# mountain/qingdai

Measured on AMD Instinct MI355X. Metric: simulated planet-days/sec at 721x1440 f64, higher is better.
Workload: dtype f64; 1 GPU; 721x1440 seed-42 planet, dt=300 s: forcing + time_step(Teq, dt, albedo) with QD_ENERGY_W=1 QD_CLOUD_COUPLE=1 + slab-ocean coupling + driver-side precipitation/cloud/albedo diagnostics (run_simulation.py:1766-1934,2063-2146) (BASELINE configs[2]; loop order of benchmark_jax.py:124-158); ocean_n_sub=13, parallelism=lat-bands x1

## Files before the change

qingdai_amd/csrc/qd_api.hip:

```cpp
#include "qd_span.h"
#include <chrono>
#include <atomic>
#include <cstring>
#include <cstdio>
#include <cstdlib>
#include <algorithm>

thread_local std::string g_qd_create_err;

int qd_fail(qd_ctx* c, const char* what, hipError_t e) {
    std::string m = what ? what : "error";
    if (e != hipSuccess) { m += ": "; m += hipGetErrorString(e); }
    if (c) c->err = m; else g_qd_create_err = m;
    return -1;
}

static hipEvent_t qd_get_event(qd_ctx* c) {
    if (!c->ev_free.empty()) { hipEvent_t e = c->ev_free.back(); c->ev_free.pop_back(); return e; }
    hipEvent_t e = nullptr;
    hipEventCreate(&e);
    return e;
}
QdScope::QdScope(qd_ctx* c_, const char* n, bool attach_) : c(c_), name(n), attach(attach_) {
    on = c->timing == 1;
// ... 64 lines not shown
        double s = (lat_deg - p.polar_sponge_lat) / std::max(1e-6, 90.0 - p.polar_sponge_lat);
        s = std::min(std::max(s, 0.0), 1.0);
        rx[i] = p.polar_sponge_gain * (s * s);
    }
    {
        const double a = p.a, dphi = c->dlat, dlam = c->dlon;
        const double f_min = 2.0 * p.omega * std::sin(5.0 * (M_PI / 180.0));
        for (int k = 0; k < 2; ++k) {
            const std::vector<double>& ck = k == 0 ? c02 : c05;
            std::vector<double> A(nlat), P(nlat), Q(nlat);
            for (int i = 0; i < nlat; ++i) {
                A[i] = ck[i] / (2.0 * dphi);
                P[i] = 1.0 / ((a * a) * ck[i] * (2.0 * dphi));
                Q[i] = 1.0 / ((a * a) * (dlam * dlam) * (ck[i] * ck[i]));
            }
            std::vector<double> PA(8, 0.0);
            if (nlat >= 5) {
                const int n = nlat;
                PA[0] = ck[0] / dphi;               PA[1] = ck[1] / (2.0 * dphi);      P[0] = 1.0 / ((a * a) * ck[0] * dphi);
                PA[2] = ck[0] / dphi;               PA[3] = ck[2] / (2.0 * dphi);      P[1] = 1.0 / ((a * a) * ck[1] * (2.0 * dphi));
                PA[4] = ck[n - 3] / (2.0 * dphi);   PA[5] = ck[n - 1] / dphi;          P[n - 2] = 1.0 / ((a * a) * ck[n - 2] * (2.0 * dphi));
                PA[6] = ck[n - 2] / (2.0 * dphi);   PA[7] = ck[n - 1] / dphi;          P[n - 1] = 1.0 / ((a * a) * ck[n - 1] * dphi);
            }
            c->tabs.lapA[k] = dev_table(c, A); c->tabs.lapP[k] = dev_table(c, P); c->tabs.lapQ[k] = dev_table(c, Q);
            c->tabs.lapPoleA[k] = dev_table(c, PA);
            std::vector<double> K4((size_t)nlat * 4);
            for (int i = 0; i < nlat; ++i) {
                K4[4 * i + 0] = A[i > 0 ? i - 1 : 0]; K4[4 * i + 1] = A[i < nlat - 1 ? i + 1 : nlat - 1];
                K4[4 * i + 2] = P[i]; K4[4 * i + 3] = Q[i];
            }
            c->tabs.lapK[k] = dev_table(c, K4);
            c->h_lapK[k] = K4;
        }
        std::vector<double> cu(nlat), cv(nlat), px(nlat), igx(nlat), ia6(nlat);
        for (int i = 0; i < nlat; ++i) {
            const double f = fc[i];
            const double sgn = f >= 0.0 ? 1.0 : -1.0;
            const double f_safe = std::fabs(f) < f_min ? sgn * f_min : f;
            cu[i] = -(p.g / (f_safe * a * c6[i]));
            cv[i] = p.g / (f_safe * a);
            px[i] = -(p.g / (a * c6[i]));
            igx[i] = 1.0 / (a * c05[i]);
            ia6[i] = 1 / (a * c6[i]);
        }
        c->tabs.mom_cu = dev_table(c, cu); c->tabs.mom_cv = dev_table(c, cv); c->tabs.mom_px = dev_table(c, px);
        c->tabs.ocn_igx = dev_table(c, igx);
        c->tabs.inv_acos6 = dev_table(c, ia6);
    }
    std::vector<double> lr(nlon), sl(nlon), cl(nlon);
    for (int j = 0; j < nlon; ++j) { lr[j] = lon[j] * d2r; sl[j] = std::sin(lr[j]); cl[j] = std::cos(lr[j]); }
    QdTabs& T = c->tabs;
    T.cos_raw = dev_table(c, cr); T.sin_raw = dev_table(c, sr); T.cos6 = dev_table(c, c6); T.cos3 = dev_table(c, c3);
    T.cos02 = dev_table(c, c02); T.cos05 = dev_table(c, c05); T.fcor = dev_table(c, fc); T.warea = dev_table(c, wa);
    T.r_extra = dev_table(c, rx);
    T.lat_deg = dev_table(c, lat);
    T.lon_rad = dev_table(c, lr); T.sin_lon = dev_table(c, sl); T.cos_lon = dev_table(c, cl);
    if (!T.cos_raw || !T.lon_rad || !T.cos_lon) return -1;
    double ws = 0.0;
    for (int i = 0; i < nlat; ++i) ws += wa[i] * nlon;
    c->wsum_all = ws;
    return 0;
}

int qd_build_k4_tables(qd_ctx* c, double dt, bool ocean, double sub_dt) {
    const int nlat = c->geo.nlat;
    const qd_params& p = c->p;
    const double d2r = M_PI / 180.0;
    std::vector<double> lat = linspace(-90.0, 90.0, nlat);
    auto isset = [](double x) { return !(x != x); };
    if (!ocean) {
        if (c->k4_atm_dt == dt) return 0;
        std::vector<double> tab((size_t)5 * nlat);
        const double scale[5] = {1.0, 1.0, 0.5, 0.5, 0.25};
        const double ov[5] = {p.k4_u, p.k4_v, p.k4_h, p.k4_q, p.k4_cloud};
        bool anypos[5] = {false, false, false, false, false};
        for (int i = 0; i < nlat; ++i) {
            const double cs = std::max(std::cos(lat[i] * d2r), 1e-3);
            const double dxm = std::min(p.a * c->dlat, p.a * c->dlon * cs);
            const double base = p.sigma4 * std::pow(dxm, 4.0) / std::max(1e-12, dt);
            for (int f = 0; f < 5; ++f) {
// ... 738 lines not shown
```

qingdai_amd/csrc/qd_atmos.hip:

```cpp
#include "qd_internal.h"
#include "qd_pointwise.h"
#include "qd_device.h"
#include "qd_saf.h"

#include "qd_fluxes.h"
#include "qd_fused.h"

struct QdColPtrs {
    const double *u, *v, *Teq, *isr, *albedo, *csmap;
    double *h, *Ts, *q, *cloud, *hice;
    double *E, *Pcond, *LH, *LHrel, *olr, *cloud_eff;
    const uint8_t* land;
    const double* pref;
    unsigned long long* npos;
};

struct QdColIn { double cloud, isr, albedo, teq; };

template <int PHASE, bool HAS_ALB>
__device__ __forceinline__ void qd_column_cell(const QdColP& P, const QdColPtrs& A, size_t o, const QdColIn* IN, int i, int nlat) {
    const double u = A.u[o], v = A.v[o], h = A.h[o], Ts = A.Ts[o];
    const double hice = A.hice[o];
    const bool land = (A.land[o] == 1);
    const bool ocean = !land;
    const double T_a = 288.0 + P.ga * h;
    const double qsat_air = qd_qsat(T_a, P.p0);

    const QdHum Hm = qd_humidity_column(P, u, v, Ts, A.q[o], qsat_air, land, hice);
    const double q = Hm.q, E = Hm.E, Pc = Hm.Pc, LH = Hm.LH, LHrel = Hm.LHrel;
    if (PHASE == 1) { A.Pcond[o] = Pc; return; }
    A.q[o] = q; A.LH[o] = LH;
    if (PHASE != 2) A.Pcond[o] = Pc;
    if (P.write_diag) { A.E[o] = E; A.LHrel[o] = LHrel; }

    const double Teq = IN ? IN->teq : A.Teq[o];
    const double olr_old = P.sigma * qd_pow4(Ts);
    const double net_old = P.sigma * qd_pow4(Teq) + P.gfs * qd_pow4(T_a) - olr_old;
    const double Ts_newton = Ts + (net_old / P.c_sfc_safe) * P.dt;

    double Ts_new, h_new = h;
    QdFlux F;
    if (HAS_ALB) {
        const double cloud = IN ? IN->cloud : A.cloud[o];
        double cloud_eff;
        if (P.couple) {
            const double RH = qd_clip(q / qd_max(1e-12, qsat_air), 0.0, 1.5);
            const double rh_excess = qd_max(0.0, RH - P.rh0);
            const double P_ref = *A.pref;
            const double p_term = qd_tanh(P_ref > 0 ? Pc / P_ref : 0.0);
            cloud_eff = qd_clip(cloud + P.k_q * rh_excess + P.k_p * p_term, 0.0, 1.0);
        } else cloud_eff = cloud;
        A.cloud_eff[o] = cloud_eff;
        F = qd_surface_fluxes(P, IN ? IN->isr : A.isr[o], IN ? IN->albedo : A.albedo[o], cloud_eff, Ts, T_a, u, v, land, hice);
        double Ts_energy;
        if (P.seaice) {
            double Q = F.SW_sfc - F.LW_sfc - F.SH - LH;
            double Tn = Ts, hi = hice;
            if (hi > 0.0 && ocean && Q > 0.0) {
                const double dh_melt = (Q * P.dt) / P.rhoiLf;
                const double dh_cap = qd_min(dh_melt, hi);
                hi -= dh_cap;
                Q = Q - (dh_cap * P.rho_i * P.L_f) / P.dt;
            }
            if (ocean && Q < 0.0 && Tn <= (P.t_freeze + 0.5)) {
                hi += (-Q * P.dt) / P.rhoiLf;
                Q = 0.0;
                Tn = qd_min(Tn, P.t_freeze);
            }
            double Cs = land ? P.Cs_land : (hi > 0.0 ? P.Cs_ice : P.Cs_ocean);
            Cs = (isfinite(Cs) && Cs > 1e3) ? Cs : 1e3;
            Tn = Tn + (Q / Cs) * P.dt;
            if ((i == 0 && P.fix_s) || (i == nlat - 1 && P.fix_n)) {
                if (ocean && Q < 0.0 && Tn > P.t_freeze) Tn = P.t_freeze;
            }
            if (hi > 0.0 && ocean) Tn = qd_min(Tn, P.t_freeze);
            Tn = qd_max(P.t_floor, Tn);
            Ts_energy = qd_nn(Tn);
            { const double hn_ = qd_nn(hi); if (__double_as_longlong(hn_) != __double_as_longlong(hice)) A.hice[o] = hn_; }
        } else {
            const double net = F.SW_sfc - F.LW_sfc - F.SH - LH;
            double Cs;
            if (P.has_csmap) { const double cm = A.csmap[o]; Cs = (isfinite(cm) && cm > 1e3) ? cm : 1e3; }
            else Cs = P.c_sfc_safe;
            Ts_energy = qd_nn(qd_max(P.t_floor, Ts + (net / Cs) * P.dt));
        }
        if (P.write_diag) A.olr[o] = F.OLR;
        Ts_new = (1.0 - P.w_energy) * Ts_newton + P.w_energy * Ts_energy;
    } else {
        if (P.write_diag) A.olr[o] = olr_old;
        Ts_new = Ts_newton;
    }
    A.Ts[o] = Ts_new;

    const double h_eq = P.h_eq_fac * Teq;
    h_new = h + ((h_eq - h) / P.tau_rad) * P.dt;
    if (HAS_ALB && P.atm_couple) {
        const double F_atm = F.SW_atm + F.LW_atm + F.SH + LHrel;
        h_new = qd_nn(h_new + P.atm_w * (F_atm / P.atm_denom) * P.dt);
    }
    A.h[o] = h_new;
}

template <int PHASE, bool HAS_ALB>
__global__ void __launch_bounds__(QD_BLOCK)
k_column(QdGeom G, QdColP P, QdColPtrs A) {
    const QdTile tl = qd_tile();
    const int j = tl.seg * QD_BLOCK + threadIdx.x;
    if (j >= G.nlon) return;
    const int i = G.row0 + tl.row;
    qd_column_cell<PHASE, HAS_ALB>(P, A, (size_t)qd_lrow(G, i) * G.nlon + j, nullptr, i, G.nlat);
}

__global__ void __launch_bounds__(QD_BLOCK)
k_saf_column2(QdSafArgs K, QdColP P, QdColPtrs A) {
    const QdTile tl = qd_tile();
    const int j = tl.seg * QD_BLOCK + threadIdx.x;
    if (j >= K.G.nlon) return;
    const int i = K.G.row0 + tl.row;
    const size_t o = (size_t)qd_lrow(K.G, i) * K.G.nlon + j;
    const QdSafOut s = qd_saf_cell(K, i, j, o, K.write_diag != 0);
    const QdColIn in{s.cloud, s.isr, s.albedo, s.teq};
    qd_column_cell<2, true>(P, A, o, &in, i, K.G.nlat);
}

struct QdMomP { double g, a, dt, dlat, dlon, f_min; int primitive; };

__global__ void __launch_bounds__(QD_BLOCK)
k_momentum(QdGeom G, QdTabs T, QdMomP P, const double* __restrict__ h, const double* __restrict__ fric,
           double* __restrict__ u, double* __restrict__ v) {
    const QdTile tl = qd_tile();
    const int j = tl.seg * QD_BLOCK + threadIdx.x;
    if (j >= G.nlon) return;
    const int i = G.row0 + tl.row;
    const int n = G.nlat, m = G.nlon;
    const size_t b = (size_t)qd_lrow(G, i) * m;
    const size_t o = b + j;
    double dh_dlon;
    if (j == 0) dh_dlon = (h[b + 1] - h[b]) / P.dlon;
    else if (j == m - 1) dh_dlon = (h[b + m - 1] - h[b + m - 2]) / P.dlon;
    else dh_dlon = (h[b + j + 1] - h[b + j - 1]) / (2.0 * P.dlon);
    double dh_dlat;
    if (i == 0) dh_dlat = (h[(size_t)qd_lrow(G, 1) * m + j] - h[o]) / P.dlat;
    else if (i == n - 1) dh_dlat = (h[o] - h[(size_t)qd_lrow(G, n - 2) * m + j]) / P.dlat;
    else dh_dlat = (h[(size_t)qd_lrow(G, i + 1) * m + j] - h[(size_t)qd_lrow(G, i - 1) * m + j]) / (2.0 * P.dlat);
    const double cosc = T.cos6[i];
    const double f = T.fcor[i];
    const double r = fric[o];
    const double u0 = u[o], v0 = v[o];
    if (P.primitive) {
        const double PGF_x = -(P.g / (P.a * cosc)) * dh_dlon;
        const double PGF_y = -(P.g / P.a) * dh_dlat;
        const double du = (PGF_x + f * v0 - r * u0) * P.dt;
        const double dv = (PGF_y - f * u0 - r * v0) * P.dt;
        u[o] = qd_clip(u0 + du, -200.0, 200.0);
        v[o] = qd_clip(v0 + dv, -200.0, 200.0);
    } else {
        const double sgn = (f >= 0.0) ? 1.0 : -1.0;
        const double f_safe = (fabs(f) < P.f_min) ? sgn * P.f_min : f;
        const double u_g = qd_clip(-(P.g / (f_safe * P.a * cosc)) * dh_dlat, -200.0, 200.0);
        const double v_g = qd_clip((P.g / (f_safe * P.a)) * dh_dlon, -200.0, 200.0);
        double un = u0 * 0.8 + u_g * 0.2;
        double vn = v0 * 0.8 + v_g * 0.2;
        un = un + (-r * un) * P.dt;
        vn = vn + (-r * vn) * P.dt;
        u[o] = un; v[o] = vn;
    }
}

__global__ void __launch_bounds__(QD_BLOCK)
k_final(QdGeom G, const double* __restrict__ cosl, double dt, double a, double dlat, double dlon,
        double* __restrict__ u, double* __restrict__ v, double* __restrict__ h, double* __restrict__ Ts,
        double* __restrict__ q, const double* __restrict__ cloud_in, double* __restrict__ cloud_out,
        double decay, double dfac) {
    const QdTile tl = qd_tile();
    const int j = tl.seg * QD_BLOCK + threadIdx.x;
    if (j >= G.nlon) return;
    const int i = G.row0 + tl.row;
    const size_t o = (size_t)qd_lrow(G, i) * G.nlon + j;
    const double uu = u[o], vv = v[o];
    const QdBilin b = qd_departure(G, i, j, uu, vv, dt, a, cosl[i], dlat, dlon);
    double c = qd_gather(cloud_in, G, b);
    c = c * decay;
    cloud_out[o] = qd_nn(c * dfac);
    u[o] = qd_nn(uu * dfac);
    v[o] = qd_nn(vv * dfac);
    h[o] = qd_nn(h[o] * dfac);
    q[o] = qd_nn(q[o] * dfac);
    Ts[o] = qd_nn(Ts[o]);
}

__global__ void __launch_bounds__(QD_BLOCK)
k_forcing(QdGeom G, QdTabs T, QdForcingP P, double* __restrict__ isrA, double* __restrict__ isrB, double* __restrict__ isr,
          const double* __restrict__ albedo, double* __restrict__ Teq, double* __restrict__ eday, double eday_dt) {
    const QdTile tl = qd_tile();
    const int j = tl.seg * QD_BLOCK + threadIdx.x;
    if (j >= G.nlon) return;
    const int i = G.row0 + tl.row;
    const size_t o = (size_t)qd_lrow(G, i) * G.nlon + j;
    qd_forcing_cell(T, P, i, j, o, P.with_teq ? albedo[o] : 0.0, isrA, isrB, isr, Teq, eday, eday_dt);
}

int qd_forcing_impl(qd_ctx* c, const double* sa, const double* sb, double theta, int with_teq) {
    QdScope sc(c, "forcing");
    QdStar A{sa[0], std::sin(sa[1]), std::cos(sa[1]), sa[2]};
    QdStar B{sb[0], std::sin(sb[1]), std::cos(sb[1]), sb[2]};
    const int m = with_teq ? qd_plan(c, {QD_IN(c->f[QD_F_ALBEDO], 0)}) : c->geo.halo;
    if (m < 0) return -1;
    const QdForcingP FP{A, B, theta, 5.670374e-8, with_teq};
    QD_ROWS(c, m, G, hipLaunchKernelGGL(k_forcing, qd_grid2d(G), dim3(QD_BLOCK), 0, c->stream, G, c->tabs, FP,
                                        c->f[QD_F_ISR_A], c->f[QD_F_ISR_B], c->f[QD_F_ISR],
                                        c->f[QD_F_ALBEDO], c->f[QD_F_TEQ], c->eco.eday_dt > 0 ? c->f[QD_F_ECO_EDAY] : (double*)nullptr,
                                        c->eco.eday_dt));
    c->eco.eday_dt = 0;
// ... 24 lines not shown

QdColP qd_make_colp(const qd_ctx* c, double dt) {
    const qd_params& p = c->p;
    QdColP P;
    P.ga = p.g / 1004.0;
    P.M_col = std::max(1e-6, p.rho_a * p.h_mbl);
    P.tau_c = std::max(1e-6, p.tau_cond);
    P.L_v = p.L_v; P.p0 = p.p0; P.rhoCE = p.rho_a * p.C_E;
    P.s_ocean = p.ocean_evap_scale; P.s_land = p.land_evap_scale; P.s_ice = p.ice_evap_scale;
    P.sigma = 5.670374e-8;
    P.gfs = p.greenhouse_factor * P.sigma;
    P.c_sfc_safe = std::max(1e-12, p.c_sfc);
    P.dt = dt;
    P.rh0 = p.rh0; P.k_q = p.k_q; P.k_p = p.k_p;
    P.sw_a0 = p.sw_a0; P.sw_kc = p.sw_kc; P.lw_eps0 = p.lw_eps0; P.lw_kc = p.lw_kc;
    P.eps_clear = std::min(std::max(p.lw_eps0, 0.0), 1.0);
    P.tau0 = p.lw_tau0; P.k_tau = p.lw_ktau;
    P.hice_ref_safe = std::max(1e-6, p.hice_ref);
    P.eps_ocean = p.eps_ocean; P.eps_land = p.eps_land; P.eps_ice = p.eps_ice; P.eps_default = p.eps_default;
    P.g_lw = p.gh_factor_lw;
    P.rhocpch = p.rho_a * p.cp_a * p.ch;
    P.t_freeze = p.t_freeze; P.rho_i = p.rho_i; P.L_f = p.L_f; P.rhoiLf = p.rho_i * p.L_f;
    P.Cs_ocean = p.Cs_ocean; P.Cs_land = p.Cs_land; P.Cs_ice = p.Cs_ice; P.t_floor = p.t_floor;
    P.w_energy = std::min(1.0, std::max(0.0, p.energy_w));
    P.h_eq_fac = 287.0 / p.g;
    P.tau_rad = p.tau_rad;
    const double H_atm = qd_isset(p.atm_h) ? p.atm_h : p.h_mbl;
    P.atm_denom = std::max(1e-6, p.rho_a) * std::max(1.0, H_atm) * p.g;
    P.atm_w = p.energy_w;
    P.atm_couple = (p.energy_w > 0.0) ? 1 : 0;
    P.couple = p.cloud_couple; P.lw_v2 = p.lw_v2; P.gh_lock = p.gh_lock; P.seaice = p.seaice_enabled;
    P.fix_s = p.polar_freeze_fix_s; P.fix_n = p.polar_freeze_fix_n; P.has_csmap = p.has_csmap;
    P.write_diag = c->diag_write;
    return P;
}

__global__ void k_set_scalar(double* p, double v) { if (threadIdx.x == 0 && blockIdx.x == 0) *p = v; }
__global__ void k_zero_count(unsigned long long* p) { if (threadIdx.x == 0 && blockIdx.x == 0) *p = 0ull; }

static QdColPtrs qd_col_ptrs(qd_ctx* c) {
    double** F = c->f;
    QdColPtrs A;
    A.u = F[QD_F_U]; A.v = F[QD_F_V]; A.Teq = F[QD_F_TEQ]; A.isr = F[QD_F_ISR];
    A.albedo = F[QD_F_ALBEDO]; A.csmap = F[QD_F_CSMAP];
    A.h = F[QD_F_H]; A.Ts = F[QD_F_TS]; A.q = F[QD_F_Q]; A.cloud = F[QD_F_CLOUD]; A.hice = F[QD_F_HICE];
    A.E = F[QD_F_EFLUX]; A.Pcond = F[QD_F_PCOND]; A.LH = F[QD_F_LH]; A.LHrel = F[QD_F_LHREL];
    A.olr = F[QD_F_OLR]; A.cloud_eff = F[QD_F_CLOUD_EFF];
    A.land = c->land; A.pref = c->dscal + QD_S_PREF; A.npos = c->dcount;
    return A;
}

int qd_pcond_phase1(qd_ctx* c, double dt) {
    hipLaunchKernelGGL((k_column<1, true>), qd_grid2d(c->geo), dim3(QD_BLOCK), 0, c->stream, c->geo, qd_make_colp(c, dt), qd_col_ptrs(c));
    return 0;
}
int qd_pcond_median_side(qd_ctx* c, double dt) {
    QD_HIP(c, hipEventRecord(c->med_fork, c->stream));
    QD_HIP(c, hipStreamWaitEvent(c->side_stream, c->med_fork, 0));
    std::swap(c->stream, c->side_stream);
    c->med_side_active = true;
    const QdColP P = qd_make_colp(c, dt);
    const QdColPtrs A = qd_col_ptrs(c);
    hipLaunchKernelGGL((k_column<1, true>), qd_grid2d(c->geo), dim3(QD_BLOCK), 0, c->stream, c->geo, P, A);
    const int r = qd_median_positive_dev(c, c->f[QD_F_PCOND], 1e-6, QD_S_PREF, 0, 0.0, 1);
    c->med_side_active = false;
    std::swap(c->stream, c->side_stream);
// ... 13 lines not shown

    if (c->saf_pending && !(has_albedo && p.cloud_couple && !qd_isset(p.pcond_ref) && c->pcond_ahead == 3) && qd_saf_flush(c)) return -1;
    {
        QdScope sc(c, "column");
        int m = has_albedo
            ? qd_plan(c, {QD_IN(F[QD_F_U], 0), QD_IN(F[QD_F_V], 0), QD_IN(F[QD_F_H], 0), QD_IN(F[QD_F_TS], 0), QD_IN(F[QD_F_Q], 0),
                          QD_IN(F[QD_F_CLOUD], 0), QD_IN(F[QD_F_HICE], 0), QD_IN(F[QD_F_TEQ], 0), QD_IN(F[QD_F_ISR], 0),
                          QD_IN(F[QD_F_ALBEDO], 0)})
            : qd_plan(c, {QD_IN(F[QD_F_U], 0), QD_IN(F[QD_F_V], 0), QD_IN(F[QD_F_H], 0), QD_IN(F[QD_F_TS], 0), QD_IN(F[QD_F_Q], 0),
                          QD_IN(F[QD_F_HICE], 0), QD_IN(F[QD_F_TEQ], 0)});
        if (m < 0) return -1;
        QdColPtrs A;
        A.u = F[QD_F_U]; A.v = F[QD_F_V]; A.Teq = F[QD_F_TEQ]; A.isr = F[QD_F_ISR];
        A.albedo = F[QD_F_ALBEDO]; A.csmap = F[QD_F_CSMAP];
        A.h = F[QD_F_H]; A.Ts = F[QD_F_TS]; A.q = F[QD_F_Q]; A.cloud = F[QD_F_CLOUD]; A.hice = F[QD_F_HICE];
        A.E = F[QD_F_EFLUX]; A.Pcond = F[QD_F_PCOND]; A.LH = F[QD_F_LH]; A.LHrel = F[QD_F_LHREL];
        A.olr = F[QD_F_OLR]; A.cloud_eff = F[QD_F_CLOUD_EFF];
        A.land = c->land; A.pref = c->dscal + QD_S_PREF; A.npos = c->dcount;
        if (!has_albedo) {
            QD_ROWS(c, m, G, hipLaunchKernelGGL((k_column<0, false>), qd_grid2d(G), blk, 0, c->stream, G, P, A));
        } else if (!p.cloud_couple || qd_isset(p.pcond_ref)) {
            hipLaunchKernelGGL(k_set_scalar, dim3(1), dim3(1), 0, c->stream, c->dscal + QD_S_PREF,
                               qd_isset(p.pcond_ref) ? p.pcond_ref : 1e-6);
            QD_ROWS(c, m, G, hipLaunchKernelGGL((k_column<0, true>), qd_grid2d(G), blk, 0, c->stream, G, P, A));
        } else {
            const int ahead = c->pcond_ahead;
            c->pcond_ahead = 0;
            if (!ahead) QD_ROWS(c, m, G, hipLaunchKernelGGL((k_column<1, true>), qd_grid2d(G), blk, 0, c->stream, G, P, A));
            if (ahead == 2) QD_HIP(c, hipStreamWaitEvent(c->stream, c->med_done, 0));
            else if (ahead != 3 && qd_median_positive_dev(c, F[QD_F_PCOND], 1e-6, QD_S_PREF, 0, 0.0, 1)) return -1;
            if (c->saf_pending && ahead == 3 && c->geo.full) {
                QdSafArgs* K = (QdSafArgs*)c->saf_pending;
                c->saf_pending = nullptr;
                hipLaunchKernelGGL(k_saf_column2, qd_grid2d(K->G), blk, 0, c->stream, *K, P, A);
                delete K;
            } else {
                if (qd_saf_flush(c)) return -1;
                QD_ROWS(c, m, G, hipLaunchKernelGGL((k_column<2, true>), qd_grid2d(G), blk, 0, c->stream, G, P, A));
            }
        }
        qd_mark(c, {F[QD_F_H], F[QD_F_TS], F[QD_F_Q], F[QD_F_EFLUX], F[QD_F_PCOND], F[QD_F_LH], F[QD_F_LHREL], F[QD_F_OLR]}, m);
        if (has_albedo) { qd_mark(c, {F[QD_F_HICE], F[QD_F_CLOUD_EFF]}, m); c->cloud_eff_valid = 1; }
    }
    c->atm_counter += 1;
    const int64_t sc_ = c->atm_counter;

    {
        QdScope sc(c, "advect_tsq");
        const int m = qd_plan(c, {QD_IN(F[QD_F_TS], R), QD_IN(F[QD_F_Q], R), QD_IN(F[QD_F_U], 0), QD_IN(F[QD_F_V], 0)});
        if (m < 0) return -1;
        double* oT = qd_scratch(c, 0); double* oq = qd_scratch(c, 1);
        qd_launch_advect(c, F[QD_F_U], F[QD_F_V], c->tabs.cos6, dt, F[QD_F_TS], oT, F[QD_F_Q], oq, 0.2, 1, m);
        qd_swap(c, QD_F_TS, 0); qd_swap(c, QD_F_Q, 1);
    }
    const int ft = p.filter_type;
    const bool do_diff = p.diff_enable && (ft == 0 || ft == 1) && (sc_ % std::max(1, p.diff_every) == 0);
    const double f_min = 2.0 * p.omega * std::sin(5.0 * (M_PI / 180.0));
    if (do_diff) { int rc = qd_build_k4_tables(c, dt, false, 0.0); if (rc) return rc; }
    const double ov[5] = {p.k4_u, p.k4_v, p.k4_h, p.k4_q, p.k4_cloud};
    if (do_diff && c->use_fused && p.k4_nsub == 1) {
        const int m = qd_plan(c, {QD_IN(F[QD_F_H], 5), QD_IN(F[QD_F_U], 4), QD_IN(F[QD_F_V], 4), QD_IN(F[QD_F_FRICTION], 4),
                                  QD_IN(F[QD_F_Q], 4), QD_IN(F[QD_F_CLOUD], 4)});
        if (m < 0) return -1;
        QdDynArgs D;
        D.u = F[QD_F_U]; D.v = F[QD_F_V]; D.h = F[QD_F_H]; D.fric = F[QD_F_FRICTION];
        D.q = F[QD_F_Q]; D.cloud = F[QD_F_CLOUD];
        D.uo = qd_scratch(c, 0); D.vo = qd_scratch(c, 1); D.ho = qd_scratch(c, 2); D.qo = qd_scratch(c, 3); D.co = qd_scratch(c, 4);
// ... 41 lines not shown
        const int m = qd_plan(c, {QD_IN(F[QD_F_U], np_), QD_IN(F[QD_F_V], np_), QD_IN(F[QD_F_H], np_)});
        if (m < 0) return -1;
        double* fl[3] = {F[QD_F_U], F[QD_F_V], F[QD_F_H]};
        qd_shapiro_fields(c, fl, 3, np_, m);
        F[QD_F_U] = fl[0]; F[QD_F_V] = fl[1]; F[QD_F_H] = fl[2];
        const int n1 = std::max(1, p.shapiro_n - 1);
        if (p.diff_q) {
            const int mq = qd_plan(c, {QD_IN(F[QD_F_Q], n1)}); if (mq < 0) return -1;
            double* g1[1] = {F[QD_F_Q]}; qd_shapiro_fields(c, g1, 1, n1, mq); F[QD_F_Q] = g1[0];
        }
        if (p.diff_cloud) {
            const int mc = qd_plan(c, {QD_IN(F[QD_F_CLOUD], n1)}); if (mc < 0) return -1;
            double* g1[1] = {F[QD_F_CLOUD]}; qd_shapiro_fields(c, g1, 1, n1, mc); F[QD_F_CLOUD] = g1[0];
        }
    }
    if ((ft == 0 || ft == 3) && p.spec_every > 0 && (sc_ % p.spec_every == 0)) {
        QdScope sc(c, "zonal_filter");
        const int m = qd_plan(c, {QD_IN(F[QD_F_U], 0), QD_IN(F[QD_F_V], 0), QD_IN(F[QD_F_H], 0)});
        if (m < 0) return -1;
        double* fl[3] = {F[QD_F_U], F[QD_F_V], F[QD_F_H]};
        if (qd_zonal_filter_fields(c, fl, 3, p.spec_cutoff, p.spec_damp, m)) return -1;
    }
    {
        QdScope sc(c, "final");
        const int m = qd_plan(c, {QD_IN(F[QD_F_CLOUD], R), QD_IN(F[QD_F_U], 0), QD_IN(F[QD_F_V], 0), QD_IN(F[QD_F_H], 0),
                                  QD_IN(F[QD_F_TS], 0), QD_IN(F[QD_F_Q], 0)});
        if (m < 0) return -1;
        const double decay = 1 - dt / (2.0 * 24 * 3600);
        if (c->defer_final && c->geo.full) {
            c->final_pending.on = 1; c->final_pending.dt = dt; c->final_pending.decay = decay; c->final_pending.dfac = p.diff_factor;
            return 0;
        }
        double* oc = qd_scratch(c, 0);
        QD_ROWS(c, m, G, hipLaunchKernelGGL(k_final, qd_grid2d(G), blk, 0, c->stream, G, c->tabs.cos6, dt, p.a, c->dlat, c->dlon,
                                            F[QD_F_U], F[QD_F_V], F[QD_F_H], F[QD_F_TS], F[QD_F_Q], F[QD_F_CLOUD], oc, decay,
                                            p.diff_factor));
        qd_mark(c, {F[QD_F_U], F[QD_F_V], F[QD_F_H], F[QD_F_TS], F[QD_F_Q], oc}, m);
        qd_swap(c, QD_F_CLOUD, 0);
    }
    return 0;
}
```

qingdai_amd/csrc/qd_device.h:

```cpp
#pragma once
#include "qd_internal.h"
#include "qd_math.h"

template <bool SCRUB>
__device__ __forceinline__ double qd_ld(const double* __restrict__ F, const QdGeom& G, int g, int j) {
    double x = F[(size_t)qd_lrow(G, g) * G.nlon + j];
    return SCRUB ? qd_nn(x) : x;
}

template <bool SCRUB>
__device__ __forceinline__ double qd_dphi(const double* __restrict__ F, const QdGeom& G, int r, int j, double dphi) {
    const int n = G.nlat;
    if (r == 0) return (qd_ld<SCRUB>(F, G, 1, j) - qd_ld<SCRUB>(F, G, 0, j)) / dphi;
    if (r == n - 1) return (qd_ld<SCRUB>(F, G, n - 1, j) - qd_ld<SCRUB>(F, G, n - 2, j)) / dphi;
    return (qd_ld<SCRUB>(F, G, r + 1, j) - qd_ld<SCRUB>(F, G, r - 1, j)) / (2.0 * dphi);
}

template <bool SCRUB>
__device__ __forceinline__ double qd_lap_point(const double* __restrict__ F, const QdGeom& G,
                                               const double* __restrict__ cosf, int i, int j,
                                               double dphi, double dlam, double a) {
    const int n = G.nlat;
    int ra, rb; double den;
    if (i == 0) { ra = 0; rb = 1; den = dphi; }
// ... 4 lines not shown
    const double ci = cosf[i];
    const double term_phi = (1.0 / ci) * ((Gb - Ga) / den);
    const int jp = qd_wrapc(j + 1, G.nlon), jm = qd_wrapc(j - 1, G.nlon);
    const double c = qd_ld<SCRUB>(F, G, i, j);
    const double d2 = ((qd_ld<SCRUB>(F, G, i, jp) - 2.0 * c) + qd_ld<SCRUB>(F, G, i, jm)) / (dlam * dlam);
    const double term_lam = d2 / (ci * ci);
    return (term_phi + term_lam) / (a * a);
}


template <bool SCRUB>
__device__ __forceinline__ double qd_lap_point_fast(const double* __restrict__ F, const QdGeom& G, const QdTabs& T,
                                                    int k, int i, int j, double dphi, double dlam, double a) {
    if (i < 2 || i > G.nlat - 3) return qd_lap_point<SCRUB>(F, G, k ? T.cos05 : T.cos02, i, j, dphi, dlam, a);
    const int jp = qd_wrapc(j + 1, G.nlon), jm = qd_wrapc(j - 1, G.nlon);
    const double cc = qd_ld<SCRUB>(F, G, i, j);
    const double Gb = T.lapA[k][i + 1] * (qd_ld<SCRUB>(F, G, i + 2, j) - cc);
    const double Ga = T.lapA[k][i - 1] * (cc - qd_ld<SCRUB>(F, G, i - 2, j));
    const double d2 = (qd_ld<SCRUB>(F, G, i, jp) - 2.0 * cc) + qd_ld<SCRUB>(F, G, i, jm);
    return T.lapP[k][i] * (Gb - Ga) + T.lapQ[k][i] * d2;
}

__device__ __forceinline__ double qd_fold(double x, int n) {
    const double sz = (double)(n - 1);
    if (n <= 1) return 0.0;
    if (x < 0.0) return x + sz * (trunc(-x / sz) + 1.0);
    if (x > sz) return x - sz * trunc(x / sz);
    return x;
}

struct QdBilin { int l0, l1, c0, c1; double wr0, wr1, wc0, wc1; bool nan_coord; };

__device__ __forceinline__ QdBilin qd_departure(const QdGeom& G, int gi, int j, double u, double v, double dt,
                                                double a, double cosl, double dlat, double dlon) {
    const double dl = u * dt / (a * cosl);
    const double dp = v * dt / a;
    const double dx = dl / dlon;
    const double dy = dp / dlat;
    double r = qd_fold((double)gi - dy, G.nlat);
    double cc = qd_fold((double)j - dx, G.nlon);
    const bool nan_coord = (dx != dx) || (dy != dy);
    r = fmin(fmax(r, 0.0), (double)(G.nlat - 1));
    cc = fmin(fmax(cc, 0.0), (double)(G.nlon - 1));
    const double r0f = floor(r), c0f = floor(cc);
    QdBilin b;
    const int r0 = (int)r0f, c0 = (int)c0f;
    const int r1 = r0 + 1 < G.nlat ? r0 + 1 : G.nlat - 1;
    b.c0 = c0; b.c1 = c0 + 1 < G.nlon ? c0 + 1 : G.nlon - 1;
    b.l0 = qd_lrow_far(G, r0); b.l1 = qd_lrow_far(G, r1);
    const double tr = r - r0f, tc = cc - c0f;
    b.wr0 = 1.0 - tr; b.wr1 = tr; b.wc0 = 1.0 - tc; b.wc1 = tc;
    b.nan_coord = nan_coord;
    return b;
}

__device__ __forceinline__ double qd_gather(const double* __restrict__ F, const QdGeom& G, const QdBilin& b) {
    const size_t r0 = (size_t)b.l0 * G.nlon, r1 = (size_t)b.l1 * G.nlon;
    double t = 0.0;
    t += F[r0 + b.c0] * b.wr0 * b.wc0;
    t += F[r0 + b.c1] * b.wr0 * b.wc1;
    t += F[r1 + b.c0] * b.wr1 * b.wc0;
    t += F[r1 + b.c1] * b.wr1 * b.wc1;
    return b.nan_coord ? 0.0 : t;
}


__device__ __forceinline__ double qd_divvort_point(const QdGeom& G, const QdTabs& T, const double* __restrict__ p,
                                                   const double* __restrict__ q, int i, int j, double a,
                                                   double dlat, double dlon, int vort) {
    const size_t b = (size_t)qd_lrow(G, i) * G.nlon;
    const int jp = qd_wrapc(j + 1, G.nlon), jm = qd_wrapc(j - 1, G.nlon);
    const double dp = (p[b + jp] - p[b + jm]) / (2 * dlon);
    double dq = 0.0;
    if (i != 0 && i != G.nlat - 1) {
        const double qn = q[(size_t)qd_lrow(G, i + 1) * G.nlon + j] * T.cos_raw[i + 1];
        const double qs = q[(size_t)qd_lrow(G, i - 1) * G.nlon + j] * T.cos_raw[i - 1];
        dq = (qn - qs) / (2 * dlat);
    }
    const double pre = 1 / (a * T.cos6[i]);
    return vort ? pre * (dp - dq) : pre * (dp + dq);
}
```

qingdai_amd/csrc/qd_fluxes.h:

```cpp
#pragma once
#include "qd_internal.h"

#define QD_EPSILON 0.622

struct QdColP {
    double ga;
    double M_col, tau_c, L_v, p0, rhoCE, s_ocean, s_land, s_ice;
    double sigma, gfs, c_sfc_safe, dt;
    double rh0, k_q, k_p;
    double sw_a0, sw_kc, lw_eps0, lw_kc, eps_clear, tau0, k_tau, hice_ref_safe;
    double eps_ocean, eps_land, eps_ice, eps_default;
    double g_lw, rhocpch;
    double t_freeze, rhoiLf, rho_i, L_f, Cs_ocean, Cs_land, Cs_ice, t_floor;
    double w_energy, h_eq_fac, tau_rad, atm_denom, atm_w;
    int couple, lw_v2, gh_lock, seaice, fix_s, fix_n, has_csmap, atm_couple;
    int write_diag = 1;
};

__device__ __forceinline__ double qd_qsat(double T, double p0) {
    const double T_c = qd_clip(T - 273.15, -80.0, 60.0);
    const double e_s = 610.94 * exp(17.625 * T_c / (T_c + 243.04));
    const double denom = qd_max(p0 - (1.0 - QD_EPSILON) * e_s, 1.0);
    return qd_clip(QD_EPSILON * e_s / denom, 0.0, 0.5);
}

struct QdHum { double q, E, Pc, LH, LHrel; };
__device__ __forceinline__ QdHum qd_humidity_column(const QdColP& P, double u, double v, double Ts, double q0, double qsat_air,
                                                    bool land, double hice) {
    QdHum r;
    const double fac = land ? P.s_land : ((hice > 1e-6) ? P.s_ice : P.s_ocean);
    const double V = sqrt(u * u + v * v);
    const double deficit = qd_max(0.0, qd_qsat(Ts, P.p0) - q0);
    r.E = qd_nn(P.rhoCE * V * deficit * fac);
    r.LH = P.L_v * r.E;
    const double q_evap = q0 + (r.E / P.M_col) * P.dt;
    const double excess = qd_max(0.0, q_evap - qsat_air);
    double Pc = (excess / P.tau_c) * P.M_col;
    double q_next = q_evap - (Pc / P.M_col) * P.dt;
    q_next = qd_clip(qd_nn(q_next), 0.0, 0.5);
    r.Pc = qd_nn(Pc);
    r.LHrel = P.L_v * r.Pc;
    r.q = qd_clip(qd_nn(q_next), 0.0, 0.5);
    return r;
}

struct QdFlux { double SW_atm, SW_sfc, R, LW_atm, LW_sfc, OLR, SH; };

__device__ __forceinline__ QdFlux qd_surface_fluxes(const QdColP& P, double I, double albedo, double cloud_eff,
                                                    double Ts, double Ta, double u, double v, bool land, double hice) {
    QdFlux F;
    const double alpha = qd_clip(albedo, 0.0, 1.0);
    const double Ic = qd_max(0.0, I);
    F.R = Ic * alpha;
    const double A_sw = qd_clip(P.sw_a0 + P.sw_kc * qd_clip(cloud_eff, 0.0, 1.0), 0.0, 0.95);
    F.SW_atm = Ic * A_sw;
    F.SW_sfc = qd_max(0.0, Ic - F.R - F.SW_atm);
    const double s = P.sigma;
    const double Tsp = qd_max(0.0, Ts), Tap = qd_max(0.0, Ta);
    const double Ts4 = qd_pow4(Tsp), Ta4 = qd_pow4(Tap);
    if (P.lw_v2) {
        const double ce = qd_clip(cloud_eff, 0.0, 1.0);
        const double tau_cloud = P.tau0 * ce;
        const double eps_cloud = qd_clip(1.0 - exp(-P.k_tau * tau_cloud), 0.0, 1.0);
        const double eps_eff = 1.0 - (1.0 - P.eps_clear) * (1.0 - eps_cloud);
        double es;
        if (land) es = P.eps_land;
        else {
            const double ice_frac = 1.0 - exp(-qd_max(hice, 0.0) / P.hice_ref_safe);
            const double fi = qd_clip(ice_frac, 0.0, 1.0);
            es = (1.0 - fi) * P.eps_ocean + fi * P.eps_ice;
        }
        es = qd_clip(qd_nn(es), 0.0, 1.0);
        F.OLR = eps_eff * s * Ta4 + (1.0 - eps_eff) * s * es * Ts4;
        const double DLR = eps_eff * s * Ta4;
        F.LW_sfc = DLR - s * es * Ts4;
        F.LW_atm = eps_eff * (s * es * Ts4 - 2.0 * s * Ta4);
        if (P.gh_lock) {
            F.OLR = (1.0 - P.g_lw) * s * Ts4;
            const double DLRt = P.g_lw * s * Ts4;
            F.LW_sfc = DLRt - s * es * Ts4;
        }
    } else {
        const double eps = qd_clip(P.lw_eps0 + P.lw_kc * qd_clip(cloud_eff, 0.0, 1.0), 0.0, 1.0);
        F.OLR = eps * s * Ta4 + (1.0 - eps) * s * Ts4;
        const double DLR = eps * s * Ta4;
        F.LW_sfc = DLR - s * Ts4;
        F.LW_atm = eps * (s * Ts4 - 2.0 * s * Ta4);
        if (P.gh_lock) {
            F.OLR = (1.0 - P.g_lw) * s * Ts4;
            const double DLRt = P.g_lw * s * Ts4;
            F.LW_sfc = DLRt - s * Ts4;
        }
    }
    const double V = sqrt(u * u + v * v);
    F.SH = P.rhocpch * V * (Ts - Ta);
    return F;
}
```

qingdai_amd/csrc/qd_internal.h:

```cpp
#pragma once

#include <hip/hip_runtime.h>
#include <hip/hip_ext.h>
#include <stdint.h>
#include <string>
#include <vector>
#include <functional>
#include <map>
#include <unordered_map>
#include <initializer_list>
#include <climits>
#include <cfloat>
#include <cmath>

#include "../../include/qingdai_hip.h"

#define QD_NSCRATCH 16
#define QD_MAX_DEVICES 64
#define QD_PAD_ROWS 8
#define QD_BLOCK 256
#define QD_MAXF 5
#define QD_HIST_BINS 2048

struct QdGeom {
    int nlat, nlon;
    int row0, nrows, halo;
    int full;
    int lbase;
    int lrows_;
    __host__ __device__ inline int lrows() const { return lrows_; }
    __host__ __device__ inline size_t cells() const { return (size_t)lrows() * (size_t)nlon; }
};

struct QdTabs {
    const double* cos_raw;
    const double* sin_raw;
    const double* cos6;
    const double* cos3;
    const double* cos02;
    const double* cos05;
    const double* fcor;
    const double* warea;
    const double* r_extra;
    const double* lapA[2];
    const double* lapP[2];
    const double* lapQ[2];
    const double* lapPoleA[2];
    const double* lapK[2];
    const double* mom_cu;
    const double* mom_cv;
    const double* mom_px;
    const double* ocn_igx;
    const double* inv_acos6;
    const double* lat_deg;
    const double* lon_rad;
    const double* sin_lon;
    const double* cos_lon;
};

__device__ __forceinline__ double qd_nn(double x) {
    if (x != x) return 0.0;
    if (x > DBL_MAX) return DBL_MAX;
    if (x < -DBL_MAX) return -DBL_MAX;
    return x;
}
__device__ __forceinline__ double qd_max(double a, double b) {
    return (a >= b || a != a) ? a : b;
}
__device__ __forceinline__ double qd_min(double a, double b) {
    return (a <= b || a != a) ? a : b;
}
__device__ __forceinline__ double qd_clip(double x, double lo, double hi) {
    return qd_min(qd_max(x, lo), hi);
}
__device__ __forceinline__ double qd_pow4(double x) { double x2 = x * x; return x2 * x2; }

__device__ __forceinline__ int qd_lrow(const QdGeom& G, int g) {
    int l = g - G.lbase;
    if (l < 0) l += G.nlat; else if (l >= G.nlat) l -= G.nlat;
    return l;
}
__device__ __forceinline__ int qd_lrow_far(const QdGeom& G, int g) {
    int l = g - G.lbase;
    if (l < 0) l += G.nlat; else if (l >= G.nlat) l -= G.nlat;
    if (l >= G.lrows()) l = G.lrows() - 1;
    return l;
}
__device__ __forceinline__ int qd_wrapc(int j, int n) {
    return j < 0 ? j + n : (j >= n ? j - n : j);
}

// ... 365 lines not shown
```

qingdai_amd/csrc/qd_math.h:

```cpp
#pragma once
#include <math.h>
#ifdef __HIPCC__
#define QD_MATH_FN __host__ __device__ __forceinline__
#else
#define QD_MATH_FN static inline
#endif

QD_MATH_FN double qd_expm1_pos(double y) {
    const double k = rint(y * 1.4426950408889634);
    double r = fma(k, -6.93147180369123816490e-01, y);
    r = fma(k, -1.90821492927058770002e-10, r);
    double p = 1.0 / 6227020800.0;
    p = fma(p, r, 1.0 / 479001600.0);
    p = fma(p, r, 1.0 / 39916800.0);
    p = fma(p, r, 1.0 / 3628800.0);
    p = fma(p, r, 1.0 / 362880.0);
    p = fma(p, r, 1.0 / 40320.0);
    p = fma(p, r, 1.0 / 5040.0);
    p = fma(p, r, 1.0 / 720.0);
    p = fma(p, r, 1.0 / 120.0);
    p = fma(p, r, 1.0 / 24.0);
    p = fma(p, r, 1.0 / 6.0);
    p = fma(p, r, 0.5);
    p = fma(p, r, 1.0);
    const double pm1 = p * r;
    const double twok = ldexp(1.0, (int)k);
    return fma(twok, pm1, twok - 1.0);
}

QD_MATH_FN double qd_tanh_nonneg(double x) {
    const double s = x * x;
    double q = 18888466084.0 / 194896477400625.0;
    q = fma(q, s, -443861162.0 / 1856156927625.0);
    q = fma(q, s, 6404582.0 / 10854718875.0);
    q = fma(q, s, -929569.0 / 638512875.0);
    q = fma(q, s, 21844.0 / 6081075.0);
    q = fma(q, s, -1382.0 / 155925.0);
    q = fma(q, s, 62.0 / 2835.0);
    q = fma(q, s, -17.0 / 315.0);
    q = fma(q, s, 2.0 / 15.0);
    q = fma(q, s, -1.0 / 3.0);
    const double small = fma(x * s, q, x);
    const double xe = x < 19.1 ? x : 19.1;
    const double em1 = qd_expm1_pos(xe + xe);
    const double big = em1 / (em1 + 2.0);
    const double t = x < 0.25 ? small : big;
    return x != x ? x : t;
}

QD_MATH_FN double qd_tanh(double x) { return copysign(qd_tanh_nonneg(fabs(x)), x); }
```

qingdai_amd/csrc/qd_ocean.hip:

```cpp
#include <cstdlib>
#include <atomic>
#include <chrono>
#include "qd_internal.h"
#include "qd_device.h"
#include "qd_wave.h"

#include "qd_fluxes.h"
#include "qd_fused.h"
#include "qd_ocntail.h"
#include "qd_band.h"
#include "qd_blockred.h"

QdColP qd_make_colp(const qd_ctx* c, double dt);

__global__ void __launch_bounds__(QD_BLOCK)
k_qnet(QdGeom G, QdColP P, const double* __restrict__ isr, const double* __restrict__ albedo,
       const double* __restrict__ cloud, const double* __restrict__ Ts, const double* __restrict__ h,
       const double* __restrict__ u, const double* __restrict__ v, const uint8_t* __restrict__ land,
       const double* __restrict__ hice, const double* __restrict__ LH, double* __restrict__ qnet,
       uint8_t* __restrict__ icemask) {
    const QdTile tl = qd_tile();
    const int j = tl.seg * QD_BLOCK + threadIdx.x;
    if (j >= G.nlon) return;
    const size_t o = (size_t)qd_lrow(G, G.row0 + tl.row) * G.nlon + j;
// ... 84 lines not shown
             double* __restrict__ taux, double* __restrict__ tauy, double* __restrict__ partial, double* seq_out, double seq) {
    __shared__ double sm[2][QD_BLOCK / 64];
    const int i = G.row0 + blockIdx.y;
    const size_t b = (size_t)qd_lrow(G, i) * G.nlon;
    double mVa = 0.0, mUo = 0.0;
    for (int j = threadIdx.x; j < G.nlon; j += QD_BLOCK) {
        const size_t o = b + j;
        const double u_o = uo[o], v_o = vo[o];
        const double u_rel = ua[o] - u_o, v_rel = va[o] - v_o;
        const double Va = sqrt(u_rel * u_rel + v_rel * v_rel);
        const double Va_eff = qd_min(Va, vcap);
        taux[o] = tau_scale * (rhoCD * Va_eff * u_rel);
        tauy[o] = tau_scale * (rhoCD * Va_eff * v_rel);
        const double so = sqrt(u_o * u_o + v_o * v_o);
        mVa = Va > mVa ? Va : mVa;
        mUo = so > mUo ? so : mUo;
    }
    mVa = qd_wave_max(mVa); mUo = qd_wave_max(mUo);
    const int lane = threadIdx.x & 63, w = threadIdx.x >> 6;
    if (lane == 0) { sm[0][w] = mVa; sm[1][w] = mUo; }
    __syncthreads();
    if (threadIdx.x == 0) {
        for (int k = 1; k < QD_BLOCK / 64; ++k) { mVa = sm[0][k] > mVa ? sm[0][k] : mVa; mUo = sm[1][k] > mUo ? sm[1][k] : mUo; }
        partial[blockIdx.y] = mVa;
        partial[gridDim.y + blockIdx.y] = mUo;
        if (seq_out) {
            asm volatile("s_waitcnt vmcnt(0)" ::: "memory");
            __hip_atomic_store(seq_out + blockIdx.y, seq, __ATOMIC_RELAXED, __HIP_MEMORY_SCOPE_SYSTEM);
        }
    }
}

struct QdFqsArgs {
    const double* cosl; double dt, a, dlat, dlon, decay, dfac;
    double *u, *v, *h, *Ts, *q; const double* cloud_in; double* cloud_out;
    const double *isr, *albedo, *cloud_eff, *hice, *LH; const uint8_t* land; double* qnet; uint8_t* icemask;
    const double *uo, *vo; double vcap, rhoCD, tau_scale; double *taux, *tauy;
    double* dev_wg; int n_wg;
};
__global__ void __launch_bounds__(QD_BLOCK)
k_final_qnet_stress(QdGeom G, QdColP P, QdFqsArgs A) {
    __shared__ double sm[2][QD_BLOCK / 64];
    const QdTile tl = qd_tile();
    const int j = tl.seg * QD_BLOCK + threadIdx.x;
    const int i = G.row0 + tl.row;
    double Va = 0.0, so = 0.0;
    if (j < G.nlon) {
        const size_t o = (size_t)qd_lrow(G, i) * G.nlon + j;
        const double uu = A.u[o], vv = A.v[o];
        const QdBilin b = qd_departure(G, i, j, uu, vv, A.dt, A.a, A.cosl[i], A.dlat, A.dlon);
        double c = qd_gather(A.cloud_in, G, b);
        c = c * A.decay;
        const double cn = qd_nn(c * A.dfac), un = qd_nn(uu * A.dfac), vn = qd_nn(vv * A.dfac);
        const double t0 = A.Ts[o];
        const double hn = qd_nn(A.h[o] * A.dfac), tn = qd_nn(t0);
        A.cloud_out[o] = cn; A.u[o] = un; A.v[o] = vn; A.h[o] = hn; A.q[o] = qd_nn(A.q[o] * A.dfac);
        if (__double_as_longlong(tn) != __double_as_longlong(t0)) A.Ts[o] = tn;
        const double u_o = A.uo[o], v_o = A.vo[o];
        const double u_rel = un - u_o, v_rel = vn - v_o;
        Va = sqrt(u_rel * u_rel + v_rel * v_rel);
        const double Va_eff = qd_min(Va, A.vcap);
        A.taux[o] = A.tau_scale * (A.rhoCD * Va_eff * u_rel);
        A.tauy[o] = A.tau_scale * (A.rhoCD * Va_eff * v_rel);
        so = sqrt(u_o * u_o + v_o * v_o);
        const double T_a = 288.0 + P.ga * hn;
        const double hi = A.hice[o];
        const QdFlux F = qd_surface_fluxes(P, A.isr[o], A.albedo[o], A.cloud_eff ? A.cloud_eff[o] : cn, tn, T_a, un, vn, A.land[o] == 1, hi);
        A.qnet[o] = F.SW_sfc - F.LW_sfc - F.SH - A.LH[o];
        A.icemask[o] = (hi > 0.0) ? 1 : 0;
    }
    double mVa = Va > 0.0 ? Va : 0.0, mUo = so > 0.0 ? so : 0.0;
    mVa = qd_wave_max(mVa); mUo = qd_wave_max(mUo);
    const int lane = threadIdx.x & 63, w = threadIdx.x >> 6;
    if (lane == 0) { sm[0][w] = mVa; sm[1][w] = mUo; }
    __syncthreads();
    if (threadIdx.x == 0) {
        for (int k = 1; k < QD_BLOCK / 64; ++k) { mVa = sm[0][k] > mVa ? sm[0][k] : mVa; mUo = sm[1][k] > mUo ? sm[1][k] : mUo; }
        const unsigned wg = (unsigned)tl.row * gridDim.x + (unsigned)tl.seg;
        A.dev_wg[wg] = mVa; A.dev_wg[A.n_wg + wg] = mUo;
    }
}

__global__ void __launch_bounds__(1024)
// ... 37 lines not shown
}

struct QdOcnP { double a, g, dlat, dlon, sub_dt, rhoH, r_bot; };

__global__ void __launch_bounds__(QD_BLOCK)
k_ocean_momentum(QdGeom G, QdTabs T, QdOcnP P, const double* __restrict__ eta, const double* __restrict__ taux,
                 const double* __restrict__ tauy, const uint8_t* __restrict__ land,
                 double* __restrict__ uo, double* __restrict__ vo) {
    const QdTile tl = qd_tile();
    const int j = tl.seg * QD_BLOCK + threadIdx.x;
    if (j >= G.nlon) return;
    const int i = G.row0 + tl.row;
    const size_t b = (size_t)qd_lrow(G, i) * G.nlon;
    const size_t o = b + j;
    const int jp = qd_wrapc(j + 1, G.nlon), jm = qd_wrapc(j - 1, G.nlon);
    const double deta_dlam = (eta[b + jp] - eta[b + jm]) / (2.0 * P.dlon);
    const double deta_dphi = (eta[(size_t)qd_lrow(G, i + 1) * G.nlon + j] - eta[(size_t)qd_lrow(G, i - 1) * G.nlon + j]) / (2.0 * P.dlat);
    const double gx = deta_dlam / (P.a * T.cos05[i]);
    const double gy = deta_dphi / P.a;
    const double f = T.fcor[i];
    const double u0 = uo[o], v0 = vo[o];
    const double du = (f * v0 - P.g * gx + taux[o] / P.rhoH - P.r_bot * u0);
    const double dv = (-f * u0 - P.g * gy + tauy[o] / P.rhoH - P.r_bot * v0);
    double un = u0 + P.sub_dt * du;
    double vn = v0 + P.sub_dt * dv;
    if (land[o] == 1) { un = 0.0; vn = 0.0; }
    const double rx = T.r_extra[i];
    un = un - P.sub_dt * rx * un;
    vn = vn - P.sub_dt * rx * vn;
    uo[o] = un; vo[o] = vn;
}

__global__ void __launch_bounds__(QD_BLOCK)
k_continuity(QdGeom G, QdTabs T, double a, double dlat, double dlon, double msdtH, const double* __restrict__ uo,
             const double* __restrict__ vo, const uint8_t* __restrict__ land, double* __restrict__ eta,
             double* __restrict__ partial) {
    __shared__ double sm[QD_BLOCK / 64];
    const int i = G.row0 + blockIdx.y;
    const size_t b = (size_t)qd_lrow(G, i) * G.nlon;
    const double w = T.warea[i];
    double acc = 0.0;
    for (int j = threadIdx.x; j < G.nlon; j += QD_BLOCK) {
        const size_t o = b + j;
        const double div = qd_divvort_point(G, T, uo, vo, i, j, a, dlat, dlon, 0);
        double e = eta[o] + msdtH * div;
        const bool island = land[o] == 1;
        if (island) e = 0.0;
        eta[o] = e;
        acc += e * (island ? 0.0 : w);
    }
    acc = qd_wave_sum(acc);
    const int lane = threadIdx.x & 63, wv = threadIdx.x >> 6;
    if (lane == 0) sm[wv] = acc;
    __syncthreads();
    if (threadIdx.x == 0) {
        double r = sm[0];
        for (int k = 1; k < QD_BLOCK / 64; ++k) r += sm[k];
        partial[blockIdx.y] = r;
    }
}

__global__ void __launch_bounds__(QD_BLOCK)
k_eta_mean(const double* __restrict__ partial, int n, double wsum, double* __restrict__ out, double seq = 0.0) {
    __shared__ double sm[QD_BLOCK / 64];
    double acc = 0.0;
    for (int k = threadIdx.x; k < n; k += QD_BLOCK) acc += partial[k];
    acc = qd_wave_sum(acc);
    const int lane = threadIdx.x & 63, wv = threadIdx.x >> 6;
    if (lane == 0) sm[wv] = acc;
    __syncthreads();
    if (threadIdx.x == 0) {
        double r = sm[0];
        for (int k = 1; k < QD_BLOCK / 64; ++k) r += sm[k];
        *out = (wsum < 0.0) ? r : r / (wsum + 1e-15);
        if (seq != 0.0) __hip_atomic_store(&out[1], seq, __ATOMIC_RELEASE, __HIP_MEMORY_SCOPE_SYSTEM);
    }
}

__global__ void __launch_bounds__(QD_BLOCK)
k_cont_sstadv(QdGeom G, QdTabs T, double a, double dlat, double dlon, double msdtH, double sub_dt, double alpha,
              const double* __restrict__ uo, const double* __restrict__ vo, const uint8_t* __restrict__ land,
              double* __restrict__ eta, const double* __restrict__ Ts, double* __restrict__ Ts_out,
              int own0, int own1, double* __restrict__ partial, unsigned long long* ticket, double wsum,
              double* __restrict__ eta_mean) {
    __shared__ double sm[QD_BLOCK / 64];
    __shared__ int s_last;
    const int i = G.row0 + blockIdx.y;
    const size_t b = (size_t)qd_lrow(G, i) * G.nlon;
    const double w = (i >= own0 && i < own1) ? T.warea[i] : 0.0;
    const double cosl = T.cos05[i];
    const int pidx = blockIdx.y * gridDim.x + blockIdx.x, pcount = gridDim.x * gridDim.y;
    double acc = 0.0;
    for (int j = blockIdx.x * QD_BLOCK + threadIdx.x; j < G.nlon; j += gridDim.x * QD_BLOCK) {
        const size_t o = b + j;
        const double div = qd_divvort_point(G, T, uo, vo, i, j, a, dlat, dlon, 0);
        double e = eta[o] + msdtH * div;
        const bool island = land[o] == 1;
        if (island) e = 0.0;
        eta[o] = e;
        acc += e * (island ? 0.0 : w);
        const QdBilin bl = qd_departure(G, i, j, uo[o], vo[o], sub_dt, a, cosl, dlat, dlon);
        Ts_out[o] = (1.0 - alpha) * Ts[o] + alpha * qd_gather(Ts, G, bl);
    }
    acc = qd_wave_sum(acc);
    const int lane = threadIdx.x & 63, wv = threadIdx.x >> 6;
    if (lane == 0) sm[wv] = acc;
    __syncthreads();
    if (threadIdx.x == 0) {
        double r = sm[0];
        for (int k = 1; k < QD_BLOCK / 64; ++k) r += sm[k];
        if (!ticket) partial[pidx] = r;
        else {
            __hip_atomic_store(&partial[pidx], r, __ATOMIC_RELAXED, __HIP_MEMORY_SCOPE_AGENT);
            asm volatile("s_waitcnt vmcnt(0)" ::: "memory");
            const unsigned long long t = atomicAdd(ticket, 1ull);
            s_last = (t == (unsigned long long)pcount - 1ull) ? 1 : 0;
        }
    }
    if (!ticket) return;
    __syncthreads();
    if (!s_last) return;
    double a2 = 0.0;
    for (int k = threadIdx.x; k < pcount; k += QD_BLOCK)
        a2 += __hip_atomic_load(&partial[k], __ATOMIC_RELAXED, __HIP_MEMORY_SCOPE_AGENT);
    a2 = qd_wave_sum(a2);
    __syncthreads();
    if (lane == 0) sm[wv] = a2;
    __syncthreads();
    if (threadIdx.x == 0) {
        double r = sm[0];
        for (int k = 1; k < QD_BLOCK / 64; ++k) r += sm[k];
        *eta_mean = r / (wsum + 1e-15);
        __hip_atomic_store(ticket, 0ull, __ATOMIC_RELAXED, __HIP_MEMORY_SCOPE_AGENT);
    }
}

__global__ void __launch_bounds__(QD_BLOCK)
k_sst_advect(QdGeom G, const double* __restrict__ cos05, double sub_dt, double a, double dlat, double dlon,
             const double* __restrict__ uo, const double* __restrict__ vo, const double* __restrict__ Ts,
             double* __restrict__ Ts_out, double alpha, double* __restrict__ eta, const double* __restrict__ eta_mean,
             int has_ocean) {
    const QdTile tl = qd_tile();
    const int j = tl.seg * QD_BLOCK + threadIdx.x;
    if (j >= G.nlon) return;
    const int i = G.row0 + tl.row;
    const size_t o = (size_t)qd_lrow(G, i) * G.nlon + j;
    if (has_ocean) eta[o] = eta[o] - *eta_mean;
    const QdBilin b = qd_departure(G, i, j, uo[o], vo[o], sub_dt, a, cos05[i], dlat, dlon);
    const double adv = qd_gather(Ts, G, b);
    Ts_out[o] = (1.0 - alpha) * Ts[o] + alpha * adv;
}

struct QdHeatP { double sub_dt, K_h, rcH, ice_qfac; int use_q, has_ice; };

__global__ void __launch_bounds__(QD_BLOCK)
k_sst_diffuse_heat(QdGeom G, const double* __restrict__ cos05, double dlat, double dlon, double a, QdHeatP P,
                   const double* __restrict__ Ts1, double* __restrict__ Ts_out, const double* __restrict__ qnet,
                   const uint8_t* __restrict__ land, const uint8_t* __restrict__ ice) {
    const QdTile tl = qd_tile();
    const int j = tl.seg * QD_BLOCK + threadIdx.x;
    if (j >= G.nlon) return;
    const int i = G.row0 + tl.row;
    const size_t o = (size_t)qd_lrow(G, i) * G.nlon + j;
    double T = Ts1[o];
    if (P.K_h > 0.0) T = qd_nn(T) + P.sub_dt * P.K_h * qd_lap_point<true>(Ts1, G, cos05, i, j, dlat, dlon, a);
    if (P.use_q) {
        const double heat = qnet[o] / P.rcH;
        const bool ocean = land[o] == 0;
        if (P.has_ice) {
            const bool ic = ice[o] != 0;
            if (ocean && !ic) T = T + P.sub_dt * heat;
            if (P.ice_qfac > 0.0 && ocean && ic) T = T + P.sub_dt * P.ice_qfac * heat;
        } else if (ocean) T = T + P.sub_dt * heat;
    }
    Ts_out[o] = qd_nn(T);
}

__global__ void __launch_bounds__(QD_BLOCK)
k_outlier(QdGeom G, const double* __restrict__ uo, const double* __restrict__ vo, double* __restrict__ uo_out,
          double* __restrict__ vo_out, double* __restrict__ eta, double cap, double eta_cap, int mean4) {
    const QdTile tl = qd_tile();
// ... 259 lines not shown
        QdScope sc(c, "ocean_qnet");
        QdColP P = qd_make_colp_driver(c, dt);
        double*& cl = c->cloud_eff_valid ? F[QD_F_CLOUD_EFF] : F[QD_F_CLOUD];
        const int m = qd_plan(c, {QD_IN(F[QD_F_ISR], 0), QD_IN(F[QD_F_ALBEDO], 0), QD_IN(cl, 0), QD_IN(F[QD_F_TS], 0),
                                  QD_IN(F[QD_F_H], 0), QD_IN(F[QD_F_U], 0), QD_IN(F[QD_F_V], 0), QD_IN(F[QD_F_HICE], 0),
                                  QD_IN(F[QD_F_LH], 0)});
        if (m < 0) return -1;
        QD_ROWS(c, m, G, hipLaunchKernelGGL(k_qnet, qd_grid2d(G), blk, 0, c->stream, G, P, F[QD_F_ISR], F[QD_F_ALBEDO], cl,
                                            F[QD_F_TS], F[QD_F_H], F[QD_F_U], F[QD_F_V], c->land, F[QD_F_HICE], F[QD_F_LH],
                                            F[QD_F_QNET], c->icemask));
        qd_mark(c, {F[QD_F_QNET], c->icemask}, m);
        use_ice_mask = 1;
        return 0;
    };
    if (compute_qnet && band && launch_qnet()) return -1;
    double*& taux = c->scratch[14];
    double*& tauy = c->scratch[15];
    int n_sub;
    bool band_fix_stats = false;
    {
        QdScope sc(c, "ocean_stress");
        const int m = qd_plan(c, {QD_IN(F[QD_F_U], 0), QD_IN(F[QD_F_V], 0), QD_IN(F[QD_F_UO], 0), QD_IN(F[QD_F_VO], 0)});
        if (m < 0) return -1;
        QdSegs S = qd_segments(c, m);
        double maxVa = 0.0, maxUo = 0.0;
        if (!band) {
            const QdGeom& G = S.g[0];
            c->eta_seq += 1.0;
            bool merged_final = false;
            if (c->final_pending.on) {
                if (!compute_qnet) return qd_fail(c, "ocean step: a deferred k_final needs compute_qnet");
                c->final_pending.on = 0;
                QdFqsArgs A;
                A.cosl = c->tabs.cos6; A.dt = c->final_pending.dt; A.a = p.a; A.dlat = c->dlat; A.dlon = c->dlon;
                A.decay = c->final_pending.decay; A.dfac = c->final_pending.dfac;
                A.u = F[QD_F_U]; A.v = F[QD_F_V]; A.h = F[QD_F_H]; A.Ts = F[QD_F_TS]; A.q = F[QD_F_Q];
                A.cloud_in = F[QD_F_CLOUD]; A.cloud_out = qd_scratch(c, 0);
                A.isr = F[QD_F_ISR]; A.albedo = F[QD_F_ALBEDO]; A.cloud_eff = c->cloud_eff_valid ? F[QD_F_CLOUD_EFF] : nullptr;
                A.hice = F[QD_F_HICE]; A.LH = F[QD_F_LH]; A.land = c->land; A.qnet = F[QD_F_QNET]; A.icemask = c->icemask;
                A.uo = F[QD_F_UO]; A.vo = F[QD_F_VO]; A.vcap = p.vcap; A.rhoCD = p.rho_a_ocean * p.CD; A.tau_scale = p.tau_scale;
                A.taux = taux; A.tauy = tauy;
                A.dev_wg = c->wgmax; A.n_wg = c->n_wgmax;
                merged_final = true;
                hipLaunchKernelGGL(k_final_qnet_stress, qd_grid2d(G), blk, 0, c->stream, G, qd_make_colp_driver(c, dt), A);
                hipLaunchKernelGGL(k_max2_publish, dim3(1), dim3(1024), 0, c->stream, c->wgmax, c->n_wgmax, c->hpin + 58, c->fix_count);
                qd_swap(c, QD_F_CLOUD, 0);
                use_ice_mask = 1;
            } else {
            hipLaunchKernelGGL(k_stress_max, dim3(1, G.nrows), blk, 0, c->stream, G, F[QD_F_U], F[QD_F_V], F[QD_F_UO],
                               F[QD_F_VO], p.vcap, p.rho_a_ocean * p.CD, p.tau_scale, taux, tauy, c->hpin_rows,
                               c->hpin_rows + (size_t)2 * G0.lrows(), c->eta_seq);
            qd_mark(c, {taux, tauy}, m);
            if (compute_qnet && launch_qnet()) return -1;
            }
            if (c->before_cfl_wait) {
                std::function<int()> fn = std::move(c->before_cfl_wait);
                c->before_cfl_wait = nullptr;
                if (c->side_stream_on && c->timing != 1 && !c->ocn_fused) {
                    QD_HIP(c, hipEventRecord(c->side_fork, c->stream));
                    QD_HIP(c, hipStreamWaitEvent(c->side_stream, c->side_fork, 0));
                    std::swap(c->stream, c->side_stream);
                    const int r = fn();
                    std::swap(c->stream, c->side_stream);
                    if (r) return -1;
                    QD_HIP(c, hipEventRecord(c->side_done, c->side_stream));
                    c->side_pending = true;
                } else if (fn()) return -1;
// ... 208 lines not shown
                const bool folded = qd_peer_fold_begin(c, &pf);
                if (fix_now && S.n == 1) { A.fix_count = c->fix_count; A.fix_list = c->fix_list; }
                for (int k = 0; k < S.n; ++k) {
                    const QdGeom& Gs = S.g[k];
                    const bool owned = Gs.row0 <= c->own_row0 && c->own_row0 < Gs.row0 + Gs.nrows;
                    A.acc = owned ? c->eta_acc : nullptr;
                    A.pf = owned ? pf : QdPeerFold();
                    A.partial = c->red_partial + off;
                    if (qd_launch_ocn_tail(c, Gs, A)) return -1;
                    off += (size_t)qd_ocn_tail_tiles(c, Gs);
                }
                if (!folded && qd_allreduce_sum_deferred(c, c->dscal + QD_S_ETA_MEAN)) return -1;
                if (A.fix_count) qd_mark(c, {F[QD_F_ETA], A.Ts_out, F[QD_F_UO], F[QD_F_VO]}, m);
                else qd_mark(c, {F[QD_F_ETA], A.Ts_out, A.uo_out, A.vo_out}, m);
            } else {
            if (fix_now) { A.fix_count = c->fix_count; A.fix_list = c->fix_list; }
            if (qd_launch_ocn_tail(c, Gown, A)) return -1;
            if (!tail_acc)
                hipLaunchKernelGGL(k_eta_mean_tail, dim3(1), dim3(256), 0, c->stream, c->red_partial, qd_ocn_tail_tiles(c, Gown), c->wsum_ocean,
                                   c->dscal + QD_S_ETA_MEAN);
            }
            qd_swap(c, QD_F_SST, 1);
            if (!A.fix_count) { qd_swap(c, QD_F_UO, 2); qd_swap(c, QD_F_VO, 3); }
        } else if (c->use_fused) {
            QdScope sc(c, "ocean_cont_sst");
            bool band_raw_mean = false;
            const int m = qd_plan(c, {QD_IN(F[QD_F_UO], 1), QD_IN(F[QD_F_VO], 1), QD_IN(F[QD_F_ETA], 0), QD_IN(F[QD_F_SST], Ro)});
            if (m < 0) return -1;
            double* T1 = qd_scratch(c, 0);
            const int own0 = c->own_row0, own1 = c->own_row0 + c->own_nrows;
            const int has_ocean = c->wsum_ocean > 0.0 ? 1 : 0;
            if (!band) {
                const dim3 g2 = qd_grid2d(Gown);
                hipLaunchKernelGGL(k_cont_sstadv, g2, blk, 0, c->stream, Gown, c->tabs, p.a, c->dlat, c->dlon, -sub_dt * H, sub_dt,
                                   p.ocean_adv_alpha, F[QD_F_UO], F[QD_F_VO], c->land, F[QD_F_ETA], F[QD_F_SST], T1, own0, own1,
                                   c->red_partial, (unsigned long long*)nullptr, 0.0, (double*)nullptr);
                if (!defer_eta)
                    hipLaunchKernelGGL(k_eta_mean, dim3(1), blk, 0, c->stream, c->red_partial, (int)(g2.x * g2.y), c->wsum_ocean,
                                       c->dscal + QD_S_ETA_MEAN);
            } else {
                QdSegs S = qd_segments(c, m);
                size_t off = 0;
                for (int k = 0; k < S.n; ++k) {
                    hipLaunchKernelGGL(k_cont_sstadv, qd_grid2d(S.g[k]), blk, 0, c->stream, S.g[k], c->tabs, p.a, c->dlat, c->dlon,
                                       -sub_dt * H, sub_dt, p.ocean_adv_alpha, F[QD_F_UO], F[QD_F_VO], c->land, F[QD_F_ETA],
                                       F[QD_F_SST], T1, own0, own1, c->red_partial + off, (unsigned long long*)nullptr, 0.0,
                                       (double*)nullptr);
                    off += (size_t)S.g[k].nrows * qd_grid2d(S.g[k]).x;
                }
                if (band_defer) {
                    c->eta_seq += 1.0;
                    hipLaunchKernelGGL(k_eta_mean, dim3(1), blk, 0, c->stream, c->red_partial, (int)off, -1.0, c->hpin + 40, c->eta_seq);
                } else {
                hipLaunchKernelGGL(k_eta_mean, dim3(1), blk, 0, c->stream, c->red_partial, (int)off, -1.0, c->dscal + QD_S_ETA_MEAN);
                if (qd_allreduce_f64(c, c->dscal + QD_S_ETA_MEAN, 1, 0)) return -1;
                band_raw_mean = !defer_eta;
                if (!band_raw_mean)
                    hipLaunchKernelGGL(k_eta_mean_post, dim3(1), dim3(64), 0, c->stream, c->dscal + QD_S_ETA_MEAN, c->wsum_ocean);
                }
            }
            qd_mark(c, {T1, F[QD_F_ETA]}, m);
            double*& T1s = c->scratch[0];
            double* T2 = qd_scratch(c, 1);
            const int m2 = qd_plan(c, {QD_IN(T1s, 2), QD_IN(F[QD_F_QNET], 0), QD_IN8(c->icemask, 0), QD_IN(F[QD_F_UO], 1),
                                       QD_IN(F[QD_F_VO], 1), QD_IN(F[QD_F_ETA], 0)});
            if (m2 < 0) return -1;
            double* u2 = qd_scratch(c, 2); double* v2 = qd_scratch(c, 3);
            QD_ROWS(c, m2, G, hipLaunchKernelGGL(k_sst_outlier_fused, qd_grid2d(G), blk, 0, c->stream, G, c->tabs, c->dlat,
                                                 c->dlon, p.a, HP, c->scratch[0], T2, F[QD_F_QNET], c->land, c->icemask,
                                                 F[QD_F_UO], F[QD_F_VO], u2, v2, F[QD_F_ETA], p.ocean_max_u, p.eta_cap,
                                                 p.ocean_outlier == 0 ? 1 : 0,
                                                 has_ocean ? c->dscal + QD_S_ETA_MEAN : (const double*)nullptr,
                                                 c->red_partial, band_defer ? 0 : (band_raw_mean ? -1 : (int)(qd_grid2d(Gown).x * qd_grid2d(Gown).y)), c->wsum_ocean,
                                                 band_defer ? c->dscal + QD_S_TMP1 : (defer_eta ? c->dscal + QD_S_ETA_MEAN : (double*)nullptr)));
            qd_mark(c, {T2, u2, v2, F[QD_F_ETA]}, m2);
            if (band_defer) {
                if (qd_wait_host_flag(c, c->hpin + 41, c->eta_seq, "ocean sub-step: the eta sum never arrived")) return -1;
                double sum = c->hpin[40];
                if (qd_host_allreduce(c, &sum, 1, 0)) return -1;
                c->hpin[42] = sum / (c->wsum_ocean + 1e-15);
            }
            qd_swap(c, QD_F_SST, 1); qd_swap(c, QD_F_UO, 2); qd_swap(c, QD_F_VO, 3);
        } else {
        {
            QdScope sc(c, "ocean_continuity");
            const int m = qd_plan(c, {QD_IN(F[QD_F_UO], 1), QD_IN(F[QD_F_VO], 1), QD_IN(F[QD_F_ETA], 0)});
            if (m < 0) return -1;
            if (band && m > 0) {
                QdSegs S = qd_segments(c, m);
                for (int k = 0; k < S.n; ++k) {
                    QdGeom G = S.g[k];
                    const int own0 = c->own_row0, own1 = c->own_row0 + c->own_nrows;
                    int a0 = G.row0, a1 = G.row0 + G.nrows;
                    auto run = [&](int r0, int r1) {
                        if (r1 <= r0) return;
                        QdGeom g2 = G; g2.row0 = r0; g2.nrows = r1 - r0;
                        hipLaunchKernelGGL(k_continuity, dim3(1, g2.nrows), blk, 0, c->stream, g2, c->tabs, p.a, c->dlat, c->dlon,
                                           -sub_dt * H, F[QD_F_UO], F[QD_F_VO], c->land, F[QD_F_ETA],
                                           c->red_partial + (size_t)G0.lrows());
                    };
                    if (a1 <= own0 || a0 >= own1) run(a0, a1);
                    else { run(a0, std::max(a0, own0)); run(std::min(a1, own1), a1); }
                }
            }
            hipLaunchKernelGGL(k_continuity, rows, blk, 0, c->stream, Gown, c->tabs, p.a, c->dlat, c->dlon, -sub_dt * H,
                               F[QD_F_UO], F[QD_F_VO], c->land, F[QD_F_ETA], c->red_partial);
            qd_mark(c, {F[QD_F_ETA]}, m);
            if (band) {
                hipLaunchKernelGGL(k_eta_mean, dim3(1), blk, 0, c->stream, c->red_partial, Gown.nrows, -1.0,
                                   c->dscal + QD_S_ETA_MEAN);
                if (qd_allreduce_f64(c, c->dscal + QD_S_ETA_MEAN, 1, 0)) return -1;
                hipLaunchKernelGGL(k_eta_mean_post, dim3(1), dim3(64), 0, c->stream, c->dscal + QD_S_ETA_MEAN, c->wsum_ocean);
            } else {
                hipLaunchKernelGGL(k_eta_mean, dim3(1), blk, 0, c->stream, c->red_partial, Gown.nrows, c->wsum_ocean,
                                   c->dscal + QD_S_ETA_MEAN);
            }
        }
        {
            QdScope sc(c, "ocean_sst");
            const int m1 = qd_plan(c, {QD_IN(F[QD_F_SST], Ro), QD_IN(F[QD_F_UO], 0), QD_IN(F[QD_F_VO], 0), QD_IN(F[QD_F_ETA], 0)});
            if (m1 < 0) return -1;
            double* T1 = qd_scratch(c, 0);
            QD_ROWS(c, m1, G, hipLaunchKernelGGL(k_sst_advect, qd_grid2d(G), blk, 0, c->stream, G, c->tabs.cos05, sub_dt, p.a,
                                                 c->dlat, c->dlon, F[QD_F_UO], F[QD_F_VO], F[QD_F_SST], T1, p.ocean_adv_alpha,
                                                 F[QD_F_ETA], c->dscal + QD_S_ETA_MEAN, c->wsum_ocean > 0.0 ? 1 : 0));
            qd_mark(c, {T1, F[QD_F_ETA]}, m1);
            double*& T1s = c->scratch[0];
            double* T2 = qd_scratch(c, 1);
            const int m2 = qd_plan(c, {QD_IN(T1s, 2), QD_IN(F[QD_F_QNET], 0), QD_IN8(c->icemask, 0)});
            if (m2 < 0) return -1;
            QD_ROWS(c, m2, G, hipLaunchKernelGGL(k_sst_diffuse_heat, qd_grid2d(G), blk, 0, c->stream, G, c->tabs.cos05,
                                                 c->dlat, c->dlon, p.a, HP, c->scratch[0], T2, F[QD_F_QNET], c->land,
                                                 c->icemask));
            qd_mark(c, {T2}, m2);
            qd_swap(c, QD_F_SST, 1);
        }
        }
        if (!c->use_fused) {
            QdScope sc(c, "ocean_outlier");
            const int m = qd_plan(c, {QD_IN(F[QD_F_UO], 1), QD_IN(F[QD_F_VO], 1), QD_IN(F[QD_F_ETA], 0)});
            if (m < 0) return -1;
            double* u2 = qd_scratch(c, 2); double* v2 = qd_scratch(c, 3);
            QD_ROWS(c, m, G, hipLaunchKernelGGL(k_outlier, qd_grid2d(G), blk, 0, c->stream, G, F[QD_F_UO], F[QD_F_VO], u2, v2,
                                                F[QD_F_ETA], p.ocean_max_u, p.eta_cap, p.ocean_outlier == 0 ? 1 : 0));
            qd_mark(c, {u2, v2, F[QD_F_ETA]}, m);
            qd_swap(c, QD_F_UO, 2); qd_swap(c, QD_F_VO, 3);
        }
    }
    if (qd_allreduce_flush(c)) return -1;
    if (c->budget_fire != 0.0 && qd_budget_ocean_energy(c, dt, use_ice_mask)) return -1;
    {
        QdScope sc(c, "ocean_finish");
        if (!band && p.ocean_polar_fix && c->merge_pointwise) {
            hipLaunchKernelGGL(k_polar_clamp_inject, qd_grid2d(G0), blk, 0, c->stream, G0, c->tabs, F[QD_F_SST], F[QD_F_UO], F[QD_F_VO],
                               p.ts_min, p.ts_max, inject_sst, c->land, c->icemask, use_ice_mask ? 1 : 0, F[QD_F_TS],
                               (defer_eta && n_sub > 0) ? F[QD_F_ETA] : (double*)nullptr, mean_ptr, p.eta_cap);
            return 0;
// ... 18 lines not shown
```

qingdai_amd/csrc/qd_ocntail.hip:

```cpp
#include "qd_internal.h"
#include "qd_device.h"
#include "qd_wave.h"
#include "qd_ocntail.h"
#include "qd_stream.h"
#include "qd_blockred.h"
#include <cstdlib>
#include <cstdio>
#include <vector>
#include <cstring>
#include <algorithm>


__device__ __forceinline__ double qt_div(double x, double c, double rc) {
    const double q0 = x * rc;
    const double e = __builtin_fma(-c, q0, x);
    const double q1 = __builtin_fma(e, rc, q0);
    return (q0 - q0 == 0.0) ? q1 : q0;
}

__device__ __forceinline__ double qt_div_fin(double x, double c, double rc) {
    const double q0 = x * rc;
    const double e = __builtin_fma(-c, q0, x);
    return __builtin_fma(e, rc, q0);
}

__device__ __forceinline__ QdBilin qt_departure(const QdGeom& G, int gi, int j, double u, double v, double dt,
                                                double acos, double r_acos, const QdTailArgs& P) {
    const double dl = qt_div(u * dt, acos, r_acos);
    const double dp = qt_div(v * dt, P.a, P.r_a);
    const double dx = qt_div(dl, P.dlon, P.r_dlon);
    const double dy = qt_div(dp, P.dlat, P.r_dlat);
    double r = qd_fold((double)gi - dy, G.nlat);
    double cc = qd_fold((double)j - dx, G.nlon);
    const bool nan_coord = (dx != dx) || (dy != dy);
    r = fmin(fmax(r, 0.0), (double)(G.nlat - 1));
    cc = fmin(fmax(cc, 0.0), (double)(G.nlon - 1));
    const double r0f = floor(r), c0f = floor(cc);
    QdBilin b;
    const int r0 = (int)r0f, c0 = (int)c0f;
    const int r1 = r0 + 1 < G.nlat ? r0 + 1 : G.nlat - 1;
    b.c0 = c0; b.c1 = c0 + 1 < G.nlon ? c0 + 1 : G.nlon - 1;
    b.l0 = qd_lrow_far(G, r0); b.l1 = qd_lrow_far(G, r1);
    const double tr = r - r0f, tc = cc - c0f;
    b.wr0 = 1.0 - tr; b.wr1 = tr; b.wc0 = 1.0 - tc; b.wc1 = tc;
    b.nan_coord = nan_coord;
    return b;
}

__device__ __forceinline__ double qt_div_point(const QdGeom& G, const QdTabs& T, const double* __restrict__ p,
                                               const double* __restrict__ q, int i, int j, const QdTailArgs& P) {
    const size_t b = (size_t)qd_lrow(G, i) * G.nlon;
    const int jp = qd_wrapc(j + 1, G.nlon), jm = qd_wrapc(j - 1, G.nlon);
    const double dp = qt_div(p[b + jp] - p[b + jm], 2 * P.dlon, P.r_2dlon);
    double dq = 0.0;
    if (i != 0 && i != G.nlat - 1) {
        const double qn = q[(size_t)qd_lrow(G, i + 1) * G.nlon + j] * T.cos_raw[i + 1];
        const double qs = q[(size_t)qd_lrow(G, i - 1) * G.nlon + j] * T.cos_raw[i - 1];
        dq = qt_div(qn - qs, 2 * P.dlat, P.r_2dlat);
    }
    return T.inv_acos6[i] * (dp + dq);
}


#define QS_TC2 62
#define QS_TCF 60

typedef unsigned int qt_u32x2 __attribute__((ext_vector_type(2)));
typedef __amdgpu_buffer_rsrc_t qt_rsrc;
__device__ __forceinline__ qt_rsrc qt_make_rsrc(const void* p, unsigned bytes) { return __builtin_amdgcn_make_buffer_rsrc(const_cast<void*>(p), 0, (int)bytes, 0x00020000); }
__device__ __forceinline__ double qt_ld(qt_rsrc r, unsigned row_elems, unsigned vo) { return __builtin_bit_cast(double, __builtin_amdgcn_raw_buffer_load_b64(r, vo, row_elems * 8u, 0)); }
__device__ __forceinline__ void qt_st(qt_rsrc r, unsigned row_elems, unsigned vo, double v) { __builtin_amdgcn_raw_buffer_store_b64(__builtin_bit_cast(qt_u32x2, v), r, vo, row_elems * 8u, 0); }
__device__ __forceinline__ int qt_ld8(qt_rsrc r, unsigned row_elems, unsigned vo8) { return (int)__builtin_amdgcn_raw_buffer_load_b8(r, vo8, row_elems, 0); }

#define QT_FIX_STAGE 512
struct QtFixW { unsigned int* fixc; unsigned long long* fixl; unsigned long long* stage; unsigned int* nstage; };
template <bool FIX>
__device__ __forceinline__ void qt_put_uv(const QtFixW& X, qt_rsrc UO, qt_rsrc VO, unsigned row_elems, unsigned vs,
                                          double u, double v, double uc, double vc) {
    if (!FIX) { qt_st(UO, row_elems, vs, u); qt_st(VO, row_elems, vs, v); return; }
    const unsigned long long ub = (unsigned long long)__double_as_longlong(u), vb = (unsigned long long)__double_as_longlong(v);
    const bool ch = vs != 0x80000000u && (ub != (unsigned long long)__double_as_longlong(uc) || vb != (unsigned long long)__double_as_longlong(vc));
    const unsigned long long chm = __builtin_amdgcn_ballot_w64(ch);
    if (chm != 0ull) {
        const int lane = (int)(threadIdx.x & 63u);
        const unsigned cnt = (unsigned)__popcll(chm);
        const unsigned base = __hip_atomic_load(X.nstage, __ATOMIC_RELAXED, __HIP_MEMORY_SCOPE_WAVEFRONT);
        const unsigned k = base + (unsigned)__popcll(chm & ((1ull << lane) - 1ull));
        const unsigned long long off = (unsigned long long)row_elems * 8ull + (unsigned long long)vs;
        if (base + cnt <= (unsigned)QT_FIX_STAGE) {
            if (ch) { X.stage[3u * k] = off; X.stage[3u * k + 1u] = ub; X.stage[3u * k + 2u] = vb; }
            if (lane == 0) __hip_atomic_store(X.nstage, base + cnt, __ATOMIC_RELAXED, __HIP_MEMORY_SCOPE_WAVEFRONT);
        } else {
            const int leader = __ffsll((long long)chm) - 1;
// ... 57 lines not shown
        const double div = qd_sload(T.inv_acos6, g) * (dp + dq);
        double e = e0 + P.msdtH * div;
        const bool island = l0 == 1;
        if (island) e = 0.0;
        const unsigned r0 = qt_row(W, g);
        qt_st(E, r0, W.vs, e);
        acc += (W.own && g >= W.own0 && g < W.own1) ? e * (island ? 0.0 : qd_sload(T.warea, g)) : 0.0;
        double u = qd_nn(uc), v = qd_nn(vc);
        const double cap = P.cap, s2 = u * u + v * v;
        const double ue = qd_east(uc), uw = qd_west(uc), ve = qd_east(vc), vw = qd_west(vc);
        if (!(s2 < 0.81 * (cap * cap))) {
            const double speed = sqrt(s2);
            if (P.mean4) {
                if (speed > cap) {
                    u = 0.25 * (qd_nn(un) + qd_nn(us) + qd_nn(ue) + qd_nn(uw));
                    v = 0.25 * (qd_nn(vn) + qd_nn(vs) + qd_nn(ve) + qd_nn(vw));
                }
                const double sp2 = sqrt(u * u + v * v);
                const double sc2 = (sp2 > cap) ? cap / (sp2 + 1e-12) : 1.0;
                u = u * sc2; v = v * sc2;
            } else {
                const double sc = (speed > cap) ? cap / (speed + 1e-12) : 1.0;
                u = u * sc; v = v * sc;
            }
        }
        qt_put_uv<FIX>(FX, UO, VO, r0, W.vs, u, v, uc, vc);
        us = uc; uc = un; vs = vc; vc = vn;
    }
    return acc;
}

struct QtGather { double f00, f01, f10, f11, wr0, wr1, wc0, wc1; bool nan_coord; };
__device__ __forceinline__ QtGather qt_gather_issue(const QdGeom& G, const QdTabs& T, const QdTailArgs& P, int gi, int j, double u, double v) {
    const QdBilin b = qt_departure(G, gi, j, u, v, P.sub_dt, P.a * qd_sload(T.cos05, gi), qd_sload(T.ocn_igx, gi), P);
    const size_t r0 = (size_t)b.l0 * G.nlon, r1 = (size_t)b.l1 * G.nlon;
    QtGather q;
    q.f00 = P.Ts[r0 + b.c0]; q.f01 = P.Ts[r0 + b.c1]; q.f10 = P.Ts[r1 + b.c0]; q.f11 = P.Ts[r1 + b.c1];
    q.wr0 = b.wr0; q.wr1 = b.wr1; q.wc0 = b.wc0; q.wc1 = b.wc1; q.nan_coord = b.nan_coord;
    return q;
}
__device__ __forceinline__ double qt_gather_use(const QtGather& q) {
    double t = 0.0;
    t += q.f00 * q.wr0 * q.wc0;
    t += q.f01 * q.wr0 * q.wc1;
    t += q.f10 * q.wr1 * q.wc0;
    t += q.f11 * q.wr1 * q.wc1;
    return q.nan_coord ? 0.0 : t;
}

__device__ __forceinline__ double qt_lap_win(const double (&w)[5], const QdTabs& T, int i, int n, double dphi, double dlam, double a) {
    const double cc = w[2], e = qd_east(cc), wst = qd_west(cc);
    if (i >= 2 && i <= n - 3) {
        const double Gb = qd_sload(T.lapA[1], i + 1) * (w[4] - cc);
        const double Ga = qd_sload(T.lapA[1], i - 1) * (cc - w[0]);
        const double d2 = (e - 2.0 * cc) + wst;
        return qd_sload(T.lapP[1], i) * (Gb - Ga) + qd_sload(T.lapQ[1], i) * d2;
    }
    const double* __restrict__ cosf = T.cos05;
    auto dphi_of = [&](int r) -> double {
        if (r == 0) return (w[1 - i + 2] - w[0 - i + 2]) / dphi;
        if (r == n - 1) return (w[n - 1 - i + 2] - w[n - 2 - i + 2]) / dphi;
        return (w[r + 1 - i + 2] - w[r - 1 - i + 2]) / (2.0 * dphi);
    };
    int ra, rb; double den;
    if (i == 0) { ra = 0; rb = 1; den = dphi; }
    else if (i == n - 1) { ra = n - 2; rb = n - 1; den = dphi; }
    else { ra = i - 1; rb = i + 1; den = 2.0 * dphi; }
// ... 753 lines not shown
```

qingdai_amd/csrc/qd_physics.hip:

```cpp
#include "qd_internal.h"
#include "qd_band.h"
#include "qd_pointwise.h"
#include "qd_device.h"
#include "qd_saf.h"
#include "qd_fluxes.h"
#include "qd_blockred.h"
QdColP qd_make_colp(const qd_ctx* c, double dt);


__global__ void __launch_bounds__(QD_BLOCK)
k_precip_raw(QdGeom G, QdTabs T, const double* __restrict__ u, const double* __restrict__ v,
             const double* __restrict__ pcond, double a, double dlat, double dlon, double D_crit, double beta,
             const double* __restrict__ scale_p, const unsigned long long* __restrict__ sel_state,
             double* __restrict__ praw, double* __restrict__ pos_out, double* __restrict__ partial,
             const double* __restrict__ orog) {
    __shared__ double sm[2][QD_BLOCK / 64];
    const int i = G.row0 + blockIdx.y;
    const size_t b = (size_t)qd_lrow(G, i) * G.nlon;
    const double w = T.warea[i];
    const bool anypos = sel_state[0] > 0;
    const double scale = qd_max(*scale_p, 1e-12);
    double s_num = 0.0, s_den = 0.0;
    for (int j = threadIdx.x; j < G.nlon; j += QD_BLOCK) {
        const double div = qd_divvort_point(G, T, u, v, i, j, a, dlat, dlon, 0);
        const double pos = qd_max(0.0, -(div - D_crit));
        const double F_div = anypos ? qd_clip(pos / scale, 0.0, 5.0) : 0.0;
        const double Pq = qd_max(0.0, pcond[b + j]);
        const double F_orog = orog ? qd_clip(orog[b + j], 1.0, 3.0) : 1.0;
        const double F = (1.0 + beta * F_div) * F_orog;
        const double pr = Pq * F;
        praw[b + j] = pr;
        pos_out[b + j] = pos;
        s_num += Pq * w;
        s_den += pr * w;
    }
    s_num = qd_wave_sum(s_num); s_den = qd_wave_sum(s_den);
    const int lane = threadIdx.x & 63, wv = threadIdx.x >> 6;
    if (lane == 0) { sm[0][wv] = s_num; sm[1][wv] = s_den; }
    __syncthreads();
    if (threadIdx.x == 0) {
        for (int k = 1; k < QD_BLOCK / 64; ++k) { s_num += sm[0][k]; s_den += sm[1][k]; }
        partial[blockIdx.y] = s_num;
        partial[gridDim.y + blockIdx.y] = s_den;
    }
}

__global__ void __launch_bounds__(QD_BLOCK)
k_orog_factor(QdGeom G, QdTabs T, const double* __restrict__ elev, const double* __restrict__ u, const double* __restrict__ v,
              double a, double dlat, double dlon, double k_orog, double cap, double* __restrict__ out) {
    const QdTile tl = qd_tile();
    const int j = tl.seg * QD_BLOCK + threadIdx.x;
    if (j >= G.nlon) return;
    const int i = G.row0 + tl.row, n = G.nlat;
    const size_t b = (size_t)qd_lrow(G, i) * G.nlon;
    const int jp = qd_wrapc(j + 1, G.nlon), jm = qd_wrapc(j - 1, G.nlon);
    const double dx = a * T.cos6[i] * dlon, dy = a * dlat;
    const double dHdx = (elev[b + jp] - elev[b + jm]) / (2.0 * dx);
// ... 34 lines not shown
    out[o] = s ? in[o] * (*s) : k * in[o];
}

__global__ void __launch_bounds__(QD_BLOCK)
k_precip_blend(QdGeom G, const double* __restrict__ P, const double* __restrict__ Pdyn, const double* __restrict__ sc,
               double* __restrict__ out) {
    const QdTile tl = qd_tile();
    const int j = tl.seg * QD_BLOCK + threadIdx.x;
    if (j >= G.nlon) return;
    const size_t o = (size_t)qd_lrow(G, G.row0 + tl.row) * G.nlon + j;
    const double al = sc[1];
    double p = P[o];
    if (al != 0.0) p = (1.0 - al) * p + al * Pdyn[o];
    out[o] = qd_max(p, 0.0);
}

__global__ void __launch_bounds__(QD_BLOCK)
k_cloud_from_p(QdGeom G, const double* __restrict__ precip, const double* __restrict__ pref, double cmax,
               double* __restrict__ out) {
    const QdTile tl = qd_tile();
    const int j = tl.seg * QD_BLOCK + threadIdx.x;
    if (j >= G.nlon) return;
    const size_t o = (size_t)qd_lrow(G, G.row0 + tl.row) * G.nlon + j;
    out[o] = cmax * qd_tanh(precip[o] / (*pref + 1e-12));
}


__device__ __forceinline__ double qd_tanh01(double x) {
    double t = 0.0;
    if (!(x <= 0.0)) t = qd_tanh_nonneg(x);
    return qd_clip(t, 0.0, 1.0);
}

__device__ __forceinline__ double qd_cloud_source_cell(const QdGeom& G, const QdTabs& T, const double* __restrict__ u, const double* __restrict__ v,
                                                       const double* __restrict__ Ts, double a, double dlat, double dlon, int i, int j);

__global__ void __launch_bounds__(QD_BLOCK)
k_cloud_source(QdGeom G, QdTabs T, const double* __restrict__ u, const double* __restrict__ v,
               const double* __restrict__ Ts, double a, double dlat, double dlon, double* __restrict__ out) {
    const QdTile tl = qd_tile();
    const int j = tl.seg * QD_BLOCK + threadIdx.x;
    if (j >= G.nlon) return;
    const int i = G.row0 + tl.row;
    out[(size_t)qd_lrow(G, i) * G.nlon + j] = qd_cloud_source_cell(G, T, u, v, Ts, a, dlat, dlon, i, j);
}

__global__ void __launch_bounds__(QD_BLOCK)
k_cloud_fromp_source(QdGeom G, QdTabs T, const double* __restrict__ precip, const double* __restrict__ pref, double cmax,
                     const double* __restrict__ u, const double* __restrict__ v, const double* __restrict__ Ts, double a, double dlat,
                     double dlon, double* __restrict__ cfp, double* __restrict__ src) {
    const QdTile tl = qd_tile();
    const int j = tl.seg * QD_BLOCK + threadIdx.x;
    if (j >= G.nlon) return;
    const int i = G.row0 + tl.row;
    const size_t o = (size_t)qd_lrow(G, i) * G.nlon + j;
    cfp[o] = cmax * qd_tanh(precip[o] / (*pref + 1e-12));
    src[o] = qd_cloud_source_cell(G, T, u, v, Ts, a, dlat, dlon, i, j);
}

__device__ __forceinline__ double qd_cloud_source_cell(const QdGeom& G, const QdTabs& T, const double* __restrict__ u, const double* __restrict__ v,
                                                       const double* __restrict__ Ts, double a, double dlat, double dlon, int i, int j) {
    const size_t b = (size_t)qd_lrow(G, i) * G.nlon;
    const size_t o = b + j;
    const double T0 = Ts[o];
    double src = 0.0;
    src = src + 0.5 * qd_tanh01((T0 - 285.0) / 12.0);
    const double vort = qd_divvort_point(G, T, v, u, i, j, a, dlat, dlon, 1);
    const double rel = vort / (T.fcor[i] + 1e-12);
    src = src + 0.4 * qd_tanh01((rel - 0.5) / 2.0);
    const double dx = dlon * a * T.cos6[i];
    const double dy = dlat * a;
    const int jp = qd_wrapc(j + 1, G.nlon), jm = qd_wrapc(j - 1, G.nlon);
    const double gx = (Ts[b + jp] - Ts[b + jm]) / (2 * dx);
    const double gy = (Ts[(size_t)qd_lrow(G, i + 1) * G.nlon + j] - Ts[(size_t)qd_lrow(G, i - 1) * G.nlon + j]) / (2 * dy);
    const double tadv = -(u[o] * gx + v[o] * gy);
    src = src + 0.3 * qd_tanh01(fabs(tadv) / 2e-5);
    return src;
}

struct QdBlendP { double w_mem, w_p, w_src, tend, c_floor; };

__global__ void __launch_bounds__(QD_BLOCK)
k_cloud_blend(QdGeom G, QdBlendP P, const double* __restrict__ cfp, const double* __restrict__ src,
              double* __restrict__ cloud) {
    const QdTile tl = qd_tile();
    const int j = tl.seg * QD_BLOCK + threadIdx.x;
    if (j >= G.nlon) return;
    const size_t o = (size_t)qd_lrow(G, G.row0 + tl.row) * G.nlon + j;
    const double c0 = cloud[o], cp = cfp[o];
    const double tendency = src[o] * P.tend;
    double c = (P.w_mem * c0 + P.w_p * cp + P.w_src * qd_clip(c0 + tendency, 0.0, 1.0));
    if (P.c_floor > 0.0) c = qd_max(c, qd_clip(P.c_floor * cp, 0.0, 1.0));
    cloud[o] = qd_clip(c, 0.0, 1.0);
}

__global__ void __launch_bounds__(QD_BLOCK)
k_cloud_albedo(QdGeom G, QdAlbP P, const double* __restrict__ adv, double* __restrict__ cloud,
               const double* __restrict__ cloud_eff, const double* __restrict__ hice,
               const double* __restrict__ base, const uint8_t* __restrict__ land, const double* __restrict__ csnow,
               const double* __restrict__ eco_alpha, const double* __restrict__ glacier, const double* __restrict__ banded,
               const double* __restrict__ water, double* __restrict__ albedo) {
    const QdTile tl = qd_tile();
    const int j = tl.seg * QD_BLOCK + threadIdx.x;
    if (j >= G.nlon) return;
    const size_t o = (size_t)qd_lrow(G, G.row0 + tl.row) * G.nlon + j;
    double c = cloud[o];
    if (P.do_adv) { c = qd_clip((1.0 - P.alpha) * c + P.alpha * adv[o], 0.0, 1.0); cloud[o] = c; }
    const int landv = land[o];
    const double cs = (P.snow && landv == 1) ? csnow[o] : 0.0;
    const double gl = (P.eco && landv == 1) ? glacier[o] : 0.0;
    albedo[o] = qd_albedo_cell(P, o, c, cloud_eff, hice, base, landv, cs, gl, eco_alpha, banded, water);
}

__global__ void k_precip_scalars_post(const double* raw, double wsum, double pq_min, double p_blend, int use_fb, double* out) {
    if (threadIdx.x == 0 && blockIdx.x == 0) {
        const double a = raw[0], b = raw[1];
        const double den = b + 1e-20;
        out[0] = den > 0 ? a / den : 1.0;
        const double pq_mean = a / (wsum + 1e-15);
        out[1] = (use_fb && pq_mean < pq_min) ? p_blend : 0.0;
    }
}
__global__ void __launch_bounds__(QD_BLOCK)
k_precip_rawsums(const double* __restrict__ partial, int n, double* __restrict__ out) {
    __shared__ double sm[2][QD_BLOCK / 64];
    double a = 0.0, b = 0.0;
    for (int k = threadIdx.x; k < n; k += QD_BLOCK) { a += partial[k]; b += partial[n + k]; }
    a = qd_wave_sum(a); b = qd_wave_sum(b);
    const int lane = threadIdx.x & 63, wv = threadIdx.x >> 6;
    if (lane == 0) { sm[0][wv] = a; sm[1][wv] = b; }
    __syncthreads();
    if (threadIdx.x == 0) {
        for (int k = 1; k < QD_BLOCK / 64; ++k) { a += sm[0][k]; b += sm[1][k]; }
        out[0] = a; out[1] = b;
    }
}

__global__ void __launch_bounds__(QD_BLOCK)
k_snow_provisional(QdGeom G, QdTabs T, QdSnowP P, const double* __restrict__ precip, const double* __restrict__ h,
                   const double* __restrict__ S_snow, const double* __restrict__ elev, const uint8_t* __restrict__ land,
                   double* __restrict__ P_rain, double* __restrict__ S_next, double* __restrict__ melt,
                   double* __restrict__ C_snow, double* __restrict__ glacier) {
    const QdTile tl = qd_tile();
    const int j = tl.seg * QD_BLOCK + threadIdx.x;
    if (j >= G.nlon) return;
    const int i = G.row0 + tl.row;
    const size_t o = (size_t)qd_lrow(G, i) * G.nlon + j;
    const QdSnowOut r = qd_snow_cell(T, P, i, land[o] == 1, h[o], S_snow[o], elev[o], precip[o]);
    P_rain[o] = r.Pr; S_next[o] = r.Sn; melt[o] = r.melt; C_snow[o] = r.Cs; glacier[o] = r.gl;
}

__global__ void __launch_bounds__(QD_BLOCK)
k_snow_albedo_forcing(QdSafArgs K) {
    const QdTile tl = qd_tile();
    const int j = tl.seg * QD_BLOCK + threadIdx.x;
    if (j >= K.G.nlon) return;
    const int i = K.G.row0 + tl.row;
    qd_saf_cell(K, i, j, (size_t)qd_lrow(K.G, i) * K.G.nlon + j, true);
}
int qd_saf_launch(qd_ctx* c, const QdSafArgs& K) {
    hipLaunchKernelGGL(k_snow_albedo_forcing, qd_grid2d(K.G), dim3(QD_BLOCK), 0, c->stream, K);
    return 0;
}
void qd_saf_drop(qd_ctx* c) { delete (QdSafArgs*)c->saf_pending; c->saf_pending = nullptr; }
int qd_saf_flush(qd_ctx* c) {
    if (!c->saf_pending) return 0;
    QdSafArgs* K = (QdSafArgs*)c->saf_pending;
    c->saf_pending = nullptr;
    const int r = qd_saf_launch(c, *K);
    delete K;
    return r;
}

struct QdBucketP { double dt, tau_s, cap; };

__global__ void __launch_bounds__(QD_BLOCK)
k_hydro_commit(QdGeom G, QdBucketP P, const double* __restrict__ P_rain, const double* __restrict__ melt,
               const double* __restrict__ glacier, const double* __restrict__ E, const uint8_t* __restrict__ land,
               const double* __restrict__ S_next, double* __restrict__ S_snow, double* __restrict__ W_land,
               double* __restrict__ runoff) {
    const QdTile tl = qd_tile();
    const int j = tl.seg * QD_BLOCK + threadIdx.x;
    if (j >= G.nlon) return;
    const size_t o = (size_t)qd_lrow(G, G.row0 + tl.row) * G.nlon + j;
    const double L = land[o] == 1 ? 1.0 : 0.0;
    const double gl = glacier[o];
    const double non_gl = (L != 0.0 && gl == 0.0) ? 1.0 : 0.0;
    const double ml = melt[o];
    const double P_in = (P_rain[o] * L + ml) * non_gl;
    const double E_l = (E[o] * L) * non_gl;
    const double W = W_land[o];
// ... 46 lines not shown
    if (pcond_side && qd_pcond_median_side(c, dt)) return -1;
    const bool pcond_pair = part != 1 && !pcond_side && c->want_pcond_ahead && c->med_pair && c->hist_b && c->geo.full && p.cloud_couple &&
                            !isset(p.pcond_ref) && !(isset(p.pref) && p.pref != 0.0);
    if (part != 2) {
        QdScope sc(c, "phys_precip");
        int m = qd_plan(c, {QD_IN(F[QD_F_U], 1), QD_IN(F[QD_F_V], 1), QD_IN(F[QD_F_PCOND], 0)});
        if (m < 0) return -1;
        qd_launch_divvort(c, F[QD_F_U], F[QD_F_V], tmp, 0, m);
        if (qd_median_positive_dev(c, tmp, 1e-12, QD_S_PSCALE, 1, p.D_crit, 2)) return -1;
        const double* orog = nullptr;
        if (p.orog_enable && c->has_elevation) {
            double*& of = c->scratch[8];
            const int mo = qd_plan(c, {QD_IN(F[QD_F_U], 0), QD_IN(F[QD_F_V], 0), QD_IN(F[QD_F_ELEVATION], 1)});
            if (mo < 0) return -1;
            QD_ROWS(c, mo, G, hipLaunchKernelGGL(k_orog_factor, qd_grid2d(G), blk, 0, c->stream, G, c->tabs, F[QD_F_ELEVATION],
                                                 F[QD_F_U], F[QD_F_V], p.a, c->dlat, c->dlon, p.orog_k, 2.0, of));
            qd_mark(c, {of}, mo);
            const int mb = qd_plan(c, {QD_IN(of, R1)});
            if (mb < 0) return -1;
            if (qd_gaussian_swap(c, of, tmp, 1.0, 0, mb)) return -1;
            orog = of;
            m = qd_plan(c, {QD_IN(F[QD_F_U], 1), QD_IN(F[QD_F_V], 1), QD_IN(F[QD_F_PCOND], 0), QD_IN(c->scratch[8], 0)});
            if (m < 0) return -1;
        }
        if (band && m > 0) {
            QdSegs S = qd_segments(c, m);
            const int own0 = c->own_row0, own1 = c->own_row0 + c->own_nrows;
            for (int k = 0; k < S.n; ++k) {
                const QdGeom& G = S.g[k];
                auto run = [&](int r0, int r1) {
                    if (r1 <= r0) return;
                    QdGeom g2 = G; g2.row0 = r0; g2.nrows = r1 - r0;
                    hipLaunchKernelGGL(k_precip_raw, dim3(1, g2.nrows), blk, 0, c->stream, g2, c->tabs, F[QD_F_U], F[QD_F_V],
                                       F[QD_F_PCOND], p.a, c->dlat, c->dlon, p.D_crit, p.p_betadiv, c->dscal + QD_S_PSCALE,
                                       c->dcount, praw, pos, rp + (size_t)2 * G0.lrows(), orog);
                };
                const int a0 = G.row0, a1 = G.row0 + G.nrows;
                if (a1 <= own0 || a0 >= own1) run(a0, a1);
                else { run(a0, std::max(a0, own0)); run(std::min(a1, own1), a1); }
            }
        }
        hipLaunchKernelGGL(k_precip_raw, dim3(1, Gown.nrows), blk, 0, c->stream, Gown, c->tabs, F[QD_F_U], F[QD_F_V],
                           F[QD_F_PCOND], p.a, c->dlat, c->dlon, p.D_crit, p.p_betadiv, c->dscal + QD_S_PSCALE, c->dcount, praw,
                           pos, rp, orog);
        qd_mark(c, {praw, pos}, m);
        if (band && qd_peer_hooks(c)) {
            QdPeerHook H; H.pre = 2; H.partial = rp; H.n = Gown.nrows;
            H.post = 1; H.wsum = c->wsum_all; H.pq_min = p.pq_min; H.p_blend = p.p_blend; H.use_fb = p.p_hybrid_fallback; H.out = c->dscal + QD_S_RENORM;
            c->allreduces++;
            if (qd_peer_allreduce_hooked(c, c->dscal + QD_S_TMP0, 2, 0, H)) return -1;
        } else if (band) {
            hipLaunchKernelGGL(k_precip_rawsums, dim3(1), blk, 0, c->stream, rp, Gown.nrows, c->dscal + QD_S_TMP0);
            if (qd_allreduce_f64(c, c->dscal + QD_S_TMP0, 2, 0)) return -1;
            hipLaunchKernelGGL(k_precip_scalars_post, dim3(1), dim3(64), 0, c->stream, c->dscal + QD_S_TMP0, c->wsum_all, p.pq_min,
                               p.p_blend, p.p_hybrid_fallback, c->dscal + QD_S_RENORM);
        } else {
            hipLaunchKernelGGL(k_precip_scalars, dim3(1), blk, 0, c->stream, rp, Gown.nrows, c->wsum_all, p.pq_min,
                               p.p_blend, p.p_hybrid_fallback, c->dscal + QD_S_RENORM);
        }
        if (qd_gauss_pair_ok(c, 1.0)) {
            const int mg = qd_plan(c, {QD_IN(praw, R1), QD_IN(pos, R1)});
            if (mg < 0) return -1;
            if (qd_gaussian_pair(c, praw, pos, 1.0, 0, c->dscal + QD_S_RENORM, 1.0, p.k_precip, c->dscal + QD_S_RENORM, 1, nullptr,
                                 nullptr, nullptr, F[QD_F_PRECIP], mg)) return -1;
            qd_mark(c, {F[QD_F_PRECIP]}, mg);
        } else if (qd_gauss_can_fuse(c, 1.0)) {
            const int mg = qd_plan(c, {QD_IN(praw, R1), QD_IN(pos, R1)});
            if (mg < 0) return -1;
            if (qd_gaussian_swap(c, praw, tmp, 1.0, 0, mg, 0, c->dscal + QD_S_RENORM)) return -1;
            if (qd_gaussian(c, pos, pdyn, nullptr, 1.0, 0, mg, 0, nullptr, p.k_precip)) return -1;
            QD_ROWS(c, mg, G, hipLaunchKernelGGL(k_precip_blend, qd_grid2d(G), blk, 0, c->stream, G, praw, pdyn,
                                                 c->dscal + QD_S_RENORM, F[QD_F_PRECIP]));
            qd_mark(c, {F[QD_F_PRECIP]}, mg);
        } else {
        QD_ROWS(c, m, G, hipLaunchKernelGGL(k_scale_field, qd_grid2d(G), blk, 0, c->stream, G, praw, c->dscal + QD_S_RENORM, 0.0, praw));
        QD_ROWS(c, m, G, hipLaunchKernelGGL(k_scale_field, qd_grid2d(G), blk, 0, c->stream, G, pos, (const double*)nullptr,
// ... 3 lines not shown
        if (mg < 0) return -1;
        if (qd_gaussian_swap(c, praw, tmp, 1.0, 0, mg)) return -1;
        if (qd_gaussian_swap(c, pdyn, tmp, 1.0, 0, mg)) return -1;
        QD_ROWS(c, mg, G, hipLaunchKernelGGL(k_precip_blend, qd_grid2d(G), blk, 0, c->stream, G, praw, pdyn,
                                             c->dscal + QD_S_RENORM, F[QD_F_PRECIP]));
        qd_mark(c, {F[QD_F_PRECIP]}, mg);
        }
    }
    if (part == 1) return 0;
    {
        QdScope sc(c, "phys_cloud");
        if (isset(p.pref) && p.pref != 0.0) {
            hipMemcpyAsync(c->dscal + QD_S_MED_OUT, &p.pref, sizeof(double), hipMemcpyHostToDevice, c->stream);
        } else if (pcond_pair) {
            if (c->med_fold && qd_median_pair_ready(c, 3, 1)) {
                if (qd_median_pair_pcond_dev(c, F[QD_F_PRECIP], 1e-6, QD_S_MED_OUT, 0, 0.0, 3, qd_make_colp(c, dt), 1e-6, QD_S_PREF, 1)) return -1;
            } else {
                if (qd_pcond_phase1(c, dt)) return -1;
                if (qd_median_pair_dev(c, F[QD_F_PRECIP], 1e-6, QD_S_MED_OUT, 0, 0.0, 3, F[QD_F_PCOND], 1e-6, QD_S_PREF, 0, 0.0, 1)) return -1;
            }
            c->pcond_ahead = 3;
        } else {
            if (qd_median_positive_dev(c, F[QD_F_PRECIP], 1e-6, QD_S_MED_OUT, 0, 0.0, 3)) return -1;
        }
        double*& cfp = F[QD_F_CLOUD_FROM_P];
        double*& src = F[QD_F_CLOUD_SRC];
        int m = qd_plan(c, {QD_IN(F[QD_F_PRECIP], 0)});
        if (m < 0) return -1;
        int ms = qd_plan(c, {QD_IN(F[QD_F_U], 1), QD_IN(F[QD_F_V], 1), QD_IN(F[QD_F_TS], 1)});
        if (ms < 0) return -1;
        if (c->merge_pointwise) {
            m = ms = std::min(m, ms);
            QD_ROWS(c, m, G, hipLaunchKernelGGL(k_cloud_fromp_source, qd_grid2d(G), blk, 0, c->stream, G, c->tabs, F[QD_F_PRECIP],
                                                c->dscal + QD_S_MED_OUT, p.cmax, F[QD_F_U], F[QD_F_V], F[QD_F_TS], p.a, c->dlat, c->dlon, cfp, src));
        } else {
        QD_ROWS(c, m, G, hipLaunchKernelGGL(k_cloud_from_p, qd_grid2d(G), blk, 0, c->stream, G, F[QD_F_PRECIP],
                                            c->dscal + QD_S_MED_OUT, p.cmax, cfp));
        QD_ROWS(c, ms, G, hipLaunchKernelGGL(k_cloud_source, qd_grid2d(G), blk, 0, c->stream, G, c->tabs, F[QD_F_U], F[QD_F_V],
                                             F[QD_F_TS], p.a, c->dlat, c->dlon, src));
        }
        qd_mark(c, {cfp}, m);
        qd_mark(c, {src}, ms);
        const int mg = qd_plan(c, {QD_IN(cfp, R1), QD_IN(src, R1), QD_IN(F[QD_F_CLOUD], 0)});
        if (mg < 0) return -1;
        double wm = p.w_mem, wp = p.w_p, ws = p.w_src, wsum = wm + wp + ws;
        if (wsum <= 0) { wm = 0.5; wp = 0.4; ws = 0.1; wsum = 1.0; }
        wm /= wsum; wp /= wsum; ws /= wsum;
        QdBlendP B{wm, wp, ws, dt / (6 * 3600), p.cloud_from_p_floor};
        if (qd_gauss_pair_ok(c, 1.0)) {
            double*& oa = c->scratch[6]; double*& ob = c->scratch[7];
            const double b5[5] = {B.w_mem, B.w_p, B.w_src, B.tend, B.c_floor};
            if (qd_gaussian_pair(c, cfp, src, 1.0, 0, nullptr, 1.0, 1.0, nullptr, 2, b5, oa, ob, F[QD_F_CLOUD], mg)) return -1;
            std::swap(cfp, oa); std::swap(src, ob);
            qd_mark(c, {cfp, src, F[QD_F_CLOUD]}, mg);
        } else {
        if (qd_gaussian_swap(c, cfp, tmp, 1.0, 0, mg, 1)) return -1;
        if (qd_gaussian_swap(c, src, tmp, 1.0, 0, mg, 1)) return -1;
        QD_ROWS(c, mg, G, hipLaunchKernelGGL(k_cloud_blend, qd_grid2d(G), blk, 0, c->stream, G, B, cfp, src, F[QD_F_CLOUD]));
        qd_mark(c, {F[QD_F_CLOUD]}, mg);
        }
    }
    {
        QdScope sc(c, "phys_albedo");
        double*& adv = c->scratch[7];
        int m;
        if (p.cloud_advect) {
            const int ma = qd_plan(c, {QD_IN(F[QD_F_CLOUD], Rc), QD_IN(F[QD_F_U], 0), QD_IN(F[QD_F_V], 0)});
            if (ma < 0) return -1;
            qd_launch_advect(c, F[QD_F_U], F[QD_F_V], c->tabs.cos05, dt, F[QD_F_CLOUD], adv, nullptr, nullptr, 1.0, 0, ma);
            if (p.cloud_smooth_sigma > 0.0) {
                const int rs = qd_gauss_radius(p.cloud_smooth_sigma);
                const int mb = qd_plan(c, {QD_IN(adv, rs)});
                if (mb < 0) return -1;
                if (qd_gaussian_swap(c, adv, tmp, p.cloud_smooth_sigma, 1, mb)) return -1;
            }
            m = qd_plan(c, {QD_IN(adv, 0), QD_IN(F[QD_F_CLOUD], 0), QD_IN(F[QD_F_HICE], 0)});
        } else {
            m = qd_plan(c, {QD_IN(F[QD_F_CLOUD], 0), QD_IN(F[QD_F_HICE], 0)});
        }
        if (m < 0) return -1;
        if (c->cloud_eff_valid) { const int me = qd_plan(c, {QD_IN(F[QD_F_CLOUD_EFF], 0)}); if (me < 0) return -1; m = std::min(m, me); }
        const QdEco& E = c->eco;
        QdAlbP A{p.cloud_adv_alpha, std::max(1e-6, p.hice_ref), p.alpha_ice, p.alpha_cloud, p.alpha_water, p.snow_albedo_fresh, E.p.w_lai,
                 p.cloud_advect ? 1 : 0, p.use_topo_albedo ? 1 : 0, p.swe_enable ? 1 : 0,
                 (E.configured && E.p.albedo_couple && E.alpha_valid) ? 1 : 0, (E.configured && E.p.bands_couple && E.banded_valid) ? 1 : 0,
                 ((E.configured && E.p.water_couple && E.water_valid) || qd_phyto_daily_couples(c)) ? 1 : 0,
                 (E.configured && E.p.map_f32) ? 1 : 0};
        if (A.eco) { const int me = qd_plan(c, {QD_IN(F[QD_F_ECO_ALPHA], 0)}); if (me < 0) return -1; m = std::min(m, me); }
        if (A.banded) { const int me = qd_plan(c, {QD_IN(F[QD_F_ECO_ALPHA_BANDED], 0)}); if (me < 0) return -1; m = std::min(m, me); }
        if (A.water) { const int me = qd_plan(c, {QD_IN(F[QD_F_WATER_ALPHA], 0)}); if (me < 0) return -1; m = std::min(m, me); }
        {
            const int msn = qd_plan(c, {QD_IN(F[QD_F_PRECIP], 0), QD_IN(F[QD_F_H], 0), QD_IN(F[QD_F_S_SNOW], 0), QD_IN(F[QD_F_ELEVATION], 0)});
            if (msn < 0) return -1;
            QdSnowP S;
            S.dt = dt; S.ga = 9.81 / 1004.0; S.rho_snow_safe = std::max(p.rho_snow, 1e-6); S.polar_lat = p.polar_lat_thresh;
            S.ice_max = p.polar_ice_thick_max_m; S.elev_max = p.land_elev_max_m; S.gamma = p.lapse_k_kpm; S.lapse = p.lapse_enable;
            S.t_thresh = p.snow_thresh_K; S.dT = std::max(1e-6, p.snow_t_band_K); S.mode = p.snow_melt_mode;
            S.ddf_s = p.snow_ddf_mm_per_k_day / 86400.0; S.tref = p.snow_melt_tref_K; S.rate_s = p.snow_melt_rate_mm_day / 86400.0;
            S.swe_max = (p.swe_max_mm == p.swe_max_mm && p.swe_max_mm > 0) ? p.swe_max_mm : -1.0;
            S.swe_ref_safe = std::max(1e-6, p.swe_ref_mm); S.gl_frac = p.glacier_frac; S.gl_swe = p.glacier_swe_mm; S.swe = p.swe_enable;
            if (fc) {
                const QdForcingP Fo{QdStar{fc->sa[0], std::sin(fc->sa[1]), std::cos(fc->sa[1]), fc->sa[2]},
                                    QdStar{fc->sb[0], std::sin(fc->sb[1]), std::cos(fc->sb[1]), fc->sb[2]}, fc->theta, 5.670374e-8, 1};
                const int mm = std::min(m, msn);
                QdSafArgs K;
                K.T = c->tabs; K.S = S; K.A = A; K.Fo = Fo;
                K.precip = F[QD_F_PRECIP]; K.h = F[QD_F_H]; K.S_snow = F[QD_F_S_SNOW]; K.elev = F[QD_F_ELEVATION]; K.land = c->land;
                K.P_rain = F[QD_F_P_RAIN]; K.S_next = F[QD_F_S_SNOW_NEXT]; K.melt = F[QD_F_MELT]; K.C_snow = F[QD_F_C_SNOW]; K.glacier = F[QD_F_GLACIER];
                K.adv = adv; K.cloud = F[QD_F_CLOUD]; K.cloud_eff = c->cloud_eff_valid ? F[QD_F_CLOUD_EFF] : (const double*)nullptr;
                K.hice = F[QD_F_HICE]; K.base = F[QD_F_BASE_ALBEDO]; K.eco_alpha = F[QD_F_ECO_ALPHA]; K.banded = F[QD_F_ECO_ALPHA_BANDED];
                K.water = F[QD_F_WATER_ALPHA]; K.albedo = F[QD_F_ALBEDO]; K.isrA = F[QD_F_ISR_A]; K.isrB = F[QD_F_ISR_B]; K.isr = F[QD_F_ISR];
                K.Teq = F[QD_F_TEQ]; K.eday = c->eco.eday_dt > 0 ? F[QD_F_ECO_EDAY] : (double*)nullptr; K.eday_dt = c->eco.eday_dt;
                K.write_diag = c->diag_write;
                K.col1 = (c->want_pcond_ahead && !pcond_side && !pcond_pair && c->geo.full && p.cloud_couple && !isset(p.pcond_ref)) ? 1 : 0;
                K.P = qd_make_colp(c, dt);
                K.u = F[QD_F_U]; K.v = F[QD_F_V]; K.Ts = F[QD_F_TS]; K.q = F[QD_F_Q]; K.Pcond = F[QD_F_PCOND];
                if (pcond_pair && c->merge_saf && c->pcond_ahead == 3 && c->geo.full) {
                    K.G = c->geo;
                    delete (QdSafArgs*)c->saf_pending;
                    c->saf_pending = new QdSafArgs(K);
                } else
                QD_ROWS(c, mm, G, K.G = G; hipLaunchKernelGGL(k_snow_albedo_forcing, qd_grid2d(G), blk, 0, c->stream, K));
                c->eco.eday_dt = 0;
                if (K.col1) c->pcond_ahead = 1;
                qd_mark(c, {F[QD_F_P_RAIN], F[QD_F_S_SNOW_NEXT], F[QD_F_MELT], F[QD_F_C_SNOW], F[QD_F_GLACIER]}, mm);
                qd_mark(c, {F[QD_F_CLOUD], F[QD_F_ALBEDO], F[QD_F_ISR_A], F[QD_F_ISR_B], F[QD_F_ISR], F[QD_F_TEQ]}, mm);
                return 0;
            }
            QD_ROWS(c, msn, G, hipLaunchKernelGGL(k_snow_provisional, qd_grid2d(G), blk, 0, c->stream, G, c->tabs, S, F[QD_F_PRECIP],
                                                  F[QD_F_H], F[QD_F_S_SNOW], F[QD_F_ELEVATION], c->land, F[QD_F_P_RAIN],
                                                  F[QD_F_S_SNOW_NEXT], F[QD_F_MELT], F[QD_F_C_SNOW], F[QD_F_GLACIER]));
            qd_mark(c, {F[QD_F_P_RAIN], F[QD_F_S_SNOW_NEXT], F[QD_F_MELT], F[QD_F_C_SNOW], F[QD_F_GLACIER]}, msn);
            m = std::min(m, msn);
// ... 66 lines not shown
```

qingdai_amd/csrc/qd_phyto.hip:

```cpp
#include "qd_internal.h"
#include "qd_device.h"
#include <vector>

__global__ void __launch_bounds__(QD_BLOCK)
k_phyto_advect(QdGeom G, const double* __restrict__ cos05, double dt, double a, double dlat, double dlon,
               const double* __restrict__ uo, const double* __restrict__ vo, const double* __restrict__ Cst,
               double* __restrict__ Tst, size_t stride, double alpha, int scrub) {
    const QdTile tl = qd_tile();
    const int j = tl.seg * QD_BLOCK + threadIdx.x;
    if (j >= G.nlon) return;
    const int i = G.row0 + tl.row;
    const size_t o = (size_t)qd_lrow(G, i) * G.nlon + j;
    const double* __restrict__ C = Cst + (size_t)tl.fld * stride;
    const QdBilin b = qd_departure(G, i, j, uo[o], vo[o], dt, a, cos05[i], dlat, dlon);
    const double adv = qd_gather(C, G, b);
    const double v = (1.0 - alpha) * C[o] + alpha * adv;
    Tst[(size_t)tl.fld * stride + o] = scrub ? qd_nn(v) : v;
}

__global__ void __launch_bounds__(QD_BLOCK)
k_phyto_diffuse(QdGeom G, const double* __restrict__ cos05, double dlat, double dlon, double a, double dtK, int has_diff,
                const double* __restrict__ Tst, double* __restrict__ Cst, size_t stride, const uint8_t* __restrict__ land) {
    const QdTile tl = qd_tile();
    const int j = tl.seg * QD_BLOCK + threadIdx.x;
    if (j >= G.nlon) return;
    const int i = G.row0 + tl.row;
    const size_t o = (size_t)qd_lrow(G, i) * G.nlon + j;
    const double* __restrict__ T = Tst + (size_t)tl.fld * stride;
    double v = T[o];
    if (has_diff) v = v + dtK * qd_lap_point<true>(T, G, cos05, i, j, dlat, dlon, a);
    v = (v >= 0.0 || v != v) ? v : 0.0;
    Cst[(size_t)tl.fld * stride + o] = land[o] != 0 ? 0.0 : v;
}

__global__ void __launch_bounds__(QD_BLOCK)
k_phyto_polar(QdGeom G, const uint8_t* __restrict__ land, double* __restrict__ Cst, size_t stride) {
    __shared__ double sm[2][QD_BLOCK / 64];
    const int i = blockIdx.x == 1 ? G.nlat - 1 : 0;
    if (i < G.row0 || i >= G.row0 + G.nrows) return;
    const size_t b = (size_t)qd_lrow(G, i) * G.nlon;
    double* __restrict__ C = Cst + (size_t)blockIdx.y * stride;
    double cnt = 0.0, s = 0.0;
    for (int j = threadIdx.x; j < G.nlon; j += QD_BLOCK)
        if (land[b + j] == 0) { cnt += 1.0; s += C[b + j]; }
#pragma unroll
    for (int o = 32; o > 0; o >>= 1) { cnt += __shfl_down(cnt, o, 64); s += __shfl_down(s, o, 64); }
    if ((threadIdx.x & 63) == 0) { sm[0][threadIdx.x >> 6] = cnt; sm[1][threadIdx.x >> 6] = s; }
// ... 49 lines not shown
    hipSetDevice(c->desc.device);
    if (qd_band_copy_in(c, c->phyto.cur[s], host, sizeof(double))) return qd_fail(c, "qd_phyto_upload: copy failed");
    qd_mark(c, {c->phyto.cur[s]}, c->geo.halo);
    QD_HIP(c, hipStreamSynchronize(c->stream));
    return 0;
}

extern "C" int qd_phyto_download(qd_handle c, int s, double* host) {
    if (!c || !host) return -1;
    if (s < 0 || s >= c->phyto.S) return qd_fail(c, "qd_phyto_download: no such species");
    hipSetDevice(c->desc.device);
    const QdGeom& G = c->geo;
    const size_t rowb = (size_t)G.nlon * sizeof(double);
    QD_HIP(c, hipMemcpyAsync((char*)host + (size_t)G.row0 * rowb, (const char*)c->phyto.cur[s] + (size_t)G.halo * rowb,
                             rowb * G.nrows, hipMemcpyDeviceToHost, c->stream));
    QD_HIP(c, hipStreamSynchronize(c->stream));
    return 0;
}

int qd_phyto_step_impl(qd_ctx* c, double dt) {
    QdPhyto& P = c->phyto;
    if (P.S == 0 || dt <= 0.0) return 0;
    QdScope sc(c, "phyto");
    double** F = c->f;
    const qd_params& p = c->p;
    const dim3 blk(QD_BLOCK);
    const int has_diff = P.K_h > 0.0 ? 1 : 0;
    const int Ro = qd_adv_reach(c, dt, 4.0);
    std::vector<QdUse> in;
    for (int s = 0; s < P.S; ++s) in.push_back(QD_IN(P.cur[s], Ro));
    in.push_back(QD_IN(F[QD_F_UO], 0)); in.push_back(QD_IN(F[QD_F_VO], 0));
    const int m1 = qd_plan(c, in.data(), (int)in.size());
    if (m1 < 0) return -1;
    QD_ROWS(c, m1, G, hipLaunchKernelGGL(k_phyto_advect, qd_grid2d(G, P.S), blk, 0, c->stream, G, c->tabs.cos05, dt, p.a, c->dlat,
                                         c->dlon, F[QD_F_UO], F[QD_F_VO], P.stack[0], P.stack[1], P.stride, P.alpha, has_diff));
    for (int s = 0; s < P.S; ++s) qd_mark(c, {P.tmp[s]}, m1);
    in.clear();
    for (int s = 0; s < P.S; ++s) in.push_back(QD_IN(P.tmp[s], has_diff ? 2 : 0));
    const int m2 = qd_plan(c, in.data(), (int)in.size());
    if (m2 < 0) return -1;
    QD_ROWS(c, m2, G, hipLaunchKernelGGL(k_phyto_diffuse, qd_grid2d(G, P.S), blk, 0, c->stream, G, c->tabs.cos05, c->dlat, c->dlon,
                                         p.a, dt * P.K_h, has_diff, P.stack[1], P.stack[0], P.stride, c->land));
    const QdGeom Gown = qd_segments(c, 0).g[0];
    hipLaunchKernelGGL(k_phyto_polar, dim3(2, P.S), blk, 0, c->stream, Gown, c->land, P.stack[0], P.stride);
    for (int s = 0; s < P.S; ++s) qd_mark(c, {P.cur[s]}, 0);
    return 0;
}

extern "C" int qd_phyto_advect_diffuse(qd_handle c, double dt) {
    if (!c) return -1;
    if (c->phyto.S == 0) return qd_fail(c, "qd_phyto_advect_diffuse: no tracers (qd_phyto_configure first)");
    hipSetDevice(c->desc.device);
    if (int rc = qd_phyto_step_impl(c, dt)) return rc;
    return qd_launch_check(c, "qd_phyto_advect_diffuse");
}
```

qingdai_amd/csrc/qd_pointwise.h:

```cpp
#pragma once
#include "qd_internal.h"

struct QdSnowP {
    double dt, ga, rho_snow_safe, polar_lat, ice_max, elev_max, gamma, t_thresh, dT, ddf_s, tref, rate_s, swe_max, swe_ref_safe,
           gl_frac, gl_swe;
    int lapse, mode, swe;
};
struct QdSnowOut { double Pr, Sn, melt, Cs, gl; };

__device__ __forceinline__ QdSnowOut qd_snow_cell(const QdTabs& T, const QdSnowP& P, int i, bool is_land, double hval, double S0, double elev,
                                                  double Pf) {
    QdSnowOut r;
    const double T_a = 288.0 + P.ga * hval;
    const double h_snow = is_land ? qd_max(S0, 0.0) / P.rho_snow_safe : 0.0;
    const bool polar = fabs(T.lat_deg[i]) >= P.polar_lat;
    const double h_ice_eff = polar ? qd_min(h_snow, P.ice_max) : h_snow;
    const double H_eff = qd_min(elev + h_ice_eff, P.elev_max);
    const double T_hat = P.lapse ? T_a - P.gamma * (H_eff / 1000.0) : T_a;
    double f_snow = 1.0 / (1.0 + exp((T_hat - P.t_thresh) / P.dT));
    f_snow = qd_clip(f_snow, 0.0, 1.0);
    const double Ps = qd_nn(f_snow * Pf);
    const double Pr = qd_nn((1.0 - f_snow) * Pf);
    r.Pr = Pr;
    if (!P.swe) { r.Sn = S0; r.melt = 0.0; r.Cs = 0.0; r.gl = 0.0; return r; }
    const double Ps_land = Ps * (is_land ? 1.0 : 0.0);
    double melt_flux;
    if (P.mode == 0) melt_flux = P.ddf_s * qd_max(T_hat - P.tref, 0.0);
    else melt_flux = (T_hat >= P.t_thresh) ? P.rate_s : 0.0;
    const double actual = qd_min(qd_max(S0, 0.0), melt_flux * P.dt);
    double Sn = S0 + Ps_land * P.dt - actual;
    if (P.swe_max > 0.0) Sn = qd_min(Sn, P.swe_max);
    Sn = qd_max(0.0, Sn);
    const double melt_out = (P.dt > 0) ? actual / P.dt : 0.0;
    const double Cs = qd_clip(1.0 - exp(-qd_max(Sn, 0.0) / P.swe_ref_safe), 0.0, 1.0);
    Sn = qd_nn(Sn);
    const bool gl = is_land && ((Cs >= P.gl_frac) || (Sn >= P.gl_swe));
    const double Pr_gl = (Pr * (is_land ? 1.0 : 0.0)) * (gl ? 1.0 : 0.0);
    if (Pr_gl != 0.0) Sn = Sn + Pr_gl * P.dt;
    r.Sn = Sn; r.melt = qd_nn(melt_out); r.Cs = Cs; r.gl = gl ? 1.0 : 0.0;
    return r;
}

struct QdAlbP { double alpha, hice_ref_safe, alpha_ice, alpha_cloud, alpha_water, alpha_snow, w_lai; int do_adv, use_topo, snow, eco, banded, water, eco_f32; };

__device__ __forceinline__ double qd_albedo_cell(const QdAlbP& P, size_t o, double c, const double* __restrict__ cloud_eff,
                                                 const double* __restrict__ hice, const double* __restrict__ base, int landv, double cs, double gl,
                                                 const double* __restrict__ eco_alpha, const double* __restrict__ banded,
                                                 const double* __restrict__ water) {
    const double crad = cloud_eff ? cloud_eff[o] : c;
    const double C = qd_clip(crad, 0.0, 1.0);
    const double ice_frac = 1.0 - exp(-qd_max(hice[o], 0.0) / P.hice_ref_safe);
    double fi = qd_clip(ice_frac, 0.0, 1.0);
    fi = fi * ((landv == 0) ? 1.0 : 0.0);
    double b0 = P.use_topo ? base[o] : P.alpha_water;
    if (P.eco && landv == 1 && gl == 0.0) {
        const double ae = P.eco_f32 ? (double)reinterpret_cast<const float*>(eco_alpha)[o] : eco_alpha[o];
        if (fabs(ae) <= DBL_MAX) b0 = (1.0 - P.w_lai) * b0 + P.w_lai * ae;
    }
    if (P.banded && landv == 1) {
        const double ab = P.eco_f32 ? (double)reinterpret_cast<const float*>(banded)[o] : banded[o];
        if (fabs(ab) <= DBL_MAX) b0 = qd_clip(ab, 0.0, 1.0);
    }
    if (P.water && landv == 0) {
        const double aw = water[o];
        if (fabs(aw) <= DBL_MAX) b0 = qd_clip(aw, 0.0, 1.0);
    }
    if (P.snow && landv == 1) b0 = qd_clip((1.0 - cs) * b0 + cs * P.alpha_snow, 0.0, 1.0);
    const double surf = b0 * (1.0 - fi) + P.alpha_ice * fi;
    return qd_clip(surf * (1.0 - C) + P.alpha_cloud * C, 0.0, 1.0);
}

struct QdStar { double flux, sin_d, cos_d, alpha; };
struct QdForcingP { QdStar A, B; double theta, sigma; int with_teq; };

__device__ __forceinline__ void qd_star_insolation(const QdTabs& T, const QdStar& A, const QdStar& B, double theta, int i, int j,
                                                   double& a_, double& b_) {
    const double sl = T.sin_raw[i], cl = T.cos_raw[i], lon = T.lon_rad[j];
    const double hA = theta + lon - A.alpha;
    const double hB = theta + lon - B.alpha;
    const double czA = qd_max(0.0, sl * A.sin_d + cl * A.cos_d * cos(hA));
    const double czB = qd_max(0.0, sl * B.sin_d + cl * B.cos_d * cos(hB));
    a_ = A.flux * czA; b_ = B.flux * czB;
}

struct QdForcingOut { double tot, teq; };
__device__ __forceinline__ QdForcingOut qd_forcing_cell(const QdTabs& T, const QdForcingP& P, int i, int j, size_t o, double alb,
                                                        double* __restrict__ isrA, double* __restrict__ isrB, double* __restrict__ isr,
                                                        double* __restrict__ Teq, double* __restrict__ eday, double eday_dt) {
    double a_, b_;
    qd_star_insolation(T, P.A, P.B, P.theta, i, j, a_, b_);
    const double tot = a_ + b_;
    if (isrA) { isrA[o] = a_; isrB[o] = b_; }
    isr[o] = tot;
    if (eday) eday[o] += qd_nn(tot) * eday_dt;
    QdForcingOut r{tot, 0.0};
    if (P.with_teq) {
        double num = tot * (1 - alb);
        if (num < 0) num = 0;
        r.teq = sqrt(sqrt(num / P.sigma));
        if (Teq) Teq[o] = r.teq;
    }
    return r;
}
```

qingdai_amd/csrc/qd_saf.h:

```cpp
#pragma once
#include "qd_internal.h"
#include "qd_pointwise.h"
#include "qd_fluxes.h"

struct QdSafArgs {
    QdGeom G; QdTabs T; QdSnowP S; QdAlbP A; QdForcingP Fo;
    const double *precip, *h, *S_snow, *elev; const uint8_t* land;
    double *P_rain, *S_next, *melt, *C_snow, *glacier;
    const double* adv; double* cloud; const double *cloud_eff, *hice, *base, *eco_alpha, *banded, *water;
    double *albedo, *isrA, *isrB, *isr, *Teq, *eday; double eday_dt;
    int write_diag, col1; QdColP P; const double *u, *v, *Ts, *q; double* Pcond;
};
struct QdSafOut { double cloud, albedo, isr, teq; };

__device__ __forceinline__ QdSafOut qd_saf_cell(const QdSafArgs& K, int i, int j, size_t o, bool store_teq) {
    const int landv = K.land[o];
    const double hh = K.h[o];
    if (K.col1) {
        const double hi = K.hice[o];
        const double qsat_air = qd_qsat(288.0 + K.P.ga * hh, K.P.p0);
        K.Pcond[o] = qd_humidity_column(K.P, K.u[o], K.v[o], K.Ts[o], K.q[o], qsat_air, landv == 1, hi).Pc;
    }
    const QdSnowOut r = qd_snow_cell(K.T, K.S, i, landv == 1, hh, K.S_snow[o], K.elev[o], K.precip[o]);
    if (K.write_diag) { K.P_rain[o] = r.Pr; K.S_next[o] = r.Sn; K.melt[o] = r.melt; K.C_snow[o] = r.Cs; K.glacier[o] = r.gl; }
    double c = K.cloud[o];
    if (K.A.do_adv) { c = qd_clip((1.0 - K.A.alpha) * c + K.A.alpha * K.adv[o], 0.0, 1.0); K.cloud[o] = c; }
    const double alb = qd_albedo_cell(K.A, o, c, K.cloud_eff, K.hice, K.base, landv, r.Cs, r.gl, K.eco_alpha, K.banded, K.water);
    K.albedo[o] = alb;
    const QdForcingOut f = qd_forcing_cell(K.T, K.Fo, i, j, o, alb, K.write_diag ? K.isrA : nullptr, K.isrB, K.isr, store_teq ? K.Teq : nullptr,
                                           K.eday, K.eday_dt);
    return QdSafOut{c, alb, f.tot, f.teq};
}
```

qingdai_amd/csrc/qd_stencil.hip:

```cpp
#include "qd_internal.h"
#include "qd_device.h"
#include "qd_wave.h"
#include <cstdlib>

__global__ void __launch_bounds__(QD_BLOCK)
k_laplacian(QdGeom G, QdFieldList fl, const double* __restrict__ cosf, double dphi, double dlam, double a) {
    const QdTile tl = qd_tile();
    const int j = tl.seg * QD_BLOCK + threadIdx.x;
    if (j >= G.nlon) return;
    const int i = G.row0 + tl.row;
    const int f = tl.fld;
    const size_t o = (size_t)qd_lrow(G, i) * G.nlon + j;
    fl.out[f][o] = qd_lap_point<true>(fl.in[f], G, cosf, i, j, dphi, dlam, a);
}

__global__ void __launch_bounds__(QD_BLOCK)
k_hyper_apply(QdGeom G, QdFieldList fl, const double* __restrict__ cosf, double dphi, double dlam, double a,
              double sub_dt) {
    const QdTile tl = qd_tile();
    const int j = tl.seg * QD_BLOCK + threadIdx.x;
    if (j >= G.nlon) return;
    const int i = G.row0 + tl.row;
    const int f = tl.fld;
    const size_t o = (size_t)qd_lrow(G, i) * G.nlon + j;
// ... 162 lines not shown
        }
    }
}

static int qd_shapiro_rows(const qd_ctx* c) { return c->tune.shapiro_r > 0 ? c->tune.shapiro_r : 12; }

int qd_shapiro_fields(qd_ctx* c, double** fields, int n, int npass, int m_out) {
    if (npass < 1) npass = 1;
    QdFieldList a; a.n = n;
    if (npass <= 3 && c->geo.nlon >= 64 && c->shapiro_stream) {
        for (int k = 0; k < n; ++k) { a.in[k] = fields[k]; a.out[k] = qd_scratch(c, k); a.aux[k] = nullptr; a.k4row[k] = nullptr; a.k4s[k] = 0; }
        const int R = qd_shapiro_rows(c), W = 64 - 2 * npass, ntc = (c->geo.nlon + W - 1) / W;
        QD_ROWS(c, m_out, G, {
            const int ns = ((G.nrows + R - 1) / R) * ntc;
            const dim3 grid((ns + QD_SH_WAVES - 1) / QD_SH_WAVES, n), blk(64 * QD_SH_WAVES);
            if (npass == 1) hipLaunchKernelGGL(k_shapiro_stream<1>, grid, blk, 0, c->stream, G, a, 1, R, ntc, ns);
            else if (npass == 2) hipLaunchKernelGGL(k_shapiro_stream<2>, grid, blk, 0, c->stream, G, a, 1, R, ntc, ns);
            else hipLaunchKernelGGL(k_shapiro_stream<3>, grid, blk, 0, c->stream, G, a, 1, R, ntc, ns);
        });
        for (int k = 0; k < n; ++k) { double* t = fields[k]; fields[k] = c->scratch[k]; c->scratch[k] = t; qd_mark(c, {fields[k]}, m_out); }
        return 0;
    }
    for (int p = 0; p < npass; ++p) {
        for (int k = 0; k < n; ++k) { a.in[k] = fields[k]; a.out[k] = qd_scratch(c, k); a.aux[k] = nullptr; a.k4row[k] = nullptr; a.k4s[k] = 0; }
        const int m = m_out + (npass - 1 - p);
        qd_launch_shapiro_pass(c, a, p == 0, m);
        for (int k = 0; k < n; ++k) { double* t = fields[k]; fields[k] = c->scratch[k]; c->scratch[k] = t; qd_mark(c, {fields[k]}, m); }
    }
    return 0;
}

__global__ void __launch_bounds__(QD_BLOCK)
k_advect(QdGeom G, const double* __restrict__ u, const double* __restrict__ v, const double* __restrict__ cosl,
         double dt, double a, double dlat, double dlon,
         const double* __restrict__ f0, double* __restrict__ o0,
         const double* __restrict__ f1, double* __restrict__ o1, double alpha, int clipq) {
    const QdTile tl = qd_tile();
    const int j = tl.seg * QD_BLOCK + threadIdx.x;
    if (j >= G.nlon) return;
    const int i = G.row0 + tl.row;
    const size_t o = (size_t)qd_lrow(G, i) * G.nlon + j;
    const QdBilin b = qd_departure(G, i, j, u[o], v[o], dt, a, cosl[i], dlat, dlon);
    const bool blend = (alpha != 1.0);
    {
        const double adv = qd_gather(f0, G, b);
        o0[o] = blend ? (1.0 - alpha) * f0[o] + alpha * adv : adv;
    }
    if (f1) {
        const double adv = qd_gather(f1, G, b);
        double x = blend ? (1.0 - alpha) * f1[o] + alpha * adv : adv;
        if (clipq) x = qd_clip(qd_nn(x), 0.0, 0.5);
        o1[o] = x;
    }
}

void qd_launch_advect(qd_ctx* c, const double* u, const double* v, const double* coslat, double dt,
                      const double* f0, double* o0, const double* f1, double* o1, double alpha, int clipq, int m) {
    QD_ROWS(c, m, G, hipLaunchKernelGGL(k_advect, qd_grid2d(G), dim3(QD_BLOCK), 0, c->stream, G, u, v, coslat, dt,
                                        c->p.a, c->dlat, c->dlon, f0, o0, f1, o1, alpha, clipq));
    qd_mark(c, {o0, o1}, m);
}

__global__ void __launch_bounds__(QD_BLOCK)
k_divvort(QdGeom G, QdTabs T, const double* __restrict__ u, const double* __restrict__ v, double* __restrict__ out,
          double a, double dlat, double dlon, int vort) {
    const QdTile tl = qd_tile();
    const int j = tl.seg * QD_BLOCK + threadIdx.x;
    if (j >= G.nlon) return;
    const int i = G.row0 + tl.row;
    out[(size_t)qd_lrow(G, i) * G.nlon + j] =
        vort ? qd_divvort_point(G, T, v, u, i, j, a, dlat, dlon, 1) : qd_divvort_point(G, T, u, v, i, j, a, dlat, dlon, 0);
}

void qd_launch_divvort(qd_ctx* c, const double* u, const double* v, double* out, int vort, int m) {
    QD_ROWS(c, m, G, hipLaunchKernelGGL(k_divvort, qd_grid2d(G), dim3(QD_BLOCK), 0, c->stream, G, c->tabs, u, v, out,
                                        c->p.a, c->dlat, c->dlon, vort));
    qd_mark(c, {out}, m);
}

#define QD_GAUSS_MAXR 24
struct QdGaussW { double w[QD_GAUSS_MAXR + 1]; int r; };

__device__ __forceinline__ int qd_ext(int i, int n, int mode_wrap) {
    if (mode_wrap) { i %= n; return i < 0 ? i + n : i; }
    const int p = 2 * n;
    i %= p; if (i < 0) i += p;
    return i >= n ? p - 1 - i : i;
}

__global__ void __launch_bounds__(QD_BLOCK)
k_gauss_axis(QdGeom G, const double* __restrict__ in, double* __restrict__ out, QdGaussW W, int axis, int mode_wrap) {
    const QdTile tl = qd_tile();
    const int j = tl.seg * QD_BLOCK + threadIdx.x;
    if (j >= G.nlon) return;
    const int i = G.row0 + tl.row;
    const size_t o = (size_t)qd_lrow(G, i) * G.nlon + j;
    double tmp = in[o] * W.w[0];
    if (axis == 0) {
        for (int k = W.r; k >= 1; --k) {
            const double lo = in[(size_t)qd_lrow(G, qd_ext(i - k, G.nlat, mode_wrap)) * G.nlon + j];
            const double hi = in[(size_t)qd_lrow(G, qd_ext(i + k, G.nlat, mode_wrap)) * G.nlon + j];
            tmp += (lo + hi) * W.w[k];
        }
    } else {
        const size_t b = (size_t)qd_lrow(G, i) * G.nlon;
        for (int k = W.r; k >= 1; --k) {
            const double lo = in[b + qd_ext(j - k, G.nlon, mode_wrap)];
            const double hi = in[b + qd_ext(j + k, G.nlon, mode_wrap)];
            tmp += (lo + hi) * W.w[k];
// ... 353 lines not shown
```

Before: 4.963 planet-days/s.

## Replace per-cell divisions with precomputed reciprocals and share hour-angle cosines

Divisions by constants across the column physics, advection departure points and div/vort stencils become multiplications by host-precomputed reciprocals, with an FMA correction step (qd_div_rc) intended to keep results bit-identical to true division. The fused SAF+column kernel now computes the per-longitude hour-angle cosines once per block into shared memory, processes 4 rows per block, and passes the ice fraction through so the exp is not evaluated twice. New reciprocal tables and a QdMet parameter struct are added. The aim is to cut f64 division and transcendental cost; the tradeoffs are more kernel arguments, register pressure and a changed block shape.

```diff
diff --git a/qingdai_amd/csrc/qd_api.hip b/qingdai_amd/csrc/qd_api.hip
--- a/qingdai_amd/csrc/qd_api.hip
+++ b/qingdai_amd/csrc/qd_api.hip
@@ -120,7 +120,7 @@
             c->tabs.lapK[k] = dev_table(c, K4);
             c->h_lapK[k] = K4;
         }
-        std::vector<double> cu(nlat), cv(nlat), px(nlat), igx(nlat), ia6(nlat);
+        std::vector<double> cu(nlat), cv(nlat), px(nlat), igx(nlat), ia6(nlat), i2dx(nlat), ifc(nlat);
         for (int i = 0; i < nlat; ++i) {
             const double f = fc[i];
             const double sgn = f >= 0.0 ? 1.0 : -1.0;
@@ -130,10 +130,13 @@
             px[i] = -(p.g / (a * c6[i]));
             igx[i] = 1.0 / (a * c05[i]);
             ia6[i] = 1 / (a * c6[i]);
+            i2dx[i] = 1.0 / (2 * (dlam * a * c6[i]));
+            ifc[i] = 1.0 / (fc[i] + 1e-12);
         }
         c->tabs.mom_cu = dev_table(c, cu); c->tabs.mom_cv = dev_table(c, cv); c->tabs.mom_px = dev_table(c, px);
         c->tabs.ocn_igx = dev_table(c, igx);
         c->tabs.inv_acos6 = dev_table(c, ia6);
+        c->tabs.inv_2dx6 = dev_table(c, i2dx); c->tabs.inv_fcor = dev_table(c, ifc);
     }
     std::vector<double> lr(nlon), sl(nlon), cl(nlon);
     for (int j = 0; j < nlon; ++j) { lr[j] = lon[j] * d2r; sl[j] = std::sin(lr[j]); cl[j] = std::cos(lr[j]); }
diff --git a/qingdai_amd/csrc/qd_atmos.hip b/qingdai_amd/csrc/qd_atmos.hip
--- a/qingdai_amd/csrc/qd_atmos.hip
+++ b/qingdai_amd/csrc/qd_atmos.hip
@@ -5,6 +5,7 @@
 
 #include "qd_fluxes.h"
 #include "qd_fused.h"
+#include <cstring>
 
 struct QdColPtrs {
     const double *u, *v, *Teq, *isr, *albedo, *csmap;
@@ -15,7 +16,7 @@
     unsigned long long* npos;
 };
 
-struct QdColIn { double cloud, isr, albedo, teq; };
+struct QdColIn { double cloud, isr, albedo, teq, ice_frac; int has_ice_frac; };
 
 template <int PHASE, bool HAS_ALB>
 __device__ __forceinline__ void qd_column_cell(const QdColP& P, const QdColPtrs& A, size_t o, const QdColIn* IN, int i, int nlat) {
@@ -36,7 +37,7 @@
     const double Teq = IN ? IN->teq : A.Teq[o];
     const double olr_old = P.sigma * qd_pow4(Ts);
     const double net_old = P.sigma * qd_pow4(Teq) + P.gfs * qd_pow4(T_a) - olr_old;
-    const double Ts_newton = Ts + (net_old / P.c_sfc_safe) * P.dt;
+    const double Ts_newton = Ts + qd_div_rc(net_old, P.c_sfc_safe, P.r_c_sfc_safe) * P.dt;
 
     double Ts_new, h_new = h;
     QdFlux F;
@@ -51,25 +52,26 @@
             cloud_eff = qd_clip(cloud + P.k_q * rh_excess + P.k_p * p_term, 0.0, 1.0);
         } else cloud_eff = cloud;
         A.cloud_eff[o] = cloud_eff;
-        F = qd_surface_fluxes(P, IN ? IN->isr : A.isr[o], IN ? IN->albedo : A.albedo[o], cloud_eff, Ts, T_a, u, v, land, hice);
+        F = qd_surface_fluxes(P, IN ? IN->isr : A.isr[o], IN ? IN->albedo : A.albedo[o], cloud_eff, Ts, T_a, u, v, land, hice,
+                              IN && IN->has_ice_frac, IN ? IN->ice_frac : 0.0);
         double Ts_energy;
         if (P.seaice) {
             double Q = F.SW_sfc - F.LW_sfc - F.SH - LH;
             double Tn = Ts, hi = hice;
             if (hi > 0.0 && ocean && Q > 0.0) {
-                const double dh_melt = (Q * P.dt) / P.rhoiLf;
+                const double dh_melt = qd_div_rc(Q * P.dt, P.rhoiLf, P.r_rhoiLf);
                 const double dh_cap = qd_min(dh_melt, hi);
                 hi -= dh_cap;
-                Q = Q - (dh_cap * P.rho_i * P.L_f) / P.dt;
+                Q = Q - qd_div_rc(dh_cap * P.rho_i * P.L_f, P.dt, P.r_dt);
             }
             if (ocean && Q < 0.0 && Tn <= (P.t_freeze + 0.5)) {
-                hi += (-Q * P.dt) / P.rhoiLf;
+                hi += qd_div_rc(-Q * P.dt, P.rhoiLf, P.r_rhoiLf);
                 Q = 0.0;
                 Tn = qd_min(Tn, P.t_freeze);
             }
-            double Cs = land ? P.Cs_land : (hi > 0.0 ? P.Cs_ice : P.Cs_ocean);
-            Cs = (isfinite(Cs) && Cs > 1e3) ? Cs : 1e3;
-            Tn = Tn + (Q / Cs) * P.dt;
+            const double Cs = land ? P.Cs_land_safe : (hi > 0.0 ? P.Cs_ice_safe : P.Cs_ocean_safe);
+            const double r_Cs = land ? P.r_Cs_land_safe : (hi > 0.0 ? P.r_Cs_ice_safe : P.r_Cs_ocean_safe);
+            Tn = Tn + qd_div_rc(Q, Cs, r_Cs) * P.dt;
             if ((i == 0 && P.fix_s) || (i == nlat - 1 && P.fix_n)) {
                 if (ocean && Q < 0.0 && Tn > P.t_freeze) Tn = P.t_freeze;
             }
@@ -79,10 +81,10 @@
             { const double hn_ = qd_nn(hi); if (__double_as_longlong(hn_) != __double_as_longlong(hice)) A.hice[o] = hn_; }
         } else {
             const double net = F.SW_sfc - F.LW_sfc - F.SH - LH;
-            double Cs;
-            if (P.has_csmap) { const double cm = A.csmap[o]; Cs = (isfinite(cm) && cm > 1e3) ? cm : 1e3; }
-            else Cs = P.c_sfc_safe;
-            Ts_energy = qd_nn(qd_max(P.t_floor, Ts + (net / Cs) * P.dt));
+            double qc;
+            if (P.has_csmap) { const double cm = A.csmap[o]; qc = net / ((isfinite(cm) && cm > 1e3) ? cm : 1e3); }
+            else qc = qd_div_rc(net, P.c_sfc_safe, P.r_c_sfc_safe);
+            Ts_energy = qd_nn(qd_max(P.t_floor, Ts + qc * P.dt));
         }
         if (P.write_diag) A.olr[o] = F.OLR;
         Ts_new = (1.0 - P.w_energy) * Ts_newton + P.w_energy * Ts_energy;
@@ -93,10 +95,10 @@
     A.Ts[o] = Ts_new;
 
     const double h_eq = P.h_eq_fac * Teq;
-    h_new = h + ((h_eq - h) / P.tau_rad) * P.dt;
+    h_new = h + qd_div_rc(h_eq - h, P.tau_rad, P.r_tau_rad) * P.dt;
     if (HAS_ALB && P.atm_couple) {
         const double F_atm = F.SW_atm + F.LW_atm + F.SH + LHrel;
-        h_new = qd_nn(h_new + P.atm_w * (F_atm / P.atm_denom) * P.dt);
+        h_new = qd_nn(h_new + P.atm_w * qd_div_rc(F_atm, P.atm_denom, P.r_atm_denom) * P.dt);
     }
     A.h[o] = h_new;
 }
@@ -111,15 +113,21 @@
     qd_column_cell<PHASE, HAS_ALB>(P, A, (size_t)qd_lrow(G, i) * G.nlon + j, nullptr, i, G.nlat);
 }
 
-__global__ void __launch_bounds__(QD_BLOCK)
-k_saf_column2(QdSafArgs K, QdColP P, QdColPtrs A) {
-    const QdTile tl = qd_tile();
-    const int j = tl.seg * QD_BLOCK + threadIdx.x;
-    if (j >= K.G.nlon) return;
-    const int i = K.G.row0 + tl.row;
+#define QD_SAF_R 4
+__global__ void __launch_bounds__(64 * QD_SAF_R)
+k_saf_column2(QdSafArgs K, QdColP P, QdColPtrs A, int share_ice) {
+    __shared__ double hc[2][64];
+    const QdTile tl = qd_tile();
+    const int lane = threadIdx.x & 63, w = threadIdx.x >> 6;
+    const int j = tl.seg * 64 + lane;
+    const int i = K.G.row0 + tl.row * QD_SAF_R + w;
+    if (w < 2) hc[w][lane] = qd_hour_cos1(K.T, w == 0 ? K.Fo.A.alpha : K.Fo.B.alpha, K.Fo.theta, j < K.G.nlon ? j : K.G.nlon - 1);
+    __syncthreads();
+    if (j >= K.G.nlon || i >= K.G.row0 + K.G.nrows) return;
+    const QdHourCos H{hc[0][lane], hc[1][lane]};
     const size_t o = (size_t)qd_lrow(K.G, i) * K.G.nlon + j;
-    const QdSafOut s = qd_saf_cell(K, i, j, o, K.write_diag != 0);
-    const QdColIn in{s.cloud, s.isr, s.albedo, s.teq};
+    const QdSafOut s = qd_saf_cell(K, H, i, o, K.write_diag != 0);
+    const QdColIn in{s.cloud, s.isr, s.albedo, s.teq, s.ice_frac, share_ice};
     qd_column_cell<2, true>(P, A, o, &in, i, K.G.nlat);
 }
 
@@ -168,7 +176,7 @@
 }
 
 __global__ void __launch_bounds__(QD_BLOCK)
-k_final(QdGeom G, const double* __restrict__ cosl, double dt, double a, double dlat, double dlon,
+k_final(QdGeom G, const double* __restrict__ cosl, const double* __restrict__ r_acosl, double dt, QdMet M,
         double* __restrict__ u, double* __restrict__ v, double* __restrict__ h, double* __restrict__ Ts,
         double* __restrict__ q, const double* __restrict__ cloud_in, double* __restrict__ cloud_out,
         double decay, double dfac) {
@@ -178,7 +186,7 @@
     const int i = G.row0 + tl.row;
     const size_t o = (size_t)qd_lrow(G, i) * G.nlon + j;
     const double uu = u[o], vv = v[o];
-    const QdBilin b = qd_departure(G, i, j, uu, vv, dt, a, cosl[i], dlat, dlon);
+    const QdBilin b = qd_departure(G, i, j, uu, vv, dt, M.a * cosl[i], r_acosl[i], M);
     double c = qd_gather(cloud_in, G, b);
     c = c * decay;
     cloud_out[o] = qd_nn(c * dfac);
@@ -269,6 +277,7 @@
     P.couple = p.cloud_couple; P.lw_v2 = p.lw_v2; P.gh_lock = p.gh_lock; P.seaice = p.seaice_enabled;
     P.fix_s = p.polar_freeze_fix_s; P.fix_n = p.polar_freeze_fix_n; P.has_csmap = p.has_csmap;
     P.write_diag = c->diag_write;
+    qd_colp_recips(P);
     return P;
 }
 
@@ -348,7 +357,9 @@
             if (c->saf_pending && ahead == 3 && c->geo.full) {
                 QdSafArgs* K = (QdSafArgs*)c->saf_pending;
                 c->saf_pending = nullptr;
-                hipLaunchKernelGGL(k_saf_column2, qd_grid2d(K->G), blk, 0, c->stream, *K, P, A);
+                const int share_ice = (std::memcmp(&K->A.hice_ref_safe, &P.hice_ref_safe, sizeof(double)) == 0 && K->hice == A.hice) ? 1 : 0;
+                hipLaunchKernelGGL(k_saf_column2, dim3((K->G.nlon + 63) / 64, (K->G.nrows + QD_SAF_R - 1) / QD_SAF_R),
+                                   dim3(64 * QD_SAF_R), 0, c->stream, *K, P, A, share_ice);
                 delete K;
             } else {
                 if (qd_saf_flush(c)) return -1;
@@ -456,7 +467,7 @@
             return 0;
         }
         double* oc = qd_scratch(c, 0);
-        QD_ROWS(c, m, G, hipLaunchKernelGGL(k_final, qd_grid2d(G), blk, 0, c->stream, G, c->tabs.cos6, dt, p.a, c->dlat, c->dlon,
+        QD_ROWS(c, m, G, hipLaunchKernelGGL(k_final, qd_grid2d(G), blk, 0, c->stream, G, c->tabs.cos6, c->tabs.inv_acos6, dt, qd_met(p.a, c->dlat, c->dlon),
                                             F[QD_F_U], F[QD_F_V], F[QD_F_H], F[QD_F_TS], F[QD_F_Q], F[QD_F_CLOUD], oc, decay,
                                             p.diff_factor));
         qd_mark(c, {F[QD_F_U], F[QD_F_V], F[QD_F_H], F[QD_F_TS], F[QD_F_Q], oc}, m);
diff --git a/qingdai_amd/csrc/qd_device.h b/qingdai_amd/csrc/qd_device.h
--- a/qingdai_amd/csrc/qd_device.h
+++ b/qingdai_amd/csrc/qd_device.h
@@ -60,11 +60,11 @@
 struct QdBilin { int l0, l1, c0, c1; double wr0, wr1, wc0, wc1; bool nan_coord; };
 
 __device__ __forceinline__ QdBilin qd_departure(const QdGeom& G, int gi, int j, double u, double v, double dt,
-                                                double a, double cosl, double dlat, double dlon) {
-    const double dl = u * dt / (a * cosl);
-    const double dp = v * dt / a;
-    const double dx = dl / dlon;
-    const double dy = dp / dlat;
+                                                double acos, double r_acos, const QdMet& M) {
+    const double dl = qd_div_rc(u * dt, acos, r_acos);
+    const double dp = qd_div_rc(v * dt, M.a, M.r_a);
+    const double dx = qd_div_rc(dl, M.dlon, M.r_dlon);
+    const double dy = qd_div_rc(dp, M.dlat, M.r_dlat);
     double r = qd_fold((double)gi - dy, G.nlat);
     double cc = qd_fold((double)j - dx, G.nlon);
     const bool nan_coord = (dx != dx) || (dy != dy);
@@ -94,17 +94,16 @@
 
 
 __device__ __forceinline__ double qd_divvort_point(const QdGeom& G, const QdTabs& T, const double* __restrict__ p,
-                                                   const double* __restrict__ q, int i, int j, double a,
-                                                   double dlat, double dlon, int vort) {
+                                                   const double* __restrict__ q, int i, int j, const QdMet& M, int vort) {
     const size_t b = (size_t)qd_lrow(G, i) * G.nlon;
     const int jp = qd_wrapc(j + 1, G.nlon), jm = qd_wrapc(j - 1, G.nlon);
-    const double dp = (p[b + jp] - p[b + jm]) / (2 * dlon);
+    const double dp = qd_div_rc(p[b + jp] - p[b + jm], M.dlon2, M.r_dlon2);
     double dq = 0.0;
     if (i != 0 && i != G.nlat - 1) {
         const double qn = q[(size_t)qd_lrow(G, i + 1) * G.nlon + j] * T.cos_raw[i + 1];
         const double qs = q[(size_t)qd_lrow(G, i - 1) * G.nlon + j] * T.cos_raw[i - 1];
-        dq = (qn - qs) / (2 * dlat);
+        dq = qd_div_rc(qn - qs, M.dlat2, M.r_dlat2);
     }
-    const double pre = 1 / (a * T.cos6[i]);
+    const double pre = T.inv_acos6[i];
     return vort ? pre * (dp - dq) : pre * (dp + dq);
 }
diff --git a/qingdai_amd/csrc/qd_fluxes.h b/qingdai_amd/csrc/qd_fluxes.h
--- a/qingdai_amd/csrc/qd_fluxes.h
+++ b/qingdai_amd/csrc/qd_fluxes.h
@@ -1,5 +1,6 @@
 #pragma once
 #include "qd_internal.h"
+#include "qd_pointwise.h"
 
 #define QD_EPSILON 0.622
 
@@ -15,7 +16,16 @@
     double w_energy, h_eq_fac, tau_rad, atm_denom, atm_w;
     int couple, lw_v2, gh_lock, seaice, fix_s, fix_n, has_csmap, atm_couple;
     int write_diag = 1;
+    double r_M_col, r_tau_c, r_c_sfc_safe, r_dt, r_hice_ref_safe, r_rhoiLf, r_tau_rad, r_atm_denom;
+    double Cs_ocean_safe, Cs_land_safe, Cs_ice_safe, r_Cs_ocean_safe, r_Cs_land_safe, r_Cs_ice_safe;
 };
+static inline void qd_colp_recips(QdColP& P) {
+    P.r_M_col = 1.0 / P.M_col; P.r_tau_c = 1.0 / P.tau_c; P.r_c_sfc_safe = 1.0 / P.c_sfc_safe; P.r_dt = 1.0 / P.dt;
+    P.r_hice_ref_safe = 1.0 / P.hice_ref_safe; P.r_rhoiLf = 1.0 / P.rhoiLf; P.r_tau_rad = 1.0 / P.tau_rad; P.r_atm_denom = 1.0 / P.atm_denom;
+    auto safe = [](double Cs) { return (std::isfinite(Cs) && Cs > 1e3) ? Cs : 1e3; };
+    P.Cs_ocean_safe = safe(P.Cs_ocean); P.Cs_land_safe = safe(P.Cs_land); P.Cs_ice_safe = safe(P.Cs_ice);
+    P.r_Cs_ocean_safe = 1.0 / P.Cs_ocean_safe; P.r_Cs_land_safe = 1.0 / P.Cs_land_safe; P.r_Cs_ice_safe = 1.0 / P.Cs_ice_safe;
+}
 
 __device__ __forceinline__ double qd_qsat(double T, double p0) {
     const double T_c = qd_clip(T - 273.15, -80.0, 60.0);
@@ -33,10 +43,10 @@
     const double deficit = qd_max(0.0, qd_qsat(Ts, P.p0) - q0);
     r.E = qd_nn(P.rhoCE * V * deficit * fac);
     r.LH = P.L_v * r.E;
-    const double q_evap = q0 + (r.E / P.M_col) * P.dt;
+    const double q_evap = q0 + qd_div_rc(r.E, P.M_col, P.r_M_col) * P.dt;
     const double excess = qd_max(0.0, q_evap - qsat_air);
-    double Pc = (excess / P.tau_c) * P.M_col;
-    double q_next = q_evap - (Pc / P.M_col) * P.dt;
+    double Pc = qd_div_rc(excess, P.tau_c, P.r_tau_c) * P.M_col;
+    double q_next = q_evap - qd_div_rc(Pc, P.M_col, P.r_M_col) * P.dt;
     q_next = qd_clip(qd_nn(q_next), 0.0, 0.5);
     r.Pc = qd_nn(Pc);
     r.LHrel = P.L_v * r.Pc;
@@ -47,7 +57,8 @@
 struct QdFlux { double SW_atm, SW_sfc, R, LW_atm, LW_sfc, OLR, SH; };
 
 __device__ __forceinline__ QdFlux qd_surface_fluxes(const QdColP& P, double I, double albedo, double cloud_eff,
-                                                    double Ts, double Ta, double u, double v, bool land, double hice) {
+                                                    double Ts, double Ta, double u, double v, bool land, double hice,
+                                                    bool has_ice_frac = false, double ice_frac_in = 0.0) {
     QdFlux F;
     const double alpha = qd_clip(albedo, 0.0, 1.0);
     const double Ic = qd_max(0.0, I);
@@ -66,7 +77,7 @@
         double es;
         if (land) es = P.eps_land;
         else {
-            const double ice_frac = 1.0 - exp(-qd_max(hice, 0.0) / P.hice_ref_safe);
+            const double ice_frac = has_ice_frac ? ice_frac_in : qd_ice_frac(hice, P.hice_ref_safe, P.r_hice_ref_safe);
             const double fi = qd_clip(ice_frac, 0.0, 1.0);
             es = (1.0 - fi) * P.eps_ocean + fi * P.eps_ice;
         }
diff --git a/qingdai_amd/csrc/qd_internal.h b/qingdai_amd/csrc/qd_internal.h
--- a/qingdai_amd/csrc/qd_internal.h
+++ b/qingdai_amd/csrc/qd_internal.h
@@ -52,11 +52,18 @@
     const double* mom_px;
     const double* ocn_igx;
     const double* inv_acos6;
+    const double* inv_2dx6;
+    const double* inv_fcor;
     const double* lat_deg;
     const double* lon_rad;
     const double* sin_lon;
     const double* cos_lon;
 };
+
+struct QdMet { double a, dlat, dlon, dlat2, dlon2, r_a, r_dlat, r_dlon, r_dlat2, r_dlon2; };
+static inline QdMet qd_met(double a, double dlat, double dlon) {
+    return QdMet{a, dlat, dlon, 2 * dlat, 2 * dlon, 1.0 / a, 1.0 / dlat, 1.0 / dlon, 1.0 / (2 * dlat), 1.0 / (2 * dlon)};
+}
 
 __device__ __forceinline__ double qd_nn(double x) {
     if (x != x) return 0.0;
diff --git a/qingdai_amd/csrc/qd_math.h b/qingdai_amd/csrc/qd_math.h
--- a/qingdai_amd/csrc/qd_math.h
+++ b/qingdai_amd/csrc/qd_math.h
@@ -49,3 +49,10 @@
 }
 
 QD_MATH_FN double qd_tanh(double x) { return copysign(qd_tanh_nonneg(fabs(x)), x); }
+
+QD_MATH_FN double qd_div_rc(double x, double c, double rc) {
+    const double q0 = x * rc;
+    const double e = fma(-c, q0, x);
+    const double q1 = fma(e, rc, q0);
+    return (q0 - q0 == 0.0 && q0 != 0.0) ? q1 : q0;
+}
diff --git a/qingdai_amd/csrc/qd_ocean.hip b/qingdai_amd/csrc/qd_ocean.hip
--- a/qingdai_amd/csrc/qd_ocean.hip
+++ b/qingdai_amd/csrc/qd_ocean.hip
@@ -140,7 +140,7 @@
 }
 
 struct QdFqsArgs {
-    const double* cosl; double dt, a, dlat, dlon, decay, dfac;
+    const double *cosl, *r_acosl; QdMet M; double dt, decay, dfac;
     double *u, *v, *h, *Ts, *q; const double* cloud_in; double* cloud_out;
     const double *isr, *albedo, *cloud_eff, *hice, *LH; const uint8_t* land; double* qnet; uint8_t* icemask;
     const double *uo, *vo; double vcap, rhoCD, tau_scale; double *taux, *tauy;
@@ -156,7 +156,7 @@
     if (j < G.nlon) {
         const size_t o = (size_t)qd_lrow(G, i) * G.nlon + j;
         const double uu = A.u[o], vv = A.v[o];
-        const QdBilin b = qd_departure(G, i, j, uu, vv, A.dt, A.a, A.cosl[i], A.dlat, A.dlon);
+        const QdBilin b = qd_departure(G, i, j, uu, vv, A.dt, A.M.a * A.cosl[i], A.r_acosl[i], A.M);
         double c = qd_gather(A.cloud_in, G, b);
         c = c * A.decay;
         const double cn = qd_nn(c * A.dfac), un = qd_nn(uu * A.dfac), vn = qd_nn(vv * A.dfac);
@@ -260,7 +260,7 @@
 }
 
 __global__ void __launch_bounds__(QD_BLOCK)
-k_continuity(QdGeom G, QdTabs T, double a, double dlat, double dlon, double msdtH, const double* __restrict__ uo,
+k_continuity(QdGeom G, QdTabs T, QdMet M, double msdtH, const double* __restrict__ uo,
              const double* __restrict__ vo, const uint8_t* __restrict__ land, double* __restrict__ eta,
              double* __restrict__ partial) {
     __shared__ double sm[QD_BLOCK / 64];
@@ -270,7 +270,7 @@
     double acc = 0.0;
     for (int j = threadIdx.x; j < G.nlon; j += QD_BLOCK) {
         const size_t o = b + j;
-        const double div = qd_divvort_point(G, T, uo, vo, i, j, a, dlat, dlon, 0);
+        const double div = qd_divvort_point(G, T, uo, vo, i, j, M, 0);
         double e = eta[o] + msdtH * div;
         const bool island = land[o] == 1;
         if (island) e = 0.0;
@@ -306,7 +306,7 @@
 }
 
 __global__ void __launch_bounds__(QD_BLOCK)
-k_cont_sstadv(QdGeom G, QdTabs T, double a, double dlat, double dlon, double msdtH, double sub_dt, double alpha,
+k_cont_sstadv(QdGeom G, QdTabs T, QdMet M, double msdtH, double sub_dt, double alpha,
               const double* __restrict__ uo, const double* __restrict__ vo, const uint8_t* __restrict__ land,
               double* __restrict__ eta, const double* __restrict__ Ts, double* __restrict__ Ts_out,
               int own0, int own1, double* __restrict__ partial, unsigned long long* ticket, double wsum,
@@ -316,18 +316,18 @@
     const int i = G.row0 + blockIdx.y;
     const size_t b = (size_t)qd_lrow(G, i) * G.nlon;
     const double w = (i >= own0 && i < own1) ? T.warea[i] : 0.0;
-    const double cosl = T.cos05[i];
+    const double acos = M.a * T.cos05[i], r_acos = T.ocn_igx[i];
     const int pidx = blockIdx.y * gridDim.x + blockIdx.x, pcount = gridDim.x * gridDim.y;
     double acc = 0.0;
     for (int j = blockIdx.x * QD_BLOCK + threadIdx.x; j < G.nlon; j += gridDim.x * QD_BLOCK) {
         const size_t o = b + j;
-        const double div = qd_divvort_point(G, T, uo, vo, i, j, a, dlat, dlon, 0);
+        const double div = qd_divvort_point(G, T, uo, vo, i, j, M, 0);
         double e = eta[o] + msdtH * div;
         const bool island = land[o] == 1;
         if (island) e = 0.0;
         eta[o] = e;
         acc += e * (island ? 0.0 : w);
-        const QdBilin bl = qd_departure(G, i, j, uo[o], vo[o], sub_dt, a, cosl, dlat, dlon);
+        const QdBilin bl = qd_departure(G, i, j, uo[o], vo[o], sub_dt, acos, r_acos, M);
         Ts_out[o] = (1.0 - alpha) * Ts[o] + alpha * qd_gather(Ts, G, bl);
     }
     acc = qd_wave_sum(acc);
@@ -364,7 +364,7 @@
 }
 
 __global__ void __launch_bounds__(QD_BLOCK)
-k_sst_advect(QdGeom G, const double* __restrict__ cos05, double sub_dt, double a, double dlat, double dlon,
+k_sst_advect(QdGeom G, const double* __restrict__ cos05, const double* __restrict__ r_acos05, double sub_dt, QdMet M,
              const double* __restrict__ uo, const double* __restrict__ vo, const double* __restrict__ Ts,
              double* __restrict__ Ts_out, double alpha, double* __restrict__ eta, const double* __restrict__ eta_mean,
              int has_ocean) {
@@ -374,7 +374,7 @@
     const int i = G.row0 + tl.row;
     const size_t o = (size_t)qd_lrow(G, i) * G.nlon + j;
     if (has_ocean) eta[o] = eta[o] - *eta_mean;
-    const QdBilin b = qd_departure(G, i, j, uo[o], vo[o], sub_dt, a, cos05[i], dlat, dlon);
+    const QdBilin b = qd_departure(G, i, j, uo[o], vo[o], sub_dt, M.a * cos05[i], r_acos05[i], M);
     const double adv = qd_gather(Ts, G, b);
     Ts_out[o] = (1.0 - alpha) * Ts[o] + alpha * adv;
 }
@@ -700,7 +700,7 @@
                 if (!compute_qnet) return qd_fail(c, "ocean step: a deferred k_final needs compute_qnet");
                 c->final_pending.on = 0;
                 QdFqsArgs A;
-                A.cosl = c->tabs.cos6; A.dt = c->final_pending.dt; A.a = p.a; A.dlat = c->dlat; A.dlon = c->dlon;
+                A.cosl = c->tabs.cos6; A.r_acosl = c->tabs.inv_acos6; A.dt = c->final_pending.dt; A.M = qd_met(p.a, c->dlat, c->dlon);
                 A.decay = c->final_pending.decay; A.dfac = c->final_pending.dfac;
                 A.u = F[QD_F_U]; A.v = F[QD_F_V]; A.h = F[QD_F_H]; A.Ts = F[QD_F_TS]; A.q = F[QD_F_Q];
                 A.cloud_in = F[QD_F_CLOUD]; A.cloud_out = qd_scratch(c, 0);
@@ -975,7 +975,7 @@
             const int has_ocean = c->wsum_ocean > 0.0 ? 1 : 0;
             if (!band) {
                 const dim3 g2 = qd_grid2d(Gown);
-                hipLaunchKernelGGL(k_cont_sstadv, g2, blk, 0, c->stream, Gown, c->tabs, p.a, c->dlat, c->dlon, -sub_dt * H, sub_dt,
+                hipLaunchKernelGGL(k_cont_sstadv, g2, blk, 0, c->stream, Gown, c->tabs, qd_met(p.a, c->dlat, c->dlon), -sub_dt * H, sub_dt,
                                    p.ocean_adv_alpha, F[QD_F_UO], F[QD_F_VO], c->land, F[QD_F_ETA], F[QD_F_SST], T1, own0, own1,
                                    c->red_partial, (unsigned long long*)nullptr, 0.0, (double*)nullptr);
                 if (!defer_eta)
@@ -985,7 +985,7 @@
                 QdSegs S = qd_segments(c, m);
                 size_t off = 0;
                 for (int k = 0; k < S.n; ++k) {
-                    hipLaunchKernelGGL(k_cont_sstadv, qd_grid2d(S.g[k]), blk, 0, c->stream, S.g[k], c->tabs, p.a, c->dlat, c->dlon,
+                    hipLaunchKernelGGL(k_cont_sstadv, qd_grid2d(S.g[k]), blk, 0, c->stream, S.g[k], c->tabs, qd_met(p.a, c->dlat, c->dlon),
                                        -sub_dt * H, sub_dt, p.ocean_adv_alpha, F[QD_F_UO], F[QD_F_VO], c->land, F[QD_F_ETA],
                                        F[QD_F_SST], T1, own0, own1, c->red_partial + off, (unsigned long long*)nullptr, 0.0,
                                        (double*)nullptr);
@@ -1038,7 +1038,7 @@
                     auto run = [&](int r0, int r1) {
                         if (r1 <= r0) return;
                         QdGeom g2 = G; g2.row0 = r0; g2.nrows = r1 - r0;
-                        hipLaunchKernelGGL(k_continuity, dim3(1, g2.nrows), blk, 0, c->stream, g2, c->tabs, p.a, c->dlat, c->dlon,
+                        hipLaunchKernelGGL(k_continuity, dim3(1, g2.nrows), blk, 0, c->stream, g2, c->tabs, qd_met(p.a, c->dlat, c->dlon),
                                            -sub_dt * H, F[QD_F_UO], F[QD_F_VO], c->land, F[QD_F_ETA],
                                            c->red_partial + (size_t)G0.lrows());
                     };
@@ -1046,7 +1046,7 @@
                     else { run(a0, std::max(a0, own0)); run(std::min(a1, own1), a1); }
                 }
             }
-            hipLaunchKernelGGL(k_continuity, rows, blk, 0, c->stream, Gown, c->tabs, p.a, c->dlat, c->dlon, -sub_dt * H,
+            hipLaunchKernelGGL(k_continuity, rows, blk, 0, c->stream, Gown, c->tabs, qd_met(p.a, c->dlat, c->dlon), -sub_dt * H,
                                F[QD_F_UO], F[QD_F_VO], c->land, F[QD_F_ETA], c->red_partial);
             qd_mark(c, {F[QD_F_ETA]}, m);
             if (band) {
@@ -1064,8 +1064,8 @@
             const int m1 = qd_plan(c, {QD_IN(F[QD_F_SST], Ro), QD_IN(F[QD_F_UO], 0), QD_IN(F[QD_F_VO], 0), QD_IN(F[QD_F_ETA], 0)});
             if (m1 < 0) return -1;
             double* T1 = qd_scratch(c, 0);
-            QD_ROWS(c, m1, G, hipLaunchKernelGGL(k_sst_advect, qd_grid2d(G), blk, 0, c->stream, G, c->tabs.cos05, sub_dt, p.a,
-                                                 c->dlat, c->dlon, F[QD_F_UO], F[QD_F_VO], F[QD_F_SST], T1, p.ocean_adv_alpha,
+            QD_ROWS(c, m1, G, hipLaunchKernelGGL(k_sst_advect, qd_grid2d(G), blk, 0, c->stream, G, c->tabs.cos05, c->tabs.ocn_igx, sub_dt,
+                                                 qd_met(p.a, c->dlat, c->dlon), F[QD_F_UO], F[QD_F_VO], F[QD_F_SST], T1, p.ocean_adv_alpha,
                                                  F[QD_F_ETA], c->dscal + QD_S_ETA_MEAN, c->wsum_ocean > 0.0 ? 1 : 0));
             qd_mark(c, {T1, F[QD_F_ETA]}, m1);
             double*& T1s = c->scratch[0];
diff --git a/qingdai_amd/csrc/qd_ocntail.hip b/qingdai_amd/csrc/qd_ocntail.hip
--- a/qingdai_amd/csrc/qd_ocntail.hip
+++ b/qingdai_amd/csrc/qd_ocntail.hip
@@ -24,41 +24,8 @@
     return __builtin_fma(e, rc, q0);
 }
 
-__device__ __forceinline__ QdBilin qt_departure(const QdGeom& G, int gi, int j, double u, double v, double dt,
-                                                double acos, double r_acos, const QdTailArgs& P) {
-    const double dl = qt_div(u * dt, acos, r_acos);
-    const double dp = qt_div(v * dt, P.a, P.r_a);
-    const double dx = qt_div(dl, P.dlon, P.r_dlon);
-    const double dy = qt_div(dp, P.dlat, P.r_dlat);
-    double r = qd_fold((double)gi - dy, G.nlat);
-    double cc = qd_fold((double)j - dx, G.nlon);
-    const bool nan_coord = (dx != dx) || (dy != dy);
-    r = fmin(fmax(r, 0.0), (double)(G.nlat - 1));
-    cc = fmin(fmax(cc, 0.0), (double)(G.nlon - 1));
-    const double r0f = floor(r), c0f = floor(cc);
-    QdBilin b;
-    const int r0 = (int)r0f, c0 = (int)c0f;
-    const int r1 = r0 + 1 < G.nlat ? r0 + 1 : G.nlat - 1;
-    b.c0 = c0; b.c1 = c0 + 1 < G.nlon ? c0 + 1 : G.nlon - 1;
-    b.l0 = qd_lrow_far(G, r0); b.l1 = qd_lrow_far(G, r1);
-    const double tr = r - r0f, tc = cc - c0f;
-    b.wr0 = 1.0 - tr; b.wr1 = tr; b.wc0 = 1.0 - tc; b.wc1 = tc;
-    b.nan_coord = nan_coord;
-    return b;
-}
-
-__device__ __forceinline__ double qt_div_point(const QdGeom& G, const QdTabs& T, const double* __restrict__ p,
-                                               const double* __restrict__ q, int i, int j, const QdTailArgs& P) {
-    const size_t b = (size_t)qd_lrow(G, i) * G.nlon;
-    const int jp = qd_wrapc(j + 1, G.nlon), jm = qd_wrapc(j - 1, G.nlon);
-    const double dp = qt_div(p[b + jp] - p[b + jm], 2 * P.dlon, P.r_2dlon);
-    double dq = 0.0;
-    if (i != 0 && i != G.nlat - 1) {
-        const double qn = q[(size_t)qd_lrow(G, i + 1) * G.nlon + j] * T.cos_raw[i + 1];
-        const double qs = q[(size_t)qd_lrow(G, i - 1) * G.nlon + j] * T.cos_raw[i - 1];
-        dq = qt_div(qn - qs, 2 * P.dlat, P.r_2dlat);
-    }
-    return T.inv_acos6[i] * (dp + dq);
+__device__ __forceinline__ QdMet qt_met(const QdTailArgs& P) {
+    return QdMet{P.a, P.dlat, P.dlon, 2 * P.dlat, 2 * P.dlon, P.r_a, P.r_dlat, P.r_dlon, P.r_2dlat, P.r_2dlon};
 }
 
 
@@ -182,7 +149,7 @@
 
 struct QtGather { double f00, f01, f10, f11, wr0, wr1, wc0, wc1; bool nan_coord; };
 __device__ __forceinline__ QtGather qt_gather_issue(const QdGeom& G, const QdTabs& T, const QdTailArgs& P, int gi, int j, double u, double v) {
-    const QdBilin b = qt_departure(G, gi, j, u, v, P.sub_dt, P.a * qd_sload(T.cos05, gi), qd_sload(T.ocn_igx, gi), P);
+    const QdBilin b = qd_departure(G, gi, j, u, v, P.sub_dt, P.a * qd_sload(T.cos05, gi), qd_sload(T.ocn_igx, gi), qt_met(P));
     const size_t r0 = (size_t)b.l0 * G.nlon, r1 = (size_t)b.l1 * G.nlon;
     QtGather q;
     q.f00 = P.Ts[r0 + b.c0]; q.f01 = P.Ts[r0 + b.c1]; q.f10 = P.Ts[r1 + b.c0]; q.f11 = P.Ts[r1 + b.c1];
diff --git a/qingdai_amd/csrc/qd_physics.hip b/qingdai_amd/csrc/qd_physics.hip
--- a/qingdai_amd/csrc/qd_physics.hip
+++ b/qingdai_amd/csrc/qd_physics.hip
@@ -10,7 +10,7 @@
 
 __global__ void __launch_bounds__(QD_BLOCK)
 k_precip_raw(QdGeom G, QdTabs T, const double* __restrict__ u, const double* __restrict__ v,
-             const double* __restrict__ pcond, double a, double dlat, double dlon, double D_crit, double beta,
+             const double* __restrict__ pcond, QdMet M, double D_crit, double beta,
              const double* __restrict__ scale_p, const unsigned long long* __restrict__ sel_state,
              double* __restrict__ praw, double* __restrict__ pos_out, double* __restrict__ partial,
              const double* __restrict__ orog) {
@@ -22,7 +22,7 @@
     const double scale = qd_max(*scale_p, 1e-12);
     double s_num = 0.0, s_den = 0.0;
     for (int j = threadIdx.x; j < G.nlon; j += QD_BLOCK) {
-        const double div = qd_divvort_point(G, T, u, v, i, j, a, dlat, dlon, 0);
+        const double div = qd_divvort_point(G, T, u, v, i, j, M, 0);
         const double pos = qd_max(0.0, -(div - D_crit));
         const double F_div = anypos ? qd_clip(pos / scale, 0.0, 5.0) : 0.0;
         const double Pq = qd_max(0.0, pcond[b + j]);
@@ -123,49 +123,53 @@
     return qd_clip(t, 0.0, 1.0);
 }
 
+struct QdSrcP { QdMet M; double dlon_a, dy2, r_dy2; };
+static inline QdSrcP qd_srcp(double a, double dlat, double dlon) {
+    const double dy = dlat * a;
+    return QdSrcP{qd_met(a, dlat, dlon), dlon * a, 2 * dy, 1.0 / (2 * dy)};
+}
 __device__ __forceinline__ double qd_cloud_source_cell(const QdGeom& G, const QdTabs& T, const double* __restrict__ u, const double* __restrict__ v,
-                                                       const double* __restrict__ Ts, double a, double dlat, double dlon, int i, int j);
+                                                       const double* __restrict__ Ts, const QdSrcP& S, int i, int j);
 
 __global__ void __launch_bounds__(QD_BLOCK)
 k_cloud_source(QdGeom G, QdTabs T, const double* __restrict__ u, const double* __restrict__ v,
-               const double* __restrict__ Ts, double a, double dlat, double dlon, double* __restrict__ out) {
+               const double* __restrict__ Ts, QdSrcP S, double* __restrict__ out) {
     const QdTile tl = qd_tile();
     const int j = tl.seg * QD_BLOCK + threadIdx.x;
     if (j >= G.nlon) return;
     const int i = G.row0 + tl.row;
-    out[(size_t)qd_lrow(G, i) * G.nlon + j] = qd_cloud_source_cell(G, T, u, v, Ts, a, dlat, dlon, i, j);
+    out[(size_t)qd_lrow(G, i) * G.nlon + j] = qd_cloud_source_cell(G, T, u, v, Ts, S, i, j);
 }
 
 __global__ void __launch_bounds__(QD_BLOCK)
 k_cloud_fromp_source(QdGeom G, QdTabs T, const double* __restrict__ precip, const double* __restrict__ pref, double cmax,
-                     const double* __restrict__ u, const double* __restrict__ v, const double* __restrict__ Ts, double a, double dlat,
-                     double dlon, double* __restrict__ cfp, double* __restrict__ src) {
+                     const double* __restrict__ u, const double* __restrict__ v, const double* __restrict__ Ts, QdSrcP S,
+                     double* __restrict__ cfp, double* __restrict__ src) {
     const QdTile tl = qd_tile();
     const int j = tl.seg * QD_BLOCK + threadIdx.x;
     if (j >= G.nlon) return;
     const int i = G.row0 + tl.row;
     const size_t o = (size_t)qd_lrow(G, i) * G.nlon + j;
     cfp[o] = cmax * qd_tanh(precip[o] / (*pref + 1e-12));
-    src[o] = qd_cloud_source_cell(G, T, u, v, Ts, a, dlat, dlon, i, j);
+    src[o] = qd_cloud_source_cell(G, T, u, v, Ts, S, i, j);
 }
 
 __device__ __forceinline__ double qd_cloud_source_cell(const QdGeom& G, const QdTabs& T, const double* __restrict__ u, const double* __restrict__ v,
-                                                       const double* __restrict__ Ts, double a, double dlat, double dlon, int i, int j) {
+                                                       const double* __restrict__ Ts, const QdSrcP& S, int i, int j) {
     const size_t b = (size_t)qd_lrow(G, i) * G.nlon;
     const size_t o = b + j;
     const double T0 = Ts[o];
     double src = 0.0;
-    src = src + 0.5 * qd_tanh01((T0 - 285.0) / 12.0);
-    const double vort = qd_divvort_point(G, T, v, u, i, j, a, dlat, dlon, 1);
-    const double rel = vort / (T.fcor[i] + 1e-12);
+    src = src + 0.5 * qd_tanh01(qd_div_rc(T0 - 285.0, 12.0, 1.0 / 12.0));
+    const double vort = qd_divvort_point(G, T, v, u, i, j, S.M, 1);
+    const double rel = qd_div_rc(vort, T.fcor[i] + 1e-12, T.inv_fcor[i]);
     src = src + 0.4 * qd_tanh01((rel - 0.5) / 2.0);
-    const double dx = dlon * a * T.cos6[i];
-    const double dy = dlat * a;
+    const double dx = S.dlon_a * T.cos6[i];
     const int jp = qd_wrapc(j + 1, G.nlon), jm = qd_wrapc(j - 1, G.nlon);
-    const double gx = (Ts[b + jp] - Ts[b + jm]) / (2 * dx);
-    const double gy = (Ts[(size_t)qd_lrow(G, i + 1) * G.nlon + j] - Ts[(size_t)qd_lrow(G, i - 1) * G.nlon + j]) / (2 * dy);
+    const double gx = qd_div_rc(Ts[b + jp] - Ts[b + jm], 2 * dx, T.inv_2dx6[i]);
+    const double gy = qd_div_rc(Ts[(size_t)qd_lrow(G, i + 1) * G.nlon + j] - Ts[(size_t)qd_lrow(G, i - 1) * G.nlon + j], S.dy2, S.r_dy2);
     const double tadv = -(u[o] * gx + v[o] * gy);
-    src = src + 0.3 * qd_tanh01(fabs(tadv) / 2e-5);
+    src = src + 0.3 * qd_tanh01(qd_div_rc(fabs(tadv), 2e-5, 1.0 / 2e-5));
     return src;
 }
 
@@ -200,7 +204,8 @@
     const int landv = land[o];
     const double cs = (P.snow && landv == 1) ? csnow[o] : 0.0;
     const double gl = (P.eco && landv == 1) ? glacier[o] : 0.0;
-    albedo[o] = qd_albedo_cell(P, o, c, cloud_eff, hice, base, landv, cs, gl, eco_alpha, banded, water);
+    albedo[o] = qd_albedo_cell(P, o, c, cloud_eff, qd_ice_frac(hice[o], P.hice_ref_safe, P.r_hice_ref_safe), base, landv, cs, gl, eco_alpha,
+                               banded, water);
 }
 
 __global__ void k_precip_scalars_post(const double* raw, double wsum, double pq_min, double p_blend, int use_fb, double* out) {
@@ -247,7 +252,7 @@
     const int j = tl.seg * QD_BLOCK + threadIdx.x;
     if (j >= K.G.nlon) return;
     const int i = K.G.row0 + tl.row;
-    qd_saf_cell(K, i, j, (size_t)qd_lrow(K.G, i) * K.G.nlon + j, true);
+    qd_saf_cell(K, qd_hour_cos(K.T, K.Fo.A, K.Fo.B, K.Fo.theta, j), i, (size_t)qd_lrow(K.G, i) * K.G.nlon + j, true);
 }
 int qd_saf_launch(qd_ctx* c, const QdSafArgs& K) {
     hipLaunchKernelGGL(k_snow_albedo_forcing, qd_grid2d(K.G), dim3(QD_BLOCK), 0, c->stream, K);
@@ -360,7 +365,7 @@
                     if (r1 <= r0) return;
                     QdGeom g2 = G; g2.row0 = r0; g2.nrows = r1 - r0;
                     hipLaunchKernelGGL(k_precip_raw, dim3(1, g2.nrows), blk, 0, c->stream, g2, c->tabs, F[QD_F_U], F[QD_F_V],
-                                       F[QD_F_PCOND], p.a, c->dlat, c->dlon, p.D_crit, p.p_betadiv, c->dscal + QD_S_PSCALE,
+                                       F[QD_F_PCOND], qd_met(p.a, c->dlat, c->dlon), p.D_crit, p.p_betadiv, c->dscal + QD_S_PSCALE,
                                        c->dcount, praw, pos, rp + (size_t)2 * G0.lrows(), orog);
                 };
                 const int a0 = G.row0, a1 = G.row0 + G.nrows;
@@ -369,7 +374,7 @@
             }
         }
         hipLaunchKernelGGL(k_precip_raw, dim3(1, Gown.nrows), blk, 0, c->stream, Gown, c->tabs, F[QD_F_U], F[QD_F_V],
-                           F[QD_F_PCOND], p.a, c->dlat, c->dlon, p.D_crit, p.p_betadiv, c->dscal + QD_S_PSCALE, c->dcount, praw,
+                           F[QD_F_PCOND], qd_met(p.a, c->dlat, c->dlon), p.D_crit, p.p_betadiv, c->dscal + QD_S_PSCALE, c->dcount, praw,
                            pos, rp, orog);
         qd_mark(c, {praw, pos}, m);
         if (band && qd_peer_hooks(c)) {
@@ -439,12 +444,12 @@
         if (c->merge_pointwise) {
             m = ms = std::min(m, ms);
             QD_ROWS(c, m, G, hipLaunchKernelGGL(k_cloud_fromp_source, qd_grid2d(G), blk, 0, c->stream, G, c->tabs, F[QD_F_PRECIP],
-                                                c->dscal + QD_S_MED_OUT, p.cmax, F[QD_F_U], F[QD_F_V], F[QD_F_TS], p.a, c->dlat, c->dlon, cfp, src));
+                                                c->dscal + QD_S_MED_OUT, p.cmax, F[QD_F_U], F[QD_F_V], F[QD_F_TS], qd_srcp(p.a, c->dlat, c->dlon), cfp, src));
         } else {
         QD_ROWS(c, m, G, hipLaunchKernelGGL(k_cloud_from_p, qd_grid2d(G), blk, 0, c->stream, G, F[QD_F_PRECIP],
                                             c->dscal + QD_S_MED_OUT, p.cmax, cfp));
         QD_ROWS(c, ms, G, hipLaunchKernelGGL(k_cloud_source, qd_grid2d(G), blk, 0, c->stream, G, c->tabs, F[QD_F_U], F[QD_F_V],
-                                             F[QD_F_TS], p.a, c->dlat, c->dlon, src));
+                                             F[QD_F_TS], qd_srcp(p.a, c->dlat, c->dlon), src));
         }
         qd_mark(c, {cfp}, m);
         qd_mark(c, {src}, ms);
@@ -492,7 +497,8 @@
                  p.cloud_advect ? 1 : 0, p.use_topo_albedo ? 1 : 0, p.swe_enable ? 1 : 0,
                  (E.configured && E.p.albedo_couple && E.alpha_valid) ? 1 : 0, (E.configured && E.p.bands_couple && E.banded_valid) ? 1 : 0,
                  ((E.configured && E.p.water_couple && E.water_valid) || qd_phyto_daily_couples(c)) ? 1 : 0,
-                 (E.configured && E.p.map_f32) ? 1 : 0};
+                 (E.configured && E.p.map_f32) ? 1 : 0, 0.0};
+        A.r_hice_ref_safe = 1.0 / A.hice_ref_safe;
         if (A.eco) { const int me = qd_plan(c, {QD_IN(F[QD_F_ECO_ALPHA], 0)}); if (me < 0) return -1; m = std::min(m, me); }
         if (A.banded) { const int me = qd_plan(c, {QD_IN(F[QD_F_ECO_ALPHA_BANDED], 0)}); if (me < 0) return -1; m = std::min(m, me); }
         if (A.water) { const int me = qd_plan(c, {QD_IN(F[QD_F_WATER_ALPHA], 0)}); if (me < 0) return -1; m = std::min(m, me); }
@@ -506,6 +512,7 @@
             S.ddf_s = p.snow_ddf_mm_per_k_day / 86400.0; S.tref = p.snow_melt_tref_K; S.rate_s = p.snow_melt_rate_mm_day / 86400.0;
             S.swe_max = (p.swe_max_mm == p.swe_max_mm && p.swe_max_mm > 0) ? p.swe_max_mm : -1.0;
             S.swe_ref_safe = std::max(1e-6, p.swe_ref_mm); S.gl_frac = p.glacier_frac; S.gl_swe = p.glacier_swe_mm; S.swe = p.swe_enable;
+            qd_snowp_recips(S);
             if (fc) {
                 const QdForcingP Fo{QdStar{fc->sa[0], std::sin(fc->sa[1]), std::cos(fc->sa[1]), fc->sa[2]},
                                     QdStar{fc->sb[0], std::sin(fc->sb[1]), std::cos(fc->sb[1]), fc->sb[2]}, fc->theta, 5.670374e-8, 1};
diff --git a/qingdai_amd/csrc/qd_phyto.hip b/qingdai_amd/csrc/qd_phyto.hip
--- a/qingdai_amd/csrc/qd_phyto.hip
+++ b/qingdai_amd/csrc/qd_phyto.hip
@@ -3,7 +3,7 @@
 #include <vector>
 
 __global__ void __launch_bounds__(QD_BLOCK)
-k_phyto_advect(QdGeom G, const double* __restrict__ cos05, double dt, double a, double dlat, double dlon,
+k_phyto_advect(QdGeom G, const double* __restrict__ cos05, const double* __restrict__ r_acos05, double dt, QdMet M,
                const double* __restrict__ uo, const double* __restrict__ vo, const double* __restrict__ Cst,
                double* __restrict__ Tst, size_t stride, double alpha, int scrub) {
     const QdTile tl = qd_tile();
@@ -12,7 +12,7 @@
     const int i = G.row0 + tl.row;
     const size_t o = (size_t)qd_lrow(G, i) * G.nlon + j;
     const double* __restrict__ C = Cst + (size_t)tl.fld * stride;
-    const QdBilin b = qd_departure(G, i, j, uo[o], vo[o], dt, a, cos05[i], dlat, dlon);
+    const QdBilin b = qd_departure(G, i, j, uo[o], vo[o], dt, M.a * cos05[i], r_acos05[i], M);
     const double adv = qd_gather(C, G, b);
     const double v = (1.0 - alpha) * C[o] + alpha * adv;
     Tst[(size_t)tl.fld * stride + o] = scrub ? qd_nn(v) : v;
@@ -128,8 +128,8 @@
     in.push_back(QD_IN(F[QD_F_UO], 0)); in.push_back(QD_IN(F[QD_F_VO], 0));
     const int m1 = qd_plan(c, in.data(), (int)in.size());
     if (m1 < 0) return -1;
-    QD_ROWS(c, m1, G, hipLaunchKernelGGL(k_phyto_advect, qd_grid2d(G, P.S), blk, 0, c->stream, G, c->tabs.cos05, dt, p.a, c->dlat,
-                                         c->dlon, F[QD_F_UO], F[QD_F_VO], P.stack[0], P.stack[1], P.stride, P.alpha, has_diff));
+    QD_ROWS(c, m1, G, hipLaunchKernelGGL(k_phyto_advect, qd_grid2d(G, P.S), blk, 0, c->stream, G, c->tabs.cos05, c->tabs.ocn_igx, dt,
+                                         qd_met(p.a, c->dlat, c->dlon), F[QD_F_UO], F[QD_F_VO], P.stack[0], P.stack[1], P.stride, P.alpha, has_diff));
     for (int s = 0; s < P.S; ++s) qd_mark(c, {P.tmp[s]}, m1);
     in.clear();
     for (int s = 0; s < P.S; ++s) in.push_back(QD_IN(P.tmp[s], has_diff ? 2 : 0));
diff --git a/qingdai_amd/csrc/qd_pointwise.h b/qingdai_amd/csrc/qd_pointwise.h
--- a/qingdai_amd/csrc/qd_pointwise.h
+++ b/qingdai_amd/csrc/qd_pointwise.h
@@ -1,23 +1,29 @@
 #pragma once
 #include "qd_internal.h"
+#include "qd_math.h"
+
 
 struct QdSnowP {
     double dt, ga, rho_snow_safe, polar_lat, ice_max, elev_max, gamma, t_thresh, dT, ddf_s, tref, rate_s, swe_max, swe_ref_safe,
            gl_frac, gl_swe;
     int lapse, mode, swe;
+    double r_dt, r_rho_snow_safe, r_dT, r_swe_ref_safe;
 };
+static inline void qd_snowp_recips(QdSnowP& S) {
+    S.r_dt = 1.0 / S.dt; S.r_rho_snow_safe = 1.0 / S.rho_snow_safe; S.r_dT = 1.0 / S.dT; S.r_swe_ref_safe = 1.0 / S.swe_ref_safe;
+}
 struct QdSnowOut { double Pr, Sn, melt, Cs, gl; };
 
 __device__ __forceinline__ QdSnowOut qd_snow_cell(const QdTabs& T, const QdSnowP& P, int i, bool is_land, double hval, double S0, double elev,
                                                   double Pf) {
     QdSnowOut r;
     const double T_a = 288.0 + P.ga * hval;
-    const double h_snow = is_land ? qd_max(S0, 0.0) / P.rho_snow_safe : 0.0;
+    const double h_snow = is_land ? qd_div_rc(qd_max(S0, 0.0), P.rho_snow_safe, P.r_rho_snow_safe) : 0.0;
     const bool polar = fabs(T.lat_deg[i]) >= P.polar_lat;
     const double h_ice_eff = polar ? qd_min(h_snow, P.ice_max) : h_snow;
     const double H_eff = qd_min(elev + h_ice_eff, P.elev_max);
-    const double T_hat = P.lapse ? T_a - P.gamma * (H_eff / 1000.0) : T_a;
-    double f_snow = 1.0 / (1.0 + exp((T_hat - P.t_thresh) / P.dT));
+    const double T_hat = P.lapse ? T_a - P.gamma * qd_div_rc(H_eff, 1000.0, 1.0 / 1000.0) : T_a;
+    double f_snow = 1.0 / (1.0 + exp(qd_div_rc(T_hat - P.t_thresh, P.dT, P.r_dT)));
     f_snow = qd_clip(f_snow, 0.0, 1.0);
     const double Ps = qd_nn(f_snow * Pf);
     const double Pr = qd_nn((1.0 - f_snow) * Pf);
@@ -31,8 +37,8 @@
     double Sn = S0 + Ps_land * P.dt - actual;
     if (P.swe_max > 0.0) Sn = qd_min(Sn, P.swe_max);
     Sn = qd_max(0.0, Sn);
-    const double melt_out = (P.dt > 0) ? actual / P.dt : 0.0;
-    const double Cs = qd_clip(1.0 - exp(-qd_max(Sn, 0.0) / P.swe_ref_safe), 0.0, 1.0);
+    const double melt_out = (P.dt > 0) ? qd_div_rc(actual, P.dt, P.r_dt) : 0.0;
+    const double Cs = qd_clip(1.0 - exp(qd_div_rc(-qd_max(Sn, 0.0), P.swe_ref_safe, P.r_swe_ref_safe)), 0.0, 1.0);
     Sn = qd_nn(Sn);
     const bool gl = is_land && ((Cs >= P.gl_frac) || (Sn >= P.gl_swe));
     const double Pr_gl = (Pr * (is_land ? 1.0 : 0.0)) * (gl ? 1.0 : 0.0);
@@ -41,15 +47,19 @@
     return r;
 }
 
-struct QdAlbP { double alpha, hice_ref_safe, alpha_ice, alpha_cloud, alpha_water, alpha_snow, w_lai; int do_adv, use_topo, snow, eco, banded, water, eco_f32; };
+struct QdAlbP { double alpha, hice_ref_safe, alpha_ice, alpha_cloud, alpha_water, alpha_snow, w_lai; int do_adv, use_topo, snow, eco, banded, water, eco_f32;
+                double r_hice_ref_safe; };
+
+__device__ __forceinline__ double qd_ice_frac(double hice, double hice_ref_safe, double r_hice_ref_safe) {
+    return 1.0 - exp(qd_div_rc(-qd_max(hice, 0.0), hice_ref_safe, r_hice_ref_safe));
+}
 
 __device__ __forceinline__ double qd_albedo_cell(const QdAlbP& P, size_t o, double c, const double* __restrict__ cloud_eff,
-                                                 const double* __restrict__ hice, const double* __restrict__ base, int landv, double cs, double gl,
+                                                 double ice_frac, const double* __restrict__ base, int landv, double cs, double gl,
                                                  const double* __restrict__ eco_alpha, const double* __restrict__ banded,
                                                  const double* __restrict__ water) {
     const double crad = cloud_eff ? cloud_eff[o] : c;
     const double C = qd_clip(crad, 0.0, 1.0);
-    const double ice_frac = 1.0 - exp(-qd_max(hice[o], 0.0) / P.hice_ref_safe);
     double fi = qd_clip(ice_frac, 0.0, 1.0);
     fi = fi * ((landv == 0) ? 1.0 : 0.0);
     double b0 = P.use_topo ? base[o] : P.alpha_water;
@@ -71,24 +81,34 @@
 }
 
 struct QdStar { double flux, sin_d, cos_d, alpha; };
-struct QdForcingP { QdStar A, B; double theta, sigma; int with_teq; };
+struct QdForcingP { QdStar A, B; double theta, sigma; int with_teq; double r_sigma = 1.0 / 5.670374e-8; };
 
+struct QdHourCos { double cA, cB; };
+__device__ __forceinline__ double qd_hour_cos1(const QdTabs& T, double alpha, double theta, int j) {
+    const double lon = T.lon_rad[j];
+    return cos(theta + lon - alpha);
+}
+__device__ __forceinline__ QdHourCos qd_hour_cos(const QdTabs& T, const QdStar& A, const QdStar& B, double theta, int j) {
+    return QdHourCos{qd_hour_cos1(T, A.alpha, theta, j), qd_hour_cos1(T, B.alpha, theta, j)};
+}
+__device__ __forceinline__ void qd_star_insolation(const QdTabs& T, const QdStar& A, const QdStar& B, const QdHourCos& H, int i,
+                                                   double& a_, double& b_) {
+    const double sl = T.sin_raw[i], cl = T.cos_raw[i];
+    const double czA = qd_max(0.0, sl * A.sin_d + cl * A.cos_d * H.cA);
+    const double czB = qd_max(0.0, sl * B.sin_d + cl * B.cos_d * H.cB);
+    a_ = A.flux * czA; b_ = B.flux * czB;
+}
 __device__ __forceinline__ void qd_star_insolation(const QdTabs& T, const QdStar& A, const QdStar& B, double theta, int i, int j,
                                                    double& a_, double& b_) {
-    const double sl = T.sin_raw[i], cl = T.cos_raw[i], lon = T.lon_rad[j];
-    const double hA = theta + lon - A.alpha;
-    const double hB = theta + lon - B.alpha;
-    const double czA = qd_max(0.0, sl * A.sin_d + cl * A.cos_d * cos(hA));
-    const double czB = qd_max(0.0, sl * B.sin_d + cl * B.cos_d * cos(hB));
-    a_ = A.flux * czA; b_ = B.flux * czB;
+    qd_star_insolation(T, A, B, qd_hour_cos(T, A, B, theta, j), i, a_, b_);
 }
 
 struct QdForcingOut { double tot, teq; };
-__device__ __forceinline__ QdForcingOut qd_forcing_cell(const QdTabs& T, const QdForcingP& P, int i, int j, size_t o, double alb,
+__device__ __forceinline__ QdForcingOut qd_forcing_cell(const QdTabs& T, const QdForcingP& P, const QdHourCos& H, int i, size_t o, double alb,
                                                         double* __restrict__ isrA, double* __restrict__ isrB, double* __restrict__ isr,
                                                         double* __restrict__ Teq, double* __restrict__ eday, double eday_dt) {
     double a_, b_;
-    qd_star_insolation(T, P.A, P.B, P.theta, i, j, a_, b_);
+    qd_star_insolation(T, P.A, P.B, H, i, a_, b_);
     const double tot = a_ + b_;
     if (isrA) { isrA[o] = a_; isrB[o] = b_; }
     isr[o] = tot;
@@ -97,8 +117,13 @@
     if (P.with_teq) {
         double num = tot * (1 - alb);
         if (num < 0) num = 0;
-        r.teq = sqrt(sqrt(num / P.sigma));
+        r.teq = sqrt(sqrt(qd_div_rc(num, P.sigma, P.r_sigma)));
         if (Teq) Teq[o] = r.teq;
     }
     return r;
 }
+__device__ __forceinline__ QdForcingOut qd_forcing_cell(const QdTabs& T, const QdForcingP& P, int i, int j, size_t o, double alb,
+                                                        double* __restrict__ isrA, double* __restrict__ isrB, double* __restrict__ isr,
+                                                        double* __restrict__ Teq, double* __restrict__ eday, double eday_dt) {
+    return qd_forcing_cell(T, P, qd_hour_cos(T, P.A, P.B, P.theta, j), i, o, alb, isrA, isrB, isr, Teq, eday, eday_dt);
+}
diff --git a/qingdai_amd/csrc/qd_saf.h b/qingdai_amd/csrc/qd_saf.h
--- a/qingdai_amd/csrc/qd_saf.h
+++ b/qingdai_amd/csrc/qd_saf.h
@@ -11,9 +11,9 @@
     double *albedo, *isrA, *isrB, *isr, *Teq, *eday; double eday_dt;
     int write_diag, col1; QdColP P; const double *u, *v, *Ts, *q; double* Pcond;
 };
-struct QdSafOut { double cloud, albedo, isr, teq; };
+struct QdSafOut { double cloud, albedo, isr, teq, ice_frac; };
 
-__device__ __forceinline__ QdSafOut qd_saf_cell(const QdSafArgs& K, int i, int j, size_t o, bool store_teq) {
+__device__ __forceinline__ QdSafOut qd_saf_cell(const QdSafArgs& K, const QdHourCos& H, int i, size_t o, bool store_teq) {
     const int landv = K.land[o];
     const double hh = K.h[o];
     if (K.col1) {
@@ -25,9 +25,10 @@
     if (K.write_diag) { K.P_rain[o] = r.Pr; K.S_next[o] = r.Sn; K.melt[o] = r.melt; K.C_snow[o] = r.Cs; K.glacier[o] = r.gl; }
     double c = K.cloud[o];
     if (K.A.do_adv) { c = qd_clip((1.0 - K.A.alpha) * c + K.A.alpha * K.adv[o], 0.0, 1.0); K.cloud[o] = c; }
-    const double alb = qd_albedo_cell(K.A, o, c, K.cloud_eff, K.hice, K.base, landv, r.Cs, r.gl, K.eco_alpha, K.banded, K.water);
+    const double ice_frac = qd_ice_frac(K.hice[o], K.A.hice_ref_safe, K.A.r_hice_ref_safe);
+    const double alb = qd_albedo_cell(K.A, o, c, K.cloud_eff, ice_frac, K.base, landv, r.Cs, r.gl, K.eco_alpha, K.banded, K.water);
     K.albedo[o] = alb;
-    const QdForcingOut f = qd_forcing_cell(K.T, K.Fo, i, j, o, alb, K.write_diag ? K.isrA : nullptr, K.isrB, K.isr, store_teq ? K.Teq : nullptr,
+    const QdForcingOut f = qd_forcing_cell(K.T, K.Fo, H, i, o, alb, K.write_diag ? K.isrA : nullptr, K.isrB, K.isr, store_teq ? K.Teq : nullptr,
                                            K.eday, K.eday_dt);
-    return QdSafOut{c, alb, f.tot, f.teq};
+    return QdSafOut{c, alb, f.tot, f.teq, ice_frac};
 }
diff --git a/qingdai_amd/csrc/qd_stencil.hip b/qingdai_amd/csrc/qd_stencil.hip
--- a/qingdai_amd/csrc/qd_stencil.hip
+++ b/qingdai_amd/csrc/qd_stencil.hip
@@ -218,7 +218,7 @@
 
 __global__ void __launch_bounds__(QD_BLOCK)
 k_advect(QdGeom G, const double* __restrict__ u, const double* __restrict__ v, const double* __restrict__ cosl,
-         double dt, double a, double dlat, double dlon,
+         const double* __restrict__ r_acosl, double dt, QdMet M,
          const double* __restrict__ f0, double* __restrict__ o0,
          const double* __restrict__ f1, double* __restrict__ o1, double alpha, int clipq) {
     const QdTile tl = qd_tile();
@@ -226,7 +226,7 @@
     if (j >= G.nlon) return;
     const int i = G.row0 + tl.row;
     const size_t o = (size_t)qd_lrow(G, i) * G.nlon + j;
-    const QdBilin b = qd_departure(G, i, j, u[o], v[o], dt, a, cosl[i], dlat, dlon);
+    const QdBilin b = qd_departure(G, i, j, u[o], v[o], dt, M.a * cosl[i], r_acosl[i], M);
     const bool blend = (alpha != 1.0);
     {
         const double adv = qd_gather(f0, G, b);
@@ -242,25 +242,26 @@
 
 void qd_launch_advect(qd_ctx* c, const double* u, const double* v, const double* coslat, double dt,
                       const double* f0, double* o0, const double* f1, double* o1, double alpha, int clipq, int m) {
-    QD_ROWS(c, m, G, hipLaunchKernelGGL(k_advect, qd_grid2d(G), dim3(QD_BLOCK), 0, c->stream, G, u, v, coslat, dt,
-                                        c->p.a, c->dlat, c->dlon, f0, o0, f1, o1, alpha, clipq));
+    const double* r_acosl = coslat == c->tabs.cos05 ? c->tabs.ocn_igx : c->tabs.inv_acos6;
+    QD_ROWS(c, m, G, hipLaunchKernelGGL(k_advect, qd_grid2d(G), dim3(QD_BLOCK), 0, c->stream, G, u, v, coslat, r_acosl, dt,
+                                        qd_met(c->p.a, c->dlat, c->dlon), f0, o0, f1, o1, alpha, clipq));
     qd_mark(c, {o0, o1}, m);
 }
 
 __global__ void __launch_bounds__(QD_BLOCK)
 k_divvort(QdGeom G, QdTabs T, const double* __restrict__ u, const double* __restrict__ v, double* __restrict__ out,
-          double a, double dlat, double dlon, int vort) {
+          QdMet M, int vort) {
     const QdTile tl = qd_tile();
     const int j = tl.seg * QD_BLOCK + threadIdx.x;
     if (j >= G.nlon) return;
     const int i = G.row0 + tl.row;
     out[(size_t)qd_lrow(G, i) * G.nlon + j] =
-        vort ? qd_divvort_point(G, T, v, u, i, j, a, dlat, dlon, 1) : qd_divvort_point(G, T, u, v, i, j, a, dlat, dlon, 0);
+        vort ? qd_divvort_point(G, T, v, u, i, j, M, 1) : qd_divvort_point(G, T, u, v, i, j, M, 0);
 }
 
 void qd_launch_divvort(qd_ctx* c, const double* u, const double* v, double* out, int vort, int m) {
     QD_ROWS(c, m, G, hipLaunchKernelGGL(k_divvort, qd_grid2d(G), dim3(QD_BLOCK), 0, c->stream, G, c->tabs, u, v, out,
-                                        c->p.a, c->dlat, c->dlon, vort));
+                                        qd_met(c->p.a, c->dlat, c->dlon), vort));
     qd_mark(c, {out}, m);
 }
 
```

New measurement: 4.988 planet-days/s (median of 5 runs). Within noise of the previous version (+0.5%).
